# IIT-PAVIS/DiffAssemble

Hardware: AMD Instinct MI355X
Metric: denoising steps/sec (900-piece dense graph, T=100) (higher is better)
Workload: dtype bf16

## Files before the change

### diffassemble_amd/_lib.py

```python
import ctypes as C
import os

import torch

LIB_PATH = os.environ.get("DA_LIB_PATH") or os.path.join(os.path.dirname(os.path.abspath(__file__)), "lib", "libdiffassemble_hip.so")
DA_MAX_LAYERS = 8
ABI_VERSION = 19
PREC_F32, PREC_BF16 = 0, 1
VARIANT_2D, VARIANT_3D, VARIANT_DISCRETE, VARIANT_DISCRETE_ROT = 0, 1, 2, 3
ARCH_TRANSFORMER, ARCH_EXOPHORMER, ARCH_GCN = 0, 1, 2
MEAN_EPSILON, MEAN_START_X = 0, 1
ACT_NONE, ACT_GELU, ACT_LEAKY02 = 0, 1, 2
CONV_Q_PRESCALED, CONV_FOLDED_V32 = 1, 2
TRAIN_MMA_FP32, TRAIN_MMA_BF16 = 0, 1
TRAIN_BWD_ALL, TRAIN_BWD_EARLY, TRAIN_BWD_LATE = 0, 1, 2
D3PM_DRAW_SAMPLING, D3PM_DRAW_TRAINING, D3PM_DRAW_SAMPLING_ROT = 0, 1, 2
D3PM_LOSS = {"vb": 0, "cross_entropy": 1, "hybrid": 2}
DBG_COUNTERS = ("opt_gen_workgroups", "dense_fast_exits", "dual_gen_slabs", "opt_masked_gen_workgroups")
DBG_LAUNCH_COUNTERS = {"resident_launches": 4, "virtual_rows_in_launch": 5,
                       "resident_projection_launches": 6}
PROF_CLASSES = ("embed", "linear_mlp", "linear_qkvs", "attn_hidden", "attn_last", "head", "update", "conv_fused")

_fp = C.c_void_p
_FPL = _fp * DA_MAX_LAYERS


class DaWeights(C.Structure):
    _fields_ = [
        ("variant", C.c_int32), ("arch", C.c_int32), ("steps", C.c_int32), ("c_in", C.c_int32),
        ("c_out", C.c_int32), ("feat_dim", C.c_int32), ("hidden", C.c_int32), ("heads", C.c_int32),
        ("n_layers", C.c_int32), ("virt_nodes", C.c_int32),
        ("time_emb", _fp),
        ("pos_w0", _fp), ("pos_b0", _fp), ("pos_w1", _fp), ("pos_b1", _fp),
        ("mlp_w0", _fp), ("mlp_b0", _fp), ("mlp_w1", _fp), ("mlp_b1", _fp),
        ("conv_wq", _FPL), ("conv_bq", _FPL), ("conv_wk", _FPL), ("conv_bk", _FPL),
        ("conv_wv", _FPL), ("conv_bv", _FPL), ("conv_ws", _FPL), ("conv_bs", _FPL),
        ("virt_emb", _fp),
        ("head_w0", _fp), ("head_b0", _fp), ("head_w1", _fp), ("head_b1", _fp),
        ("head_r_w0", _fp), ("head_r_b0", _fp), ("head_r_w1", _fp), ("head_r_b1", _fp),
    ]


class DaGraph(C.Structure):
    _fields_ = [
        ("n_nodes", C.c_int32), ("n_real", C.c_int32), ("n_graphs", C.c_int32), ("dense", C.c_int32),
        ("n_edges", C.c_int64),
        ("row_ptr", _fp), ("col_src", _fp), ("edge_id", _fp), ("graph_ptr", _fp),
        ("max_graph_nodes", C.c_int32), ("n_pad", C.c_int32),
        ("pad_ptr", _fp), ("row_map", _fp),
        ("out_ptr", _fp), ("out_dst", _fp),
        ("hybrid", C.c_int32), ("band_degree", C.c_int32),
        ("mask", _fp), ("mask_ptr", _fp), ("irr_row_ptr", _fp), ("irr_col_src", _fp),
        ("slot_node", _fp), ("blk_class", _fp), ("blk_class_ptr", _fp), ("blk_class_stride", C.c_int32), ("reserved1", C.c_int32),
        ("rm_meta", _fp), ("agg_row_ptr", _fp), ("agg_col_src", _fp), ("agg_mult", _fp),
    ]


class DaLoopOpts(C.Structure):
    _fields_ = [("sampler", C.c_int32), ("eta", C.c_float), ("cfg", C.c_int32), ("cfg_w", C.c_float), ("noise", C.c_void_p)]


class DaD3pmOpts(C.Structure):
    _fields_ = [("cfg", C.c_int32), ("cfg_w", C.c_float), ("noise", C.c_void_p), ("seed", C.c_void_p)]


class DaD3pmRotOpts(C.Structure):
    _fields_ = [("cold", C.c_int32), ("reserved0", C.c_int32), ("x_fixed", C.c_void_p), ("noise_x", C.c_void_p), ("noise_rot", C.c_void_p),
                ("seed", C.c_void_p)]


class DaSchedule(C.Structure):
    _fields_ = [
        ("steps", C.c_int32),
        ("betas", _fp), ("alphas_cumprod", _fp), ("sqrt_recip_alphas", _fp),
        ("sqrt_recip_alphas_cumprod", _fp), ("sqrt_recipm1_alphas_cumprod", _fp),
        ("sqrt_one_minus_alphas_cumprod", _fp), ("posterior_variance", _fp),
    ]


ENCODER_CONVS, ENCODER_FEATS = 19, 1088


class DaEncoderWeights(C.Structure):
    _fields_ = [
        ("n_convs", C.c_int32), ("reserved0", C.c_int32),
        ("stem_w", _fp), ("stem_b", _fp),
        ("conv_w", _fp * ENCODER_CONVS), ("conv_b", _fp * ENCODER_CONVS),
        ("lin1_w", _fp), ("lin1_b", _fp), ("lin2_w", _fp), ("lin2_b", _fp),
    ]


PCD_STAGES, PCD_K = 3, 20


class DaPcdEncoderWeights(C.Structure):
    _fields_ = [
        ("feat_dim", C.c_int32), ("reserved0", C.c_int32),
        ("premap", _fp * PCD_STAGES), ("bn_a", _fp * PCD_STAGES), ("conv_b", _fp * PCD_STAGES),
        ("conv6", _fp), ("linear0", _fp),
    ]


LOSS3D_TRANS, LOSS3D_SHAPE_CD, LOSS3D_ROT, LOSS3D_ALL = 1, 2, 4, 7
PCD_TRAIN_LAYERS = 8


class DaPcdTrainWeights(C.Structure):
    _fields_ = [
        ("feat_dim", C.c_int32), ("reserved0", C.c_int32),
        ("premap", _fp * PCD_STAGES), ("bn_a", _fp * PCD_STAGES), ("conv_b", _fp * PCD_STAGES),
        ("conv6", _fp), ("linear0", _fp),
        ("gamma", _fp * PCD_TRAIN_LAYERS), ("beta", _fp * PCD_TRAIN_LAYERS),
        ("running_mean", _fp * PCD_TRAIN_LAYERS), ("running_var", _fp * PCD_TRAIN_LAYERS),
        ("momentum", C.c_float * PCD_TRAIN_LAYERS), ("eps", C.c_float * PCD_TRAIN_LAYERS),
        ("inv_wf", _fp * 2), ("inv_wd", _fp * 2),
    ]


class DaPcdTrainGrads(C.Structure):
    _fields_ = [
        ("wf", _fp * 6), ("wd", _fp * 6), ("gamma", _fp * 6), ("beta", _fp * 6),
        ("linear0_w", _fp), ("linear0_b", _fp), ("points", _fp),
    ]


PCD_PASSES = ("PREMAP", "EDGE_STAT_A", "EDGE_STAT_B", "EDGE_BWD1", "EDGE_BWD2", "EDGE_BWD3", "C6_STAT", "C6_BWD1", "C6_BWD2", "C6_DX",
              "BN_FIN_FWD", "BN_FIN_BWD", "REV_ADJ", "GATHER", "PREMAP_WGRAD", "HEAD_BWD", "LIN0_GRAD", "VN_LIN", "VN_STAT", "VN_APPLY")
PCD_PASS = {n: i for i, n in enumerate(PCD_PASSES)}


class DaPcdPassArgs(C.Structure):
    _fields_ = ([(n, C.c_int32) for n in ("n_parts", "n_points", "cin", "feat", "has_b", "inv", "channels", "nblk", "ld_x", "ld_g", "ld_m",
                                         "vn_cin")]
                + [("count", C.c_double), ("momentum", C.c_float), ("eps", C.c_float)]
                + [(n, _fp) for n in ("x", "w", "w2", "T", "idx", "rec_a", "rec_b", "dX_in", "partial", "Gb", "Hb", "E", "X1", "X2", "X3", "dm_in",
                                      "G6", "F", "dX1", "dX2", "dX3", "gamma", "beta", "running_mean", "running_var", "run_out", "ss",
                                      "dgamma", "dbeta", "cnt", "ptr", "cur", "rev", "dXp", "dTc", "Xc", "dWm", "dwf", "dwd", "grad_out",
                                      "dm", "vP", "vD", "vY")])


def pcd_train_pass(name, stream=None, **fields):
    a = DaPcdPassArgs()
    keys = dict(DaPcdPassArgs._fields_)
    for k, v in fields.items():
        if k not in keys:
            raise DaError(f"da_pcd_pass_args has no field {k!r}")
        setattr(a, k, v.data_ptr() if torch.is_tensor(v) else v)
    check(lib().da_pcd_train_pass(PCD_PASS[name], C.byref(a), stream if stream is not None else stream_ptr()))


class DaConfig(C.Structure):
    _fields_ = [(n, C.c_int32) for n in ("struct_bytes", "disable_mfma", "disable_dense", "disable_folds", "attn_level", "xpanel", "tail_next",
                                         "pair_split", "train_attn", "train_side_streams")]


PROTOTYPES = {
    "da_abi_version": (C.c_int, []),
    "da_last_error": (C.c_char_p, []),
    "da_config_get": (C.c_int, [C.POINTER(DaConfig)]),
    "da_config_set": (C.c_int, [C.POINTER(DaConfig)]),
    "da_build_flags": (C.c_int, []),
    "da_denoiser_create": (C.c_int, [C.POINTER(DaWeights), C.c_int, _fp, C.POINTER(_fp)]),
    "da_denoiser_destroy": (None, [_fp]),
    "da_denoiser_flags": (C.c_int, [_fp]),
    "da_gcn_dinv": (C.c_int, [C.POINTER(DaGraph), _fp, _fp]),
    "da_gcn_aggregate": (C.c_int, [C.c_int, C.POINTER(DaGraph), C.c_int, _fp, _fp, _fp, C.c_int, _fp, _fp]),
    "da_denoiser_workspace_bytes": (C.c_size_t, [_fp, C.POINTER(DaGraph)]),
    "da_denoiser_set_features": (C.c_int, [_fp, C.POINTER(DaGraph), _fp, _fp, C.c_size_t, _fp]),
    "da_denoiser_forward": (C.c_int, [_fp, C.POINTER(DaGraph), _fp, _fp, C.c_int64, _fp, _fp, C.c_int, _fp, _fp,
                                      C.c_size_t, _fp]),
    "da_ddim_step": (C.c_int, [C.POINTER(DaSchedule), C.c_int, C.c_int, C.c_int, C.c_int, _fp, _fp, _fp,
                               C.c_int64, C.c_int, C.c_int, C.c_float, _fp, _fp, _fp]),
    "da_ddpm_step": (C.c_int, [C.POINTER(DaSchedule), C.c_int, C.c_int, _fp, _fp, _fp, C.c_int64, _fp, _fp, _fp]),
# ... 158 lines not shown
```

### diffassemble_amd/csrc/da_api.hip

```cpp
#include <stdarg.h>
#include <stdlib.h>
#include <string.h>

#include <utility>
#include <vector>

#include "da_common.h"
#include "da_internal.h"
#include "da_config.h"

namespace da {

static thread_local char g_err[1024] = "";

void set_error(const char *fmt, ...) {
    va_list ap;
    va_start(ap, fmt);
    vsnprintf(g_err, sizeof(g_err), fmt, ap);
    va_end(ap);
}

struct ConvW {
    void *w = nullptr;
    float *b = nullptr;
    void *wd = nullptr;
    float *bd = nullptr;
    void *wdp = nullptr;
    void *wqs = nullptr;
    int din = 0, hc = 0, C = 0;
};

__global__ void k_scale_block(float *p, int rows, int cols, int ld, float s) {
    const size_t i = (size_t)blockIdx.x * blockDim.x + threadIdx.x;
    if (i < (size_t)rows * cols) p[(i / cols) * ld + (i % cols)] *= s;
}
static int scale_block(float *p, int rows, int cols, int ld, float s, hipStream_t st) {
    const size_t n = (size_t)rows * cols;
    if (!n) return 0;
    k_scale_block<<<(unsigned)((n + 255) / 256), 256, 0, st>>>(p, rows, cols, ld, s);
    DA_LAUNCH_CHECK();
    return 0;
}
__global__ void k_fill_bias_rows(int prec, int rows, int cols, const float *bias, void *dst) {
    const size_t i = (size_t)blockIdx.x * blockDim.x + threadIdx.x;
    if (i >= (size_t)rows * cols) return;
    const float v = bias[i % cols];
    if (prec == DA_PREC_BF16) ((bf16_t *)dst)[i] = f2bf(v); else ((float *)dst)[i] = v;
}
__global__ void k_cfg_combine(size_t n, float wgt, float *cond, const float *unc) {
    const size_t i = (size_t)blockIdx.x * blockDim.x + threadIdx.x;
    if (i < n) cond[i] = (1.0f + wgt) * cond[i] - wgt * unc[i];
}
static bool q_prescale_on() { return !(cfg().disable_folds & DA_FOLD_QSCALE); }
static float q_scale_log2(int C) { return 1.4426950408889634f / sqrtf((float)C); }

struct LoopKey {
    da_graph g;
    da_schedule s;
    int mean_type, ratio, max_iters;
    const float *x_init;
    float *traj, *x_final;
    void *ws;
    size_t ws_bytes;
    da_loop_opts opts;
    size_t traj_stride;
    size_t noise_stride;
    da_config cfg;
    const void *seed;
    const void *rot_init, *rot_traj, *rot_final, *x_fixed, *noise_rot;
    int cold;
};

}

using namespace da;

struct da_denoiser {
    int prec = 0, variant = 0, arch = 0, steps = 0, c_in = 0, c_out = 0, F = 0, D = 0, hidden = 0, heads = 0,
        n_layers = 0, V = 0, head_hidden = 0;
    float *time_emb = nullptr, *pos_w0 = nullptr, *pos_b0 = nullptr, *pos_w1 = nullptr, *pos_b1 = nullptr;
    void *mlp_w0 = nullptr, *mlp_w1 = nullptr;
    float *mlp_b0 = nullptr, *mlp_b1 = nullptr;
    ConvW conv[DA_MAX_LAYERS];
    void *virt_emb = nullptr;
    void *head_w0 = nullptr;
    float *head_b0 = nullptr;
    float *head_w1 = nullptr, *head_b1 = nullptr, *head_r_w1 = nullptr, *head_r_b1 = nullptr;
    bool fused_mlp2 = false;
    void *conv0c_w = nullptr;
    float *conv0c_b = nullptr;
    void *headc_w = nullptr;
    float *headc_b = nullptr;
    void *virt_qkvs = nullptr;
    void *conv0c_wd = nullptr, *virt_qkvs_d = nullptr;
    void *conv0c_wdp = nullptr, *convLf_wp = nullptr;
    void *conv0c_wqs = nullptr;
    bool attn_qsf = false;
    float *conv0c_bd = nullptr;
    bool q_prescaled = false;
    bool lastfold = false;
    bool dense_only = false;
    void *convLf_w = nullptr;
    float *convLf_b = nullptr;
    void *skipc_w = nullptr;
    float *skipc_b = nullptr;
    std::vector<void *> owned;
    bool prof_on = false;
    std::vector<hipEvent_t> prof_ev;
    std::vector<int> prof_cls;
    size_t prof_used = 0;
    struct LoopEntry { LoopKey a, b; hipGraphExec_t exec, exec_b; };
    std::vector<LoopEntry> loops;
    hipStream_t cap_stream = nullptr;
    hipStream_t side_stream = nullptr;
    hipEvent_t ev_fork = nullptr, ev_join = nullptr;
    hipStream_t pair_stream = nullptr;
    hipEvent_t ev_pair_fork = nullptr, ev_pair_join = nullptr;
    std::vector<LoopEntry> pair_loops;
};

namespace da {

struct Workspace {
    char *comb_in, *h, *combined, *qkvs, *xa, *xb, *z, *hh;
    char *hh_unc, *pz_unc, *head_pre_unc;
    void *pz;
    char *head_pre;
    char *feat_proj;
    char *feat_proj_unc;
    char *feat_proj4;
    size_t proj4_stride;
    float *model_out_unc;
    char *dq, *dk, *dvt, *dskip;
    size_t dense_off, dense_bytes;
    unsigned *virt_cnt;
    float *virt_part;
    float *model_out, *xbuf0, *xbuf1;
    float *gcn_dinv;
    size_t total;
};

static Workspace carve(const da_denoiser *d, const da_graph *g, void *base) {
    const size_t s = esize(d->prec);
    const size_t n = (size_t)g->n_nodes, nr = (size_t)g->n_real;
    const size_t nrp = nr + 64, np = n + 64;
    char *p = (char *)base;
    size_t off = 0;
    auto take = [&](size_t bytes) {
        char *q = p ? p + off : nullptr;
        off += align_up(bytes, 256);
        return q;
    };
    Workspace w;
    int hcmax = 0;
    for (int l = 0; l < d->n_layers; ++l) hcmax = d->conv[l].hc > hcmax ? d->conv[l].hc : hcmax;
    w.comb_in = take(nrp * d->D * s);
    w.h = take(nrp * d->hidden * s);
    w.feat_proj = take(nrp * d->hidden * s);
    w.feat_proj_unc = take(nrp * d->hidden * s);
    const bool rotv = d->variant == DA_VARIANT_DISCRETE_ROT;
    w.head_pre = take(nrp * (rotv ? 64 : 32) * s);
    w.pz = take(nrp * 32 * (size_t)d->heads * sizeof(float));
    w.combined = take(np * d->D * s);
    const bool gcn = d->arch == DA_ARCH_GCN;
    w.qkvs = take(gcn ? 0 : np * 4 * (size_t)hcmax * s);
    w.xa = take(np * 256 * s);
    w.xb = take(np * 256 * s);
    w.z = take(np * d->D * s);
    w.hh = take(nrp * d->head_hidden * s);
    const bool disc = d->variant == DA_VARIANT_DISCRETE;
    w.hh_unc = take(disc ? nrp * d->head_hidden * s : 0);
    w.pz_unc = take(disc ? nrp * 32 * (size_t)d->heads * sizeof(float) : 0);
    w.head_pre_unc = take(disc ? nrp * 32 * s : 0);
    w.dq = w.dk = w.dvt = w.dskip = nullptr;
    w.virt_cnt = nullptr; w.virt_part = nullptr;
    w.dense_off = off;
    w.dense_bytes = 0;
    if ((g->dense || g->hybrid) && g->n_pad > 0 && !gcn) {
        const size_t hb = ((size_t)g->n_pad + 64) * hcmax * s;
        w.dq = take(hb);
        w.dk = take(hb);
        w.dvt = take(hb);
        if (g->hybrid && n > nr) w.virt_cnt = (unsigned *)take((n - nr) * sizeof(unsigned));
        w.dense_bytes = off - w.dense_off;
        if (g->hybrid && n > nr) w.virt_part = (float *)take((n - nr) * (size_t)DA_VIRT_SPLIT_MAX * 64 * 6 * sizeof(float));
        w.dskip = take(np * (size_t)hcmax * s);
    }
    const int cpose = d->variant == DA_VARIANT_3D ? 7 : d->c_out;
    w.model_out = (float *)take(nr * cpose * sizeof(float));
    w.model_out_unc = (float *)take(nr * cpose * sizeof(float));
    w.xbuf0 = (float *)take(nr * 8 * sizeof(float));
    w.xbuf1 = (float *)take(nr * 8 * sizeof(float));
    w.gcn_dinv = d->arch == DA_ARCH_GCN ? (float *)take(n * sizeof(float)) : nullptr;
    w.proj4_stride = align_up(nrp * d->hidden * s, 256) / s;
    w.feat_proj4 = take(rotv ? 4 * w.proj4_stride * s : 0);
    w.total = off;
    return w;
}

static bool mfma_disabled() { return cfg().disable_mfma != 0; }

int linear(int prec, int M, int K, int Nout, const void *A, int lda, const void *W, const float *bias, int act,
           const void *res, void *out, int ldo, hipStream_t st) {
    if (!mfma_disabled()) {
        const int rc = launch_gemm_mfma(prec, M, K, Nout, A, lda, W, bias, act, res, out, ldo, nullptr, st);
        if (rc >= 0) return rc;
    }
    return launch_gemm_simple(prec == DA_PREC_F32_BF16MMA ? DA_PREC_F32 : prec, M, K, Nout, A, lda, W, bias, act, res, out, ldo, st);
}

static bool dense_disabled() { return cfg().disable_dense != 0; }

static bool step_rule_batch(const da_graph *g) { return g->max_graph_nodes >= 512 || g->n_real >= 16384; }

static bool stream_is_capturing(hipStream_t st) {
    hipStreamCaptureStatus cs = hipStreamCaptureStatusNone;
    return hipStreamIsCapturing(st, &cs) == hipSuccess && cs == hipStreamCaptureStatusActive;
}

static bool dense_ok(const da_graph *g, int heads, int C) {
    const bool hyb = g->hybrid && g->mask && g->mask_ptr && g->irr_row_ptr;
    return !dense_disabled() && (g->dense || hyb) && g->n_pad > 0 && g->graph_ptr && g->pad_ptr && g->row_map && heads == 8 &&
           (C == 32 || C == 144) && !mfma_disabled();
}

static int check_graph(const da_denoiser *d, const da_graph *g) {
    DA_REQUIRE(g && g->n_real > 0 && g->n_nodes >= g->n_real, "da_graph: bad node counts");
    const bool hyb = g->hybrid && g->mask && g->mask_ptr && g->irr_row_ptr;
    if (!((g->dense || hyb) && d->dense_only)) DA_REQUIRE(g->row_ptr && (g->col_src || g->n_edges == 0), "da_graph: CSR arrays missing");
    DA_REQUIRE(d->V == 0 || g->n_nodes == g->n_real + d->V * g->n_graphs,
               "da_graph: exophormer expects n_nodes = n_real + V*G (%d vs %d + %d*%d)", g->n_nodes, g->n_real,
               d->V, g->n_graphs);
    return 0;
}

static DeviceSchedule to_dev(const da_schedule *s) {
    DeviceSchedule r;
    r.steps = s->steps;
    r.betas = s->betas;
    r.alphas_cumprod = s->alphas_cumprod;
    r.sqrt_recip_alphas = s->sqrt_recip_alphas;
    r.sqrt_recip_alphas_cumprod = s->sqrt_recip_alphas_cumprod;
    r.sqrt_recipm1_alphas_cumprod = s->sqrt_recipm1_alphas_cumprod;
    r.sqrt_one_minus_alphas_cumprod = s->sqrt_one_minus_alphas_cumprod;
    r.posterior_variance = s->posterior_variance;
    return r;
}

template <typename F>
static int timed(da_denoiser *d, int cls, hipStream_t st, F &&launch) {
    if (!d->prof_on) return launch();
    if (d->prof_used + 2 > d->prof_ev.size()) {
        for (int k = 0; k < 2; ++k) {
            hipEvent_t e;
            DA_CHECK_HIP(hipEventCreate(&e));
            d->prof_ev.push_back(e);
        }
    }
    hipEvent_t a = d->prof_ev[d->prof_used], b = d->prof_ev[d->prof_used + 1];
    DA_CHECK_HIP(hipEventRecord(a, st));
    int rc = launch();
    DA_CHECK_HIP(hipEventRecord(b, st));
    d->prof_used += 2;
    d->prof_cls.push_back(cls);
    return rc;
}

struct DiscreteIn {
    const int32_t *idx;
    char *hh;
    char *pz, *pre;
    int folded;
    int rot = 0;
    const int32_t *rot_acc = nullptr;
    D3pmRows rows() const { D3pmRows r; if (folded) { r.pz = pz; r.pre = pre; } else r.hh = hh; return r; }
};

static int forward_impl(da_denoiser *d, const da_graph *g, const float *x, const int64_t *t, int64_t t_scalar,
                        float *out, float *alpha, int alpha_all, float *pre_head, const Workspace &w,
                        hipStream_t st, DdimFuse *ddim = nullptr, bool uncond = false, bool h_ready = false,
                        DiscreteIn *disc = nullptr) {
    const int prec = d->prec, nr = g->n_real, n = g->n_nodes, D = d->D;
    int rc;
    VirtScatter vsc;
    bool virt_scattered = false;
    if (!h_ready && d->fused_mlp2 && n > nr && !alpha && w.dq && d->virt_qkvs_d && dense_ok(g, d->heads, d->conv[0].C) && DA_XENV("DA_VIRT_SCATTER_IN_EMBED", 1)) {
        vsc.rows = n - nr; vsc.V = d->V; vsc.H = d->heads; vsc.C = d->conv[0].C; vsc.n_real = nr; vsc.n_pad = g->n_pad;
        vsc.src = d->virt_qkvs_d; vsc.row_map = g->row_map; vsc.Q = w.dq; vsc.K = w.dk; vsc.Vt = w.dvt; vsc.S = w.dskip;
        virt_scattered = true;
    }
    if (disc) {
        disc->folded = 0;
        if ((rc = timed(d, DA_PROF_EMBED, st, [&] {
                 if (disc->rot)
                     return launch_embed_idx_time_rot(prec, nr, d->c_out, d->F, D, d->hidden, disc->idx, disc->rot_acc, t, t_scalar, d->steps, d->time_emb,
                                                      d->pos_w1, w.comb_in, w.feat_proj4, w.proj4_stride, w.feat_proj, st);
                 return launch_embed_idx_time(prec, nr, d->c_out, d->F, D, disc->idx, t, t_scalar, d->steps, d->time_emb, d->pos_w1, w.comb_in, st); }))) return rc;
    } else
    if (!h_ready && (rc = timed(d, DA_PROF_EMBED, st, [&] {
             return launch_embed_pos_time(prec, nr, d->c_in, d->F, D, x, t, t_scalar, d->steps, d->time_emb,
                                          d->pos_w0, d->pos_b0, d->pos_w1, d->pos_b1, w.comb_in, st, virt_scattered ? &vsc : nullptr); }))) return rc;
    const int act1 = d->variant == DA_VARIANT_3D ? DA_ACT_LEAKY02 : DA_ACT_GELU;
    const int act2 = d->variant == DA_VARIANT_3D ? DA_ACT_LEAKY02 : DA_ACT_NONE;
    if (!h_ready && (rc = timed(d, DA_PROF_LINEAR_MLP, st, [&] {
             const size_t es_ = esize(prec);
             int r2 = mfma_disabled() ? -1
                                      : launch_gemm_mfma(prec, nr, D - d->F, d->hidden, w.comb_in + (size_t)d->F * es_, D,
                                                         (const char *)d->mlp_w0 + (size_t)d->F * es_, nullptr, act1, nullptr,
                                                         w.h, d->hidden, nullptr, st, D, uncond ? w.feat_proj_unc : w.feat_proj);
             if (r2 >= 0) return r2;
             if (uncond) { set_error("unconditional pass: the hoisted mlp.0 path is not available for this shape"); return 1; }
             if (disc && disc->rot) { set_error("discrete rot: the hoisted mlp.0 path is not available for this shape"); return 1; }
             return linear(prec, nr, D, d->hidden, w.comb_in, D, d->mlp_w0, d->mlp_b0, act1, nullptr, w.h, d->hidden, st); }))) return rc;
    const bool fused = d->fused_mlp2;
    if (!fused && (rc = timed(d, DA_PROF_LINEAR_MLP, st, [&] {
             return linear(prec, nr, d->hidden, D, w.h, d->hidden, d->mlp_w1, d->mlp_b1, act2, nullptr, w.combined, D, st); }))) return rc;
    const void *xin = fused ? w.h : w.combined;
    int ldx = fused ? d->hidden : D;
    if (d->arch == DA_ARCH_GCN) {
        const ConvW &c0 = d->conv[0], &c1 = d->conv[1];
        const int hid = c0.hc;
        if ((rc = timed(d, DA_PROF_LINEAR_QKVS, st, [&] {
                 return linear(prec, nr, D, hid, w.combined, D, c0.w, nullptr, DA_ACT_NONE, nullptr, w.xa, hid, st); }))) return rc;
        if ((rc = timed(d, DA_PROF_ATTN_HIDDEN, st, [&] {
                 return launch_gcn_aggregate(prec, g, hid, w.gcn_dinv, w.xa, c0.b, DA_ACT_GELU, w.xb, st); }))) return rc;
        if ((rc = timed(d, DA_PROF_ATTN_LAST, st, [&] {
                 return launch_gcn_aggregate(prec, g, hid, w.gcn_dinv, w.xb, nullptr, DA_ACT_NONE, w.xa, st); }))) return rc;
        if ((rc = timed(d, DA_PROF_LINEAR_QKVS, st, [&] {
                 return linear(prec, nr, hid, D, w.xa, hid, c1.w, c1.b, DA_ACT_GELU, w.combined, w.z, D, st); }))) return rc;
    } else
    for (int l = 0; l < d->n_layers; ++l) {
        ConvW c = d->conv[l];
        if (fused && l == 0) { c.w = d->conv0c_w; c.b = d->conv0c_b; c.din = d->hidden; }
        const int nproj = (fused && l == 0) ? nr : n;
        const bool virt0 = fused && l == 0 && n > nr;
        const bool last = l == d->n_layers - 1;
        void *dst = last ? (void *)w.z : (void *)((l & 1) ? w.xb : w.xa);
        const int act = (!last && d->arch == DA_ARCH_TRANSFORMER) ? DA_ACT_GELU : DA_ACT_NONE;
        float *al = !alpha ? nullptr
                           : (alpha_all ? alpha + (size_t)l * g->n_edges * d->heads : (last ? alpha : nullptr));
        const void *resid = (last && !fused) ? w.combined : nullptr;
        if (last && fused && d->lastfold && !al && w.dq && (g->hybrid || d->V == 0) && dense_ok(g, d->heads, c.C)) {
            QkvScatter qs;
            qs.HC = c.hc; qs.C = c.C; qs.Cv = 32; qs.n_pad = g->n_pad; qs.row_map = g->row_map;
            qs.Q = w.dq; qs.K = w.dk; qs.Vt = w.dvt; qs.S = nullptr;
            rc = timed(d, DA_PROF_LINEAR_QKVS, st, [&] {
                return launch_gemm_mfma(prec, n, c.din, 2 * c.hc + d->heads * 32, xin, ldx, d->convLf_w, d->convLf_b, DA_ACT_NONE,
                                        nullptr, nullptr, 0, &qs, st, 0, nullptr, d->convLf_wp); });
            if (rc > 0) return rc;
            if (rc == 0) {
                DenseLayout L;
                L.Q = w.dq; L.K = w.dk; L.Vt = w.dvt; L.S = nullptr; L.n_pad = g->n_pad; L.q_prescaled = d->q_prescaled;
                DenseFold fo;
                fo.cv = 32; fo.out = disc ? (void *)disc->pz : w.pz; fo.n_rows = nr;
                const DenseMask mk = dense_mask_of(g);
                rc = timed(d, DA_PROF_ATTN_LAST, st, [&] {
                    return launch_attn_dense(prec, L, d->heads, c.C, g->n_graphs, g->max_graph_nodes, g->graph_ptr,
                                             g->pad_ptr, g->dense == 2, nullptr, DA_ACT_NONE, nullptr, st,
                                             g->hybrid ? &mk : nullptr, &fo); });
                if (rc > 0) return rc;
                if (rc == 0 && disc) {
                    if ((rc = timed(d, DA_PROF_HEAD, st, [&] {
                             return linear(prec, nr, d->hidden, 32, w.h, d->hidden, d->headc_w, d->headc_b, DA_ACT_NONE, nullptr, disc->pre, 32, st); }))) return rc;
                    if ((rc = timed(d, DA_PROF_HEAD, st, [&] {
                             return linear(prec, nr, c.din, 32, xin, ldx, d->skipc_w, d->skipc_b, DA_ACT_NONE, disc->pre, disc->pre, 32, st); }))) return rc;
                    disc->folded = 1;
                    return 0;
                }
                if (rc == 0) {
                    {
                        const bool fuse_ddim = ddim && d->c_out == d->c_in;
                        int rt = -1;
                        if ((rc = timed(d, DA_PROF_HEAD, st, [&] {
                                 rt = launch_tail_fused(prec, nr, d->heads, d->c_out, d->hidden, c.din, w.h, xin, ldx, d->headc_w, d->headc_b,
                                                        d->skipc_w, d->skipc_b, w.pz, d->head_w1, d->head_b1, out, st, fuse_ddim ? ddim : nullptr);
                                 return rt > 0 ? rt : 0; }))) return rc;
                        if (rt == 0) { if (fuse_ddim) ddim->done = 1; return 0; }
                    }
                    if ((rc = timed(d, DA_PROF_HEAD, st, [&] {
                             return linear(prec, nr, d->hidden, 32, w.h, d->hidden, d->headc_w, d->headc_b, DA_ACT_NONE, nullptr, w.head_pre, 32, st); }))) return rc;
                    if ((rc = timed(d, DA_PROF_HEAD, st, [&] {
                             return linear(prec, nr, c.din, 32, xin, ldx, d->skipc_w, d->skipc_b, DA_ACT_NONE, w.head_pre, w.head_pre, 32, st); }))) return rc;
                    if (ddim && d->c_out == d->c_in) ddim->done = 1;
                    return timed(d, DA_PROF_HEAD, st, [&] {
                        return launch_head_fold(prec, nr, d->heads, d->c_out, w.pz, w.head_pre, d->head_w1, d->head_b1, out, st,
                                                (ddim && ddim->done) ? ddim : nullptr); });
                }
            }
        }
#ifdef DA_EXPERIMENTS
        if (!al && !last && g->dense && !g->hybrid && n == nr && !resid && dense_ok(g, d->heads, c.C) &&
            conv_fused_applicable(prec, d->heads, c.C, c.din, g->max_graph_nodes, c.hc)) {
            rc = timed(d, DA_PROF_CONV_FUSED, st, [&] {
                return launch_conv_fused(prec, d->heads, c.C, c.din, g->n_graphs, g->max_graph_nodes, g->graph_ptr,
                                         g->dense == 2, xin, ldx, c.w, c.b, act, dst, c.hc, st); });
            if (rc) return rc < 0 ? 1 : rc;
            xin = dst; ldx = c.hc;
            continue;
        }
#endif
        if (!al && w.dq && dense_ok(g, d->heads, c.C)) {
            QkvScatter qs;
            qs.HC = c.hc; qs.C = c.C; qs.n_pad = g->n_pad; qs.row_map = g->row_map;
            qs.Q = w.dq; qs.K = w.dk; qs.Vt = w.dvt; qs.S = w.dskip;
            const void *wdense = (fused && l == 0) ? d->conv0c_wd : c.wd;
            const float *bdense = (fused && l == 0) ? d->conv0c_bd : c.bd;
            const int xpm = xpanel_mode();
            const void *wpanel = (xpm == 1 || (xpm == 2 && step_rule_batch(g))) ? ((fused && l == 0) ? d->conv0c_wdp : c.wdp) : nullptr;
            const void *wqs = (fused && l == 0) ? d->conv0c_wqs : c.wqs;
            const bool qsf = !last && !g->hybrid && !resid && !virt0 && n == nr && wqs && ldx == c.din &&
                             attn_qsf_applicable(prec, d->heads, c.C, c.din, g->n_graphs, g->max_graph_nodes, g->n_pad, d->q_prescaled);
            if (qsf) rc = 0; else
            rc = timed(d, DA_PROF_LINEAR_QKVS, st, [&] {
                return launch_gemm_mfma(prec, nproj, c.din, 4 * c.hc, xin, ldx, wdense, bdense, DA_ACT_NONE, nullptr, nullptr, 0, &qs, st, 0,
                                        nullptr, wpanel); });
            if (rc > 0) return rc;
            if (rc == 0 && virt0 && !virt_scattered &&
                (rc = launch_scatter_virtual(prec, n - nr, d->V, d->heads, c.C, d->virt_qkvs_d, nr, g->row_map, g->n_pad, w.dq, w.dk,
                                             w.dvt, w.dskip, nullptr, st))) return rc;
            if (rc == 0) {
                DenseLayout L;
                L.Q = w.dq; L.K = w.dk; L.Vt = w.dvt; L.S = w.dskip; L.n_pad = g->n_pad; L.q_prescaled = d->q_prescaled;
                if (qsf) { L.x = xin; L.ldx = ldx; L.kin = c.din; L.wqs = wqs; L.bias = bdense; }
                if (g->hybrid) {
                    DenseMask mk = dense_mask_of(g);
                    int virt_taken = 0;
                    [[maybe_unused]] const int vil = DA_XENV("DA_VIRT_IN_LAUNCH", 1);
                    if (n > nr && !resid && w.virt_cnt && w.virt_part && !(cfg().disable_folds & DA_FOLD_HYBRID_OVERLAP) && vil && (g->n_real < 8192 || vil == 2)) {
                        mk.v_rows = n - nr; mk.v_n_real = nr;
                        mk.v_row_ptr = g->agg_row_ptr ? g->agg_row_ptr : g->irr_row_ptr; mk.v_col_src = g->agg_row_ptr ? g->agg_col_src : g->irr_col_src;
                        mk.v_mult = g->agg_row_ptr ? g->agg_mult : nullptr;
                        mk.v_part = w.virt_part; mk.v_cnt = w.virt_cnt; mk.v_taken = &virt_taken;
                        rc = timed(d, last ? DA_PROF_ATTN_LAST : DA_PROF_ATTN_HIDDEN, st, [&] {
                            return launch_attn_dense(prec, L, d->heads, c.C, g->n_graphs, g->max_graph_nodes, g->graph_ptr, g->pad_ptr, 0, resid, act, dst, st, &mk); });
                        if (rc) return rc < 0 ? 1 : rc;
                        if (!virt_taken) {
                            rc = timed(d, last ? DA_PROF_ATTN_LAST : DA_PROF_ATTN_HIDDEN, st, [&] {
                                return launch_attn_csr_cont(prec, n, nr, mk.v_row_ptr, mk.v_col_src, g->row_map, d->heads, c.C, g->n_pad, L, resid, act, dst, st, mk.v_mult); });
                            if (rc) return rc < 0 ? 1 : rc;
                        }
                        xin = dst; ldx = c.hc;
                        continue;
                    }
                    if (d->side_stream && !d->prof_on && n > nr && g->n_real >= 8192) {
                        StreamJoin side_guard;
                        DA_CHECK_HIP(hipEventRecord(d->ev_fork, st));
                        DA_CHECK_HIP(hipStreamWaitEvent(d->side_stream, d->ev_fork, 0));
                        side_guard.arm(d->side_stream, st, d->ev_join);
                        rc = launch_attn_csr_cont(prec, n, nr, g->agg_row_ptr ? g->agg_row_ptr : g->irr_row_ptr, g->agg_row_ptr ? g->agg_col_src : g->irr_col_src,
                                                  g->row_map, d->heads, c.C, g->n_pad, L, resid, act, dst, d->side_stream, g->agg_row_ptr ? g->agg_mult : nullptr);
                        if (rc) return rc < 0 ? 1 : rc;
                        DA_CHECK_HIP(hipEventRecord(d->ev_join, d->side_stream));
                        rc = launch_attn_dense(prec, L, d->heads, c.C, g->n_graphs, g->max_graph_nodes, g->graph_ptr,
                                               g->pad_ptr, 0, resid, act, dst, st, &mk);
                        if (rc) return rc < 0 ? 1 : rc;
                        DA_CHECK_HIP(hipStreamWaitEvent(st, d->ev_join, 0));
                        side_guard.armed = false;
                        xin = dst; ldx = c.hc;
                        continue;
                    }
                    rc = timed(d, last ? DA_PROF_ATTN_LAST : DA_PROF_ATTN_HIDDEN, st, [&] {
                        int r2 = launch_attn_dense(prec, L, d->heads, c.C, g->n_graphs, g->max_graph_nodes, g->graph_ptr,
                                                   g->pad_ptr, 0, resid, act, dst, st, &mk);
                        if (r2) return r2;
                        return launch_attn_csr_cont(prec, n, nr, g->agg_row_ptr ? g->agg_row_ptr : g->irr_row_ptr, g->agg_row_ptr ? g->agg_col_src : g->irr_col_src,
                                                    g->row_map, d->heads, c.C, g->n_pad, L, resid, act, dst, st, g->agg_row_ptr ? g->agg_mult : nullptr); });
                    if (rc) return rc < 0 ? 1 : rc;
                    xin = dst; ldx = c.hc;
                    continue;
                }
                rc = timed(d, qsf ? DA_PROF_CONV_FUSED : (last ? DA_PROF_ATTN_LAST : DA_PROF_ATTN_HIDDEN), st, [&] {
                    return launch_attn_dense(prec, L, d->heads, c.C, g->n_graphs, g->max_graph_nodes, g->graph_ptr,
                                             g->pad_ptr, g->dense == 2, resid, act, dst, st); });
                if (rc > 0) return rc;
                if (rc == 0) { xin = dst; ldx = c.hc; continue; }
            }
        }
        if ((rc = timed(d, DA_PROF_LINEAR_QKVS, st, [&] {
                 return linear(prec, nproj, c.din, 4 * c.hc, xin, ldx, c.w, c.b, DA_ACT_NONE, nullptr, w.qkvs, 4 * c.hc, st); }))) return rc;
        if (virt0 && (rc = launch_scatter_virtual(prec, n - nr, d->V, d->heads, c.C, d->virt_qkvs, nr, nullptr, 0, nullptr, nullptr,
                                                  nullptr, nullptr, w.qkvs, st))) return rc;
        DA_REQUIRE(g->row_ptr && (g->col_src || g->n_edges == 0), "da_graph: this call walks the edge list (alpha requested or no "
                   "MFMA attention for this layer) but the CSR arrays are missing");
        int tiny = -1;
        if (!al && g->dense && n == nr && g->graph_ptr && !dense_disabled()) {
            if ((rc = timed(d, last ? DA_PROF_ATTN_LAST : DA_PROF_ATTN_HIDDEN, st, [&] {
                     tiny = launch_attn_tiny(prec, g->n_graphs, g->max_graph_nodes, g->graph_ptr, g->dense == 2, d->heads, c.C, w.qkvs, resid, act, dst, st);
                     return tiny > 0 ? tiny : 0; }))) return rc;
        }
        if (tiny != 0 && (rc = timed(d, last ? DA_PROF_ATTN_LAST : DA_PROF_ATTN_HIDDEN, st, [&] {
                 return launch_attn_csr(prec, n, g->row_ptr, g->col_src, g->edge_id, d->heads, c.C, w.qkvs,
                                        resid, act, dst, al, nullptr, st); }))) return rc;
        xin = dst;
        ldx = c.hc;
    }
    char *const hh = disc ? disc->hh : w.hh;
    if (fused) {
        const int hw = d->variant == DA_VARIANT_DISCRETE_ROT ? 64 : 32;
        if ((rc = timed(d, DA_PROF_HEAD, st, [&] {
                 return linear(prec, nr, d->hidden, hw, w.h, d->hidden, d->headc_w, d->headc_b, DA_ACT_NONE, nullptr, w.head_pre, hw, st); }))) return rc;
        rc = timed(d, DA_PROF_HEAD, st, [&] {
            return launch_gemm_mfma(prec, nr, D, d->head_hidden, w.z, D, d->head_w0, d->head_b0, DA_ACT_GELU, nullptr, hh,
                                    d->head_hidden, nullptr, st, D, w.head_pre); });
        if (rc > 0) return rc;
        DA_REQUIRE(rc == 0, "fused head GEMM: shape not supported");
    } else if ((rc = timed(d, DA_PROF_HEAD, st, [&] {
             return linear(prec, nr, D, d->head_hidden, w.z, D, d->head_w0, d->head_b0, DA_ACT_GELU, nullptr, hh,
                           d->head_hidden, st); }))) return rc;
    if (disc) return 0;
    return timed(d, DA_PROF_HEAD, st, [&] {
        if (d->variant == DA_VARIANT_3D)
            return launch_head3d(prec, nr, hh, d->head_w1, d->head_b1, d->head_r_w1, d->head_r_b1, out, pre_head, st);
        return launch_head2d(prec, nr, d->c_out, hh, d->head_w1, d->head_b1, out, st);
    });
}

}

__global__ void k_pair_delay(unsigned long long ticks) {
    const unsigned long long t0 = wall_clock64();
    while (wall_clock64() - t0 < ticks) __builtin_amdgcn_s_sleep(32);
}


static int loop_iters(const da_schedule *s, int ratio, int max_iters) {
    const int total = (s->steps + ratio - 1) / ratio;
    return (max_iters > 0 && max_iters < total) ? max_iters : total;
}

static int loop_opts(const char *who, const da_denoiser *d, const da_loop_opts *opts, da_loop_opts *o) {
    memset(o, 0, sizeof(*o));
    if (opts) { o->sampler = opts->sampler; o->eta = opts->eta; o->cfg = opts->cfg; o->cfg_w = opts->cfg_w; o->noise = opts->noise; }
    DA_REQUIRE(o->sampler == 0 || o->sampler == 1, "%s: sampler must be 0 (DDIM) or 1 (DDPM)", who);
    DA_REQUIRE(!(o->sampler == 1 || o->eta > 0.f) || o->noise, "%s: eta > 0 / DDPM need the noise buffer", who);
    DA_REQUIRE(d->variant == DA_VARIANT_2D || (!o->cfg && o->sampler == 0 && o->eta == 0.f), "%s: the 3D loop has no guidance / stochastic variant", who);
    return 0;
}

static LoopKey loop_key(const da_graph *g, const da_schedule *s, int mean_type, int ratio, int n_iters, const void *x_init, void *traj,
                        void *x_final, void *ws, size_t ws_bytes, const da_loop_opts &o, size_t traj_stride = 0, size_t noise_stride = 0,
                        const void *seed = nullptr) {
    LoopKey k;
    memset(&k, 0, sizeof(k));
    k.g = *g; k.s = *s; k.mean_type = mean_type; k.ratio = ratio; k.max_iters = n_iters;
    k.x_init = (const float *)x_init; k.traj = (float *)traj; k.x_final = (float *)x_final; k.ws = ws; k.ws_bytes = ws_bytes;
    k.opts = o; k.traj_stride = traj ? traj_stride : 0; k.noise_stride = o.noise ? noise_stride : 0;
    k.cfg = cfg(); k.seed = seed;
    return k;
}
static const LoopKey no_key = {};

static const da_denoiser::LoopEntry *cache_find(const std::vector<da_denoiser::LoopEntry> &c, const LoopKey &a, const LoopKey &b, bool two_graphs) {
    const da_denoiser::LoopEntry *hit = nullptr;
    for (const auto &e : c)
        if (memcmp(&a, &e.a, sizeof(a)) == 0 && memcmp(&b, &e.b, sizeof(b)) == 0 && (e.exec_b != nullptr) == two_graphs) hit = &e;
    return hit;
}
static void cache_insert(std::vector<da_denoiser::LoopEntry> &c, size_t capacity, const da_denoiser::LoopEntry &e) {
    if (c.size() >= capacity) {
        (void)hipGraphExecDestroy(c.front().exec);
        if (c.front().exec_b) (void)hipGraphExecDestroy(c.front().exec_b);
        c.erase(c.begin());
    }
    c.push_back(e);
}

template <typename F>
static int record_graph(da_denoiser *d, const char *what, F &&enqueue, hipGraphExec_t *out) {
    *out = nullptr;
    if (!d->cap_stream) DA_CHECK_HIP(hipStreamCreateWithFlags(&d->cap_stream, hipStreamNonBlocking));
    hipStream_t cs = d->cap_stream;
    hipGraph_t graph = nullptr;
    DA_CHECK_HIP(hipStreamBeginCapture(cs, hipStreamCaptureModeRelaxed));
    const int rc = enqueue(cs);
    const hipError_t e_end = hipStreamEndCapture(cs, &graph);
    const bool captured = e_end == hipSuccess && graph;
    hipError_t e_inst = hipSuccess;
    if (!rc && captured) e_inst = hipGraphInstantiate(out, graph, nullptr, nullptr, 0);
    if (graph) (void)hipGraphDestroy(graph);
    if (rc) return rc;
    if (!captured) { set_error("%s: hipStreamEndCapture failed: %s", what, hipGetErrorString(e_end)); return 2; }
    if (e_inst != hipSuccess || !*out) { *out = nullptr; set_error("%s: hipGraphInstantiate failed: %s", what, hipGetErrorString(e_inst)); return 2; }
    return 0;
}

template <typename F>
static int launch_loop_graph(da_denoiser *d, const char *what, const LoopKey &key, F &&enqueue, hipStream_t st) {
    const da_denoiser::LoopEntry *hit = cache_find(d->loops, key, no_key, false);
    hipGraphExec_t exec = hit ? hit->exec : nullptr;
    if (!exec) {
        const int rc = record_graph(d, what, enqueue, &exec);
        if (rc) return rc;
        cache_insert(d->loops, 8, {key, no_key, exec, nullptr});
    }
    DA_CHECK_HIP(hipGraphLaunch(exec, st));
    return 0;
}

static int ensure_pair_stream(da_denoiser *d) {
    if (d->pair_stream) return 0;
    const int prio = DA_XENV("DA_PAIR_PRIO", 0);
    if (prio) {
        int lo = 0, hi = 0;
        DA_CHECK_HIP(hipDeviceGetStreamPriorityRange(&lo, &hi));
        DA_CHECK_HIP(hipStreamCreateWithPriority(&d->pair_stream, hipStreamNonBlocking, prio > 0 ? hi : lo));
    } else
        DA_CHECK_HIP(hipStreamCreateWithFlags(&d->pair_stream, hipStreamNonBlocking));
    DA_CHECK_HIP(hipEventCreateWithFlags(&d->ev_pair_fork, hipEventDisableTiming));
    DA_CHECK_HIP(hipEventCreateWithFlags(&d->ev_pair_join, hipEventDisableTiming));
    return 0;
}
static int fork_pair_stream(da_denoiser *d, hipStream_t us, StreamJoin &join) {
    DA_CHECK_HIP(hipEventRecord(d->ev_pair_fork, us));
    DA_CHECK_HIP(hipStreamWaitEvent(d->pair_stream, d->ev_pair_fork, 0));
    join.arm(d->pair_stream, us, d->ev_pair_join);
    return 0;
}

extern "C" {

int da_abi_version(void) { return DA_ABI_VERSION; }
const char *da_last_error(void) { return da::g_err; }

int da_denoiser_create(const da_weights *w, int precision, void *stream, da_denoiser **out) {
    DA_REQUIRE(w && out, "da_denoiser_create: null argument");
    DA_REQUIRE(precision == DA_PREC_F32 || precision == DA_PREC_BF16, "bad precision %d", precision);
    DA_REQUIRE(w->n_layers >= 2 && w->n_layers <= DA_MAX_LAYERS, "n_layers out of range");
    DA_REQUIRE(w->arch == DA_ARCH_TRANSFORMER || w->arch == DA_ARCH_EXOPHORMER || w->arch == DA_ARCH_GCN, "bad arch %d", w->arch);
    DA_REQUIRE(w->arch != DA_ARCH_GCN || w->n_layers == 2, "gcn arch: n_layers must be 2 (backbones/gcn.py:9-14)");
    DA_REQUIRE(w->heads == 8, "heads must be 8");
    DA_REQUIRE(w->c_in >= 1 && w->c_in <= 8, "da_denoiser_create: c_in = %d outside [1, 8]", w->c_in);
    DA_REQUIRE(w->variant == DA_VARIANT_2D || w->variant == DA_VARIANT_3D || w->variant == DA_VARIANT_DISCRETE || w->variant == DA_VARIANT_DISCRETE_ROT,
               "bad variant %d", w->variant);
    const bool rotv = w->variant == DA_VARIANT_DISCRETE_ROT;
    const bool discrete = w->variant == DA_VARIANT_DISCRETE || rotv;
    if (discrete) {
        DA_REQUIRE(w->c_in == 1, "da_denoiser_create(discrete): c_in must be 1 (one position index per piece), got %d", w->c_in);
        DA_REQUIRE(w->c_out >= 2 && w->c_out <= 1024, "da_denoiser_create(discrete): K = c_out = %d outside [2, 1024]", w->c_out);
        DA_REQUIRE(w->arch == DA_ARCH_TRANSFORMER, "da_denoiser_create(discrete): arch must be DA_ARCH_TRANSFORMER");
        DA_REQUIRE(w->pos_w1 && w->head_w1 && w->head_b1, "da_denoiser_create(discrete): pos_w1 (pos_mlp.weight [K, 32]) / head_w1 / head_b1 missing");
        DA_REQUIRE(!rotv || (w->head_w0 && w->head_b0 && w->head_r_w0 && w->head_r_b0 && w->head_r_w1 && w->head_r_b1),
                   "da_denoiser_create(discrete rot): head_w0 / head_b0 or head_r_w0 / head_r_b0 / head_r_w1 / head_r_b1 (final_mlp_rot) missing");
    }
    hipStream_t st = (hipStream_t)stream;
    da_denoiser *d = new da_denoiser();
    d->prec = precision; d->variant = w->variant; d->arch = w->arch; d->steps = w->steps; d->c_in = w->c_in;
    d->c_out = w->c_out; d->F = w->feat_dim; d->D = w->feat_dim + 64; d->hidden = w->hidden; d->heads = w->heads;
    d->n_layers = w->n_layers; d->V = w->arch == DA_ARCH_EXOPHORMER ? w->virt_nodes : 0;
    d->head_hidden = w->variant == DA_VARIANT_3D ? 512 : (rotv ? 64 : 32);
    const int D = d->D, H = d->heads;
    const size_t s = esize(precision);
    int rc = 0;
    auto fail = [&](int code) { da_denoiser_destroy(d); return code; };
    auto alloc = [&](size_t bytes) -> void * {
        void *p = nullptr;
        if (hipMalloc(&p, bytes < 256 ? 256 : bytes) != hipSuccess) { set_error("hipMalloc(%zu) failed", bytes); return nullptr; }
        d->owned.push_back(p);
        return p;
    };
    auto copy_f32 = [&](const float *src, size_t n) -> float * {
        float *p = (float *)alloc(n * 4);
        if (!p || hipMemcpyAsync(p, src, n * 4, hipMemcpyDeviceToDevice, st) != hipSuccess) { rc = 2; return nullptr; }
        return p;
    };
    auto pack = [&](const float *src, size_t n) -> void * {
        void *p = alloc(n * s + 4096);
        if (!p || launch_convert(precision, n, src, p, st)) { rc = 2; return nullptr; }
        return p;
    };
    d->attn_qsf = attn_qsf_enabled();
    auto pack_qs = [&](const void *wsrc, int K, int hc, int C) -> void * {
        if (!d->attn_qsf) return nullptr;
        if (precision != DA_PREC_BF16 || C != 32 || H != 8 || (K != 128 && K != 256) || !wsrc || mfma_disabled()) return nullptr;
        void *p = alloc(w_qs_bytes(H, K));
        if (!p || pack_w_qs(H, K, hc, wsrc, p, st)) { rc = 2; return nullptr; }
        return p;
    };
    auto pack_panel = [&](const void *wsrc, int K, int Nout) -> void * {
        const size_t nb = xpanel_in_model() ? da_linear_packed_bytes(precision, K, Nout) : 0;
        if (!nb || !wsrc) return nullptr;
        void *p = alloc(nb);
        if (!p || pack_w_xpanel(K, Nout, wsrc, K, p, st)) { rc = 2; return nullptr; }
        return p;
    };
    d->time_emb = copy_f32(w->time_emb, (size_t)w->steps * 32);
    if (discrete) {
        d->pos_w1 = copy_f32(w->pos_w1, (size_t)w->c_out * 32);
    } else {
        d->pos_w0 = copy_f32(w->pos_w0, 16 * (size_t)w->c_in); d->pos_b0 = copy_f32(w->pos_b0, 16);
        d->pos_w1 = copy_f32(w->pos_w1, 32 * 16); d->pos_b1 = copy_f32(w->pos_b1, 32);
    }
    d->mlp_w0 = pack(w->mlp_w0, (size_t)d->hidden * D); d->mlp_b0 = copy_f32(w->mlp_b0, d->hidden);
    d->mlp_w1 = pack(w->mlp_w1, (size_t)D * d->hidden); d->mlp_b1 = copy_f32(w->mlp_b1, D);
    if (rc) return fail(rc);
    if (d->arch == DA_ARCH_GCN) {
        for (int l = 0; l < 2; ++l) {
            ConvW &c = d->conv[l];
            c.din = l == 0 ? D : 256;
            c.hc = l == 0 ? 256 : D;
            if (!w->conv_wq[l] || !w->conv_bq[l]) { set_error("gcn conv %d: missing weight pointer", l); return fail(1); }
            c.w = pack(w->conv_wq[l], (size_t)c.hc * c.din);
            c.b = copy_f32(w->conv_bq[l], c.hc);
            c.wd = c.w; c.bd = c.b;
            if (rc) return fail(rc);
        }
    }
    for (int l = 0; l < (d->arch == DA_ARCH_GCN ? 0 : d->n_layers); ++l) {
        ConvW &c = d->conv[l];
        c.din = l == 0 ? D : 32 * H;
        c.C = l == d->n_layers - 1 ? D / H : 32;
        c.hc = c.C * H;
        const size_t blk = (size_t)c.hc * c.din;
        char *wp = (char *)alloc(4 * blk * s + 4096);
        c.b = (float *)alloc(4 * (size_t)c.hc * 4);
        if (!wp || !c.b) return fail(2);
        c.w = wp;
        const float *ws[4] = {w->conv_wq[l], w->conv_wk[l], w->conv_wv[l], w->conv_ws[l]};
        const float *bs[4] = {w->conv_bq[l], w->conv_bk[l], w->conv_bv[l], w->conv_bs[l]};
        for (int k = 0; k < 4; ++k) {
            if (!ws[k] || !bs[k]) { set_error("conv %d: missing weight pointer", l); return fail(1); }
            if (launch_convert(precision, blk, ws[k], wp + k * blk * s, st)) return fail(2);
            if (hipMemcpyAsync(c.b + (size_t)k * c.hc, bs[k], (size_t)c.hc * 4, hipMemcpyDeviceToDevice, st) != hipSuccess) return fail(2);
        }
        c.wd = c.w; c.bd = c.b;
        if (q_prescale_on()) {
            char *wd = (char *)alloc(4 * blk * s + 4096);
            float *tq = (float *)alloc(blk * 4);
            c.bd = (float *)alloc(4 * (size_t)c.hc * 4);
            if (!wd || !tq || !c.bd) return fail(2);
            c.wd = wd;
            if (hipMemcpyAsync(tq, ws[0], blk * 4, hipMemcpyDeviceToDevice, st) != hipSuccess) return fail(2);
            if (scale_block(tq, c.hc, c.din, c.din, q_scale_log2(c.C), st)) return fail(2);
            if (launch_convert(precision, blk, tq, wd, st)) return fail(2);
            if (hipMemcpyAsync(wd + blk * s, wp + blk * s, 3 * blk * s, hipMemcpyDeviceToDevice, st) != hipSuccess) return fail(2);
            if (hipMemcpyAsync(c.bd, c.b, 4 * (size_t)c.hc * 4, hipMemcpyDeviceToDevice, st) != hipSuccess) return fail(2);
            if (scale_block(c.bd, 1, c.hc, c.hc, q_scale_log2(c.C), st)) return fail(2);
        }
        c.wdp = pack_panel(c.wd, c.din, 4 * c.hc);
        if (l < d->n_layers - 1) c.wqs = pack_qs(c.wd, c.din, c.hc, c.C);
        if (rc) return fail(rc);
    }
    d->q_prescaled = q_prescale_on();
    if (d->V > 0) {
        if (!w->virt_emb) { set_error("exophormer: virt_emb missing"); return fail(1); }
        d->virt_emb = pack(w->virt_emb, (size_t)d->V * D);
    }
    float *hw0 = nullptr;
    if (d->variant == DA_VARIANT_3D) {
        char *hp = (char *)alloc(512 * (size_t)D * s + 4096);
        d->head_b0 = (float *)alloc(512 * 4);
        if (!hp || !d->head_b0) return fail(2);
        d->head_w0 = hp;
        if (launch_convert(precision, 256 * (size_t)D, w->head_w0, hp, st)) return fail(2);
        if (launch_convert(precision, 256 * (size_t)D, w->head_r_w0, hp + 256 * (size_t)D * s, st)) return fail(2);
        if (hipMemcpyAsync(d->head_b0, w->head_b0, 256 * 4, hipMemcpyDeviceToDevice, st) != hipSuccess) return fail(2);
        if (hipMemcpyAsync(d->head_b0 + 256, w->head_r_b0, 256 * 4, hipMemcpyDeviceToDevice, st) != hipSuccess) return fail(2);
        d->head_w1 = copy_f32(w->head_w1, 3 * 256); d->head_b1 = copy_f32(w->head_b1, 3);
        d->head_r_w1 = copy_f32(w->head_r_w1, 3 * 256); d->head_r_b1 = copy_f32(w->head_r_b1, 3);
    } else if (rotv) {
        hw0 = (float *)alloc(64 * (size_t)D * 4);
        d->head_b0 = (float *)alloc(64 * 4);
        if (!hw0 || !d->head_b0) return fail(2);
        if (hipMemcpyAsync(hw0, w->head_w0, 32 * (size_t)D * 4, hipMemcpyDeviceToDevice, st) != hipSuccess) return fail(2);
        if (hipMemcpyAsync(hw0 + 32 * (size_t)D, w->head_r_w0, 32 * (size_t)D * 4, hipMemcpyDeviceToDevice, st) != hipSuccess) return fail(2);
        if (hipMemcpyAsync(d->head_b0, w->head_b0, 32 * 4, hipMemcpyDeviceToDevice, st) != hipSuccess) return fail(2);
        if (hipMemcpyAsync(d->head_b0 + 32, w->head_r_b0, 32 * 4, hipMemcpyDeviceToDevice, st) != hipSuccess) return fail(2);
        d->head_w0 = pack(hw0, 64 * (size_t)D);
        d->head_w1 = copy_f32(w->head_w1, (size_t)w->c_out * 32); d->head_b1 = copy_f32(w->head_b1, w->c_out);
        d->head_r_w1 = copy_f32(w->head_r_w1, 4 * 32); d->head_r_b1 = copy_f32(w->head_r_b1, 4);
    } else {
        d->head_w0 = pack(w->head_w0, 32 * (size_t)D); d->head_b0 = copy_f32(w->head_b0, 32);
        d->head_w1 = copy_f32(w->head_w1, (size_t)w->c_out * 32); d->head_b1 = copy_f32(w->head_b1, w->c_out);
    }
    if (rc) return fail(rc);
    {
        const bool off = (cfg().disable_folds & DA_FOLD_MLP2) != 0;
        if (!off && !mfma_disabled() && (d->variant == DA_VARIANT_2D || discrete) && d->hidden % 32 == 0 && d->arch != DA_ARCH_GCN) {
            const int hid = d->hidden, hc0 = d->conv[0].hc;
            float *w2t = (float *)alloc((size_t)hid * D * 4);
            float *cw = (float *)alloc((size_t)4 * hc0 * hid * 4);
            const int hwn = rotv ? 64 : 32;
            const float *hsrc = rotv ? hw0 : w->head_w0;
            float *hw = (float *)alloc((size_t)hwn * hid * 4);
            d->conv0c_b = (float *)alloc((size_t)4 * hc0 * 4);
            d->headc_b = (float *)alloc(hwn * 4);
            if (!w2t || !cw || !hw || !d->conv0c_b || !d->headc_b) return fail(2);
            if (launch_transpose_f32(D, hid, w->mlp_w1, w2t, st)) return fail(2);
            const float *ws[4] = {w->conv_wq[0], w->conv_wk[0], w->conv_wv[0], w->conv_ws[0]};
            const float *bs[4] = {w->conv_bq[0], w->conv_bk[0], w->conv_bv[0], w->conv_bs[0]};
            for (int k = 0; k < 4; ++k) {
                if (launch_gemm_simple(DA_PREC_F32, hc0, D, hid, ws[k], D, w2t, nullptr, DA_ACT_NONE, nullptr,
                                       cw + (size_t)k * hc0 * hid, hid, st)) return fail(2);
                if (launch_gemm_simple(DA_PREC_F32, 1, D, hc0, w->mlp_b1, D, ws[k], bs[k], DA_ACT_NONE, nullptr,
                                       d->conv0c_b + (size_t)k * hc0, hc0, st)) return fail(2);
            }
            if (launch_gemm_simple(DA_PREC_F32, hwn, D, hid, hsrc, D, w2t, nullptr, DA_ACT_NONE, nullptr, hw, hid, st)) return fail(2);
            if (launch_gemm_simple(DA_PREC_F32, 1, D, hwn, w->mlp_b1, D, hsrc, nullptr, DA_ACT_NONE, nullptr, d->headc_b, hwn, st)) return fail(2);
            d->conv0c_w = pack(cw, (size_t)4 * hc0 * hid);
            d->headc_w = pack(hw, (size_t)hwn * hid);
            d->conv0c_wd = d->conv0c_w; d->conv0c_bd = d->conv0c_b;
            if (d->q_prescaled) {
                d->conv0c_bd = (float *)alloc((size_t)4 * hc0 * 4);
                if (!d->conv0c_bd) return fail(2);
                if (hipMemcpyAsync(d->conv0c_bd, d->conv0c_b, (size_t)4 * hc0 * 4, hipMemcpyDeviceToDevice, st) != hipSuccess) return fail(2);
                if (scale_block(d->conv0c_bd, 1, hc0, hc0, q_scale_log2(d->conv[0].C), st)) return fail(2);
                if (scale_block(cw, hc0, hid, hid, q_scale_log2(d->conv[0].C), st)) return fail(2);
                d->conv0c_wd = pack(cw, (size_t)4 * hc0 * hid);
            }
            d->conv0c_wdp = pack_panel(d->conv0c_wd, hid, 4 * hc0);
            if (d->n_layers > 1) d->conv0c_wqs = pack_qs(d->conv0c_wd, hid, hc0, d->conv[0].C);
            if (d->V > 0) {
                float *vq = (float *)alloc((size_t)d->V * 4 * hc0 * 4);
                if (!vq) return fail(2);
                for (int k = 0; k < 4; ++k)
                    if (launch_gemm_simple(DA_PREC_F32, d->V, D, hc0, w->virt_emb, D, ws[k], bs[k], DA_ACT_NONE, nullptr,
                                           vq + (size_t)k * hc0, 4 * hc0, st)) return fail(2);
                d->virt_qkvs = pack(vq, (size_t)d->V * 4 * hc0);
                d->virt_qkvs_d = d->virt_qkvs;
                if (d->q_prescaled) {
                    if (scale_block(vq, d->V, hc0, 4 * hc0, q_scale_log2(d->conv[0].C), st)) return fail(2);
                    d->virt_qkvs_d = pack(vq, (size_t)d->V * 4 * hc0);
                }
            }
// ... 402 lines not shown
}

int da_denoiser_set_features_rot(da_denoiser *d, const da_graph *g, const float *feats4, void *workspace, size_t workspace_bytes,
                                 void *stream) {
    DA_REQUIRE(d && g && feats4 && workspace, "da_denoiser_set_features_rot: null argument");
    int rc = require_rot("da_denoiser_set_features_rot", d);
    if (rc || (rc = check_graph(d, g))) return rc;
    Workspace w = carve(d, g, workspace);
    DA_REQUIRE(workspace_bytes >= w.total, "workspace too small: %zu < %zu", workspace_bytes, w.total);
    hipStream_t st = (hipStream_t)stream;
    for (int r = 3; r >= 0; --r) {
        if ((rc = launch_set_feats(d->prec, g->n_real, d->F, d->D, feats4 + (size_t)r * g->n_real * d->F, w.comb_in, st))) return rc;
        rc = launch_gemm_mfma(d->prec, g->n_real, d->F, d->hidden, w.comb_in, d->D, d->mlp_w0, d->mlp_b0, DA_ACT_NONE, nullptr,
                              w.feat_proj4 + (size_t)r * w.proj4_stride * esize(d->prec), d->hidden, nullptr, st, d->D, nullptr);
        if (rc > 0) return rc;
        DA_REQUIRE(rc == 0, "da_denoiser_set_features_rot: feature projection shape not supported (F=%d)", d->F);
    }
    if (w.dense_bytes)
        DA_CHECK_HIP(hipMemsetAsync((char *)workspace + w.dense_off, 0, w.dense_bytes, st));
    return 0;
}

int da_denoiser_forward_rot(da_denoiser *d, const da_graph *g, const int32_t *idx, const int32_t *rot_acc, const int64_t *t,
                            int64_t t_scalar, float *logits, float *rot_logits, float *alpha, int alpha_all_layers, void *workspace,
                            size_t workspace_bytes, void *stream) {
    DA_REQUIRE(d && g && idx && logits && rot_logits && workspace, "da_denoiser_forward_rot: null argument");
    int rc = require_rot("da_denoiser_forward_rot", d);
    if (rc || (rc = check_graph(d, g))) return rc;
    DA_REQUIRE(!alpha || g->edge_id, "alpha requested but graph has no edge_id");
    Workspace w = carve(d, g, workspace);
    DA_REQUIRE(workspace_bytes >= w.total, "workspace too small: %zu < %zu", workspace_bytes, w.total);
    hipStream_t st = (hipStream_t)stream;
    DiscreteIn di{idx, w.hh, (char *)w.pz, w.head_pre, 0, 1, rot_acc};
    if ((rc = forward_impl(d, g, nullptr, t, t_scalar, nullptr, alpha, alpha_all_layers, nullptr, w, st, nullptr, false, false, &di))) return rc;
    return timed(d, DA_PROF_HEAD, st, [&] {
        return launch_d3pm_rot_tail(d->prec, g->n_real, d->c_out, w.hh, d->head_w1, d->head_b1, d->head_r_w1, d->head_r_b1, nullptr, nullptr,
                                    logits, rot_logits, nullptr, st); });
}

static int enqueue_loop_rot(da_denoiser *d, const da_graph *g, const da_schedule *s, int ratio, int n_iters, const int32_t *idx_init,
                            const int32_t *rot_init, int32_t *traj_idx, int32_t *traj_acc, int32_t *idx_final, int32_t *acc_final,
                            const Workspace &w, hipStream_t st, const da_d3pm_rot_opts &o) {
    const int nr = g->n_real, K = d->c_out;
    const int first = ((s->steps - 1) / ratio) * ratio;
    int32_t *const st_idx = (int32_t *)w.xbuf0, *const st_acc = st_idx + nr, *const st_rot = (int32_t *)w.xbuf1;
    const int32_t *cur = idx_init, *rot = rot_init, *acc = nullptr;
    int it = 0, rc;
    for (int i = first; i >= 0 && it < n_iters; i -= ratio, ++it) {
        int32_t *nxt = traj_idx ? traj_idx + (size_t)it * nr : st_idx;
        int32_t *nacc = traj_acc ? traj_acc + (size_t)it * nr : st_acc;
        const int32_t *in = o.x_fixed ? o.x_fixed : cur;
        DiscreteIn di{in, w.hh, (char *)w.pz, w.head_pre, 0, 1, acc};
        if ((rc = forward_impl(d, g, nullptr, nullptr, i, nullptr, nullptr, 0, nullptr, w, st, nullptr, false, false, &di))) return rc;
        D3pmRotStep sp;
        sp.s = to_dev(s); sp.x_t = in; sp.rot_t = rot; sp.t_scalar = i; sp.ratio = ratio; sp.iteration = it; sp.seed = o.seed;
        sp.noise_x = o.noise_x ? o.noise_x + (size_t)it * nr * K : nullptr;
        sp.noise_rot = o.noise_rot ? o.noise_rot + (size_t)it * nr * 4 : nullptr;
        sp.x_prev = nxt; sp.cold = o.cold; sp.need_prev = o.cold;
        sp.rot_acc_in = acc; sp.rot_next = st_rot; sp.rot_acc_out = nacc;
        if ((rc = timed(d, DA_PROF_UPDATE, st, [&] {
                 return launch_d3pm_rot_tail(d->prec, nr, K, w.hh, d->head_w1, d->head_b1, d->head_r_w1, d->head_r_b1, nullptr, nullptr, nullptr,
                                             nullptr, &sp, st); }))) return rc;
        cur = nxt; acc = nacc; rot = st_rot;
    }
    if (idx_final && cur != idx_final) DA_CHECK_HIP(hipMemcpyAsync(idx_final, cur, (size_t)nr * sizeof(int32_t), hipMemcpyDeviceToDevice, st));
    if (acc_final && acc && acc != acc_final) DA_CHECK_HIP(hipMemcpyAsync(acc_final, acc, (size_t)nr * sizeof(int32_t), hipMemcpyDeviceToDevice, st));
    return 0;
}

int da_sample_loop_rot(da_denoiser *d, const da_graph *g, const da_schedule *s, int inference_ratio, int max_iters, const int32_t *idx_init,
                       const int32_t *rot_init, int32_t *traj_idx, int32_t *traj_rot_acc, int32_t *idx_final, int32_t *rot_acc_final,
                       void *workspace, size_t workspace_bytes, int use_graph, const da_d3pm_rot_opts *opts, void *stream) {
    DA_REQUIRE(d && g && s && idx_init && rot_init && workspace && opts, "da_sample_loop_rot: null argument");
    int rc = require_rot("da_sample_loop_rot", d);
    if (rc) return rc;
    DA_REQUIRE(inference_ratio >= 1 && s->steps >= 1 && s->alphas_cumprod, "da_sample_loop_rot: bad ratio / schedule");
    da_d3pm_rot_opts o;
    memset(&o, 0, sizeof(o));
    o.cold = opts->cold ? 1 : 0; o.x_fixed = opts->x_fixed; o.noise_x = opts->noise_x; o.noise_rot = o.cold ? opts->noise_rot : nullptr;
    o.seed = opts->seed;
    DA_REQUIRE((o.noise_x && (o.noise_rot || !o.cold)) || o.seed, "da_sample_loop_rot: needs the uniforms (opts->noise_x, opts->noise_rot) or a seed (opts->seed)");
    if ((rc = check_graph(d, g))) return rc;
    Workspace w = carve(d, g, workspace);
    DA_REQUIRE(workspace_bytes >= w.total, "workspace too small: %zu < %zu", workspace_bytes, w.total);
    hipStream_t st = (hipStream_t)stream;
    const int n_iters = loop_iters(s, inference_ratio, max_iters);
    auto enqueue = [&](hipStream_t on) {
        return enqueue_loop_rot(d, g, s, inference_ratio, n_iters, idx_init, rot_init, traj_idx, traj_rot_acc, idx_final, rot_acc_final, w, on, o); };
    if (d->prof_on || stream_is_capturing(st)) use_graph = 0;
    if (!use_graph) return enqueue(st);
    da_loop_opts ko;
    memset(&ko, 0, sizeof(ko));
    ko.noise = o.noise_x;
    LoopKey key = loop_key(g, s, -2, inference_ratio, n_iters, idx_init, traj_idx, idx_final, workspace, workspace_bytes, ko, 0, 0, o.seed);
    key.rot_init = rot_init; key.rot_traj = traj_rot_acc; key.rot_final = rot_acc_final; key.x_fixed = o.x_fixed; key.noise_rot = o.noise_rot;
    key.cold = o.cold;
    return launch_loop_graph(d, "da_sample_loop_rot", key, enqueue, st);
}

size_t da_attn_dense_scratch_bytes(int prec, const da_graph *g, int heads, int C) {
    if (!g) return 0;
    const size_t s = esize(prec), hc = (size_t)heads * C;
    return 3 * align_up(((size_t)g->n_pad + 64) * hc * s, 256) + align_up(((size_t)g->n_nodes + 64) * hc * s, 256);
}

int da_conv_dense(int prec, const da_graph *g, int heads, int C, int Din, const void *x, const void *w,
                  const float *b, const void *residual, int act, void *out, void *scratch, void *stream) {
    DA_REQUIRE(g && x && w && out && scratch, "da_conv_dense: null argument");
    DA_REQUIRE(dense_ok(g, heads, C), "da_conv_dense: graph is not dense or head width %d unsupported", C);
    hipStream_t st = (hipStream_t)stream;
    const size_t s = esize(prec), hc = (size_t)heads * C;
#ifdef DA_EXPERIMENTS
    if (!residual && !g->hybrid && conv_fused_applicable(prec, heads, C, Din, g->max_graph_nodes, (int)hc)) {
        int rf = launch_conv_fused(prec, heads, C, Din, g->n_graphs, g->max_graph_nodes, g->graph_ptr, g->dense == 2, x, Din, w,
                                   b, act, out, (int)hc, st);
        DA_REQUIRE(rf == 0, "da_conv_dense: fused conv launch failed (%d)", rf);
        return 0;
    }
#endif
    const size_t hb = align_up(((size_t)g->n_pad + 64) * hc * s, 256);
    char *base = (char *)scratch;
    QkvScatter qs;
    qs.HC = (int)hc; qs.C = C; qs.n_pad = g->n_pad; qs.row_map = g->row_map;
    qs.Q = base; qs.K = base + hb; qs.Vt = base + 2 * hb; qs.S = base + 3 * hb;
    int rc = launch_gemm_mfma(prec, g->n_nodes, Din, 4 * (int)hc, x, Din, w, b, DA_ACT_NONE, nullptr, nullptr, 0, &qs, st);
    DA_REQUIRE(rc <= 0, "da_conv_dense: projection launch failed");
    DA_REQUIRE(rc == 0, "da_conv_dense: projection shape (Din=%d, HC=%d) not supported by the MFMA kernel", Din, (int)hc);
    DenseLayout L;
    L.Q = qs.Q; L.K = qs.K; L.Vt = qs.Vt; L.S = qs.S; L.n_pad = g->n_pad;
    rc = launch_attn_dense(prec, L, heads, C, g->n_graphs, g->max_graph_nodes, g->graph_ptr, g->pad_ptr,
                           g->dense == 2, residual, act, out, st);
    DA_REQUIRE(rc == 0, "da_conv_dense: attention launch failed (%d)", rc);
    return 0;
}

int da_conv_dense_ex(int prec, const da_graph *g, int heads, int C, int Din, const void *x, const void *w, const float *b,
                     const void *residual, int act, void *out, void *scratch, int flags, void *stream) {
    DA_REQUIRE(g && x && w && out && scratch, "da_conv_dense_ex: null argument");
    DA_REQUIRE(dense_ok(g, heads, C), "da_conv_dense_ex: graph is not dense or head width %d unsupported", C);
    const bool folded = (flags & DA_CONV_FOLDED_V32) != 0;
    DA_REQUIRE(!folded || (C == 144 && !residual && act == DA_ACT_NONE), "da_conv_dense_ex: folded value heads need C = 144, no residual, no activation");
    hipStream_t st = (hipStream_t)stream;
    const size_t s = esize(prec), hc = (size_t)heads * C;
    const size_t hb = align_up(((size_t)g->n_pad + 64) * hc * s, 256);
    char *base = (char *)scratch;
    QkvScatter qs;
    qs.HC = (int)hc; qs.C = C; qs.n_pad = g->n_pad; qs.row_map = g->row_map;
    qs.Q = base; qs.K = base + hb; qs.Vt = base + 2 * hb; qs.S = folded ? nullptr : base + 3 * hb;
    qs.Cv = folded ? 32 : 0;
    const int nout = folded ? 2 * (int)hc + heads * 32 : 4 * (int)hc;
    const bool qsf = attn_qsf_enabled() && !folded && !residual && !g->hybrid && g->n_nodes == g->n_real && b && w_qs_bytes(heads, Din) <= 2 * hb &&
                     attn_qsf_applicable(prec, heads, C, Din, g->n_graphs, g->max_graph_nodes, g->n_pad, (flags & DA_CONV_Q_PRESCALED) ? 1 : 0);
    void *wq_img = base + hb;
    int rc = 0;
    if (qsf) {
        if ((rc = pack_w_qs(heads, Din, (int)hc, w, wq_img, st))) return rc;
    } else
    rc = launch_gemm_mfma(prec, g->n_nodes, Din, nout, x, Din, w, b, DA_ACT_NONE, nullptr, nullptr, 0, &qs, st);
    DA_REQUIRE(rc == 0, "da_conv_dense_ex: projection shape (Din=%d, Nout=%d) not supported by the MFMA kernels", Din, nout);
    DenseLayout L;
    L.Q = qs.Q; L.K = qs.K; L.Vt = qs.Vt; L.S = qs.S; L.n_pad = g->n_pad; L.q_prescaled = (flags & DA_CONV_Q_PRESCALED) ? 1 : 0;
    if (qsf) { L.x = x; L.ldx = Din; L.kin = Din; L.wqs = wq_img; L.bias = b; }
    DenseFold fo;
    fo.cv = 32; fo.out = out; fo.n_rows = g->n_real;
    const DenseMask mk = dense_mask_of(g);
    rc = launch_attn_dense(prec, L, heads, C, g->n_graphs, g->max_graph_nodes, g->graph_ptr, g->pad_ptr, g->dense == 2, residual, act,
                           folded ? nullptr : out, st, g->hybrid ? &mk : nullptr, folded ? &fo : nullptr);
    DA_REQUIRE(rc == 0, "da_conv_dense_ex: attention launch failed (%d)", rc);
    return 0;
}

int da_debug_counters(int64_t *out, int n, int reset) {
    DA_REQUIRE(out && n >= DA_DBG_NCOUNTERS, "da_debug_counters: need room for %d counters", DA_DBG_NCOUNTERS);
    unsigned long long a[4] = {0, 0, 0, 0}, b2[2] = {0, 0};
    int rc;
    if ((rc = da::attn_dense_counters(a, reset))) return rc;
#ifdef DA_EXPERIMENTS
    if ((rc = da::attn_dual_counters(b2, reset))) return rc;
#endif
    for (int k = 0; k < n; ++k) out[k] = 0;
    out[DA_DBG_OPT_GEN_WORKGROUPS] = (int64_t)a[0];
    out[DA_DBG_DENSE_FAST_EXITS] = (int64_t)a[1];
    out[DA_DBG_DUAL_GEN_SLABS] = (int64_t)b2[0];
    out[DA_DBG_OPT_MASKED_GEN_WORKGROUPS] = (int64_t)a[2];
    out[DA_DBG_RES_LAUNCHES] = (int64_t)da::attn_res_launches(reset);
    out[DA_DBG_RES_PROJ_LAUNCHES] = (int64_t)da::attn_res_qsf_launches(reset);
    out[DA_DBG_VIRT_IN_LAUNCH] = (int64_t)da::attn_virt_launches(reset);
    return 0;
}

int da_profile_enable(da_denoiser *d, int on) {
    DA_REQUIRE(d, "da_profile_enable: null denoiser");
    d->prof_on = on != 0;
    d->prof_used = 0;
    d->prof_cls.clear();
    return 0;
}

int da_profile_read(da_denoiser *d, float *ms, int32_t *counts) {
    DA_REQUIRE(d && ms && counts, "da_profile_read: null argument");
    for (int k = 0; k < DA_PROF_NCLASS; ++k) { ms[k] = 0.f; counts[k] = 0; }
    for (size_t k = 0; k < d->prof_cls.size(); ++k) {
        DA_CHECK_HIP(hipEventSynchronize(d->prof_ev[2 * k + 1]));
        float t = 0.f;
        DA_CHECK_HIP(hipEventElapsedTime(&t, d->prof_ev[2 * k], d->prof_ev[2 * k + 1]));
        ms[d->prof_cls[k]] += t;
        counts[d->prof_cls[k]] += 1;
    }
    d->prof_used = 0;
    d->prof_cls.clear();
    return 0;
}

int da_linear(int prec, int M, int K, int Nout, const void *A, int lda, const void *W, const float *bias, int act,
              const void *residual, void *out, int ldo, void *stream) {
    DA_REQUIRE(A && W && out, "da_linear: null argument");
    return da::linear(prec, M, K, Nout, A, lda, W, bias, act, residual, out, ldo, (hipStream_t)stream);
}

size_t da_linear_packed_bytes(int prec, int K, int Nout) {
    if (prec != DA_PREC_BF16 || (K != 128 && K != 256) || Nout < 512 || Nout > 4096 || (Nout & 31)) return 0;
    return da::xpanel_packed_bytes(K, Nout);
}

int da_linear_pack(int prec, int K, int Nout, const void *W, int ldw, void *packed, void *stream) {
    DA_REQUIRE(W && packed, "da_linear_pack: null argument");
    DA_REQUIRE(da_linear_packed_bytes(prec, K, Nout) > 0, "da_linear_pack: no packed form for prec %d, K %d, Nout %d", prec, K, Nout);
    DA_REQUIRE((((size_t)W) & 15) == 0 && (((size_t)packed) & 15) == 0 && ((ldw <= 0 ? K : ldw) & 7) == 0, "da_linear_pack: W / packed must be 16-byte aligned");
    return da::pack_w_xpanel(K, Nout, W, ldw, packed, (hipStream_t)stream);
}

int da_linear_packed(int prec, int M, int K, int Nout, const void *A, int lda, const void *W, const void *packed,
                     const float *bias, int act, const void *residual, void *out, int ldo, void *stream) {
    DA_REQUIRE(A && W && out, "da_linear_packed: null argument");
    if (!da::mfma_disabled()) {
        const int rc = da::launch_gemm_mfma(prec, M, K, Nout, A, lda, W, bias, act, residual, out, ldo, nullptr, (hipStream_t)stream, 0, nullptr,
                                            packed);
        if (rc >= 0) return rc;
    }
    return da::linear(prec, M, K, Nout, A, lda, W, bias, act, residual, out, ldo, (hipStream_t)stream);
}

int da_attn_csr(int prec, const da_graph *g, int heads, int C, const void *qkvs, const void *residual, int act,
                void *out, float *alpha, void *stream) {
    DA_REQUIRE(g && qkvs && out, "da_attn_csr: null argument");
    if (!alpha && g->dense && g->n_nodes == g->n_real && g->graph_ptr && !dense_disabled()) {
        const int rt = launch_attn_tiny(prec, g->n_graphs, g->max_graph_nodes, g->graph_ptr, g->dense == 2, heads, C, qkvs, residual, act, out, (hipStream_t)stream);
        if (rt >= 0) return rt;
    }
    return launch_attn_csr(prec, g->n_nodes, g->row_ptr, g->col_src, g->edge_id, heads, C, qkvs, residual, act, out,
                           alpha, nullptr, (hipStream_t)stream);
}

}
```

### diffassemble_amd/csrc/da_attn_common.h

```cpp
#pragma once
#include "da_common.h"
#include "da_internal.h"

namespace da {

typedef __attribute__((ext_vector_type(8))) __bf16 bf16x8;
typedef __attribute__((ext_vector_type(4))) __bf16 bf16x4;
typedef __attribute__((ext_vector_type(4))) float f32x4;
typedef __attribute__((ext_vector_type(4))) unsigned int u32x4;
typedef __attribute__((ext_vector_type(2))) unsigned int u32x2;
typedef __attribute__((ext_vector_type(16))) float f32x16;

struct AttnDenseParams {
    const void *Q, *K, *Vt, *S;
    const void *res;
    void *out;
    const int32_t *graph_ptr, *pad_ptr;
    int n_pad, H, n_graphs, nqt, act, nodiag;
    int max_nodes;
    float sc;
    unsigned long long *prof;
    int fast;
    int debug;
    int force_gen;
    const unsigned char *mask;
    const long long *mask_ptr;
    const int32_t *irr_row_ptr;
    const int32_t *irr_col_src;
    const int32_t *row_map;
    const int32_t *slot_node;
    const unsigned char *blk_class;
    const long long *blk_class_ptr;
    int blk_class_stride;
    const int32_t *rm_meta;
    void *fold_out;
    int n_rows;
    int v_rows, v_split, v_n_real;
    const int32_t *v_row_ptr, *v_col_src;
    const float *v_mult;
    float *v_part;
    unsigned *v_cnt;
    const void *x;
    int ldx, kin;
    const void *wqs;
    const float *bias_q, *bias_k, *bias_v, *bias_s;
};

template <typename T, int C, int CV = C, int BK = 0> struct Cfg {
    static constexpr int ES = (int)sizeof(T);
    static constexpr int ROWB = C * ES;
    static constexpr int ROWBV = CV * ES;
    static constexpr int NCH = ROWB / 32;
    static constexpr int RS = ROWB + (((ROWB / 16) & 1) ? 0 : 16);
    static constexpr int KSPR = RS / 16;
    static constexpr int KVALID = ROWB / 16;
    static constexpr int BKEYS = BK ? BK : (ES == 2 ? 64 : 32);
    static constexpr int KB = BKEYS / 32;
    static constexpr int RSV = ES == 2 ? ((ROWBV - 64 + 255) / 256 * 256 + 64) : ((ROWBV - 32 + 63) / 64 * 64 + 32);
    static constexpr int KVALIDV = ROWBV / 16;
    static constexpr int VSPR = RSV / 16;
    static constexpr int NCB = (CV + 31) / 32;
    static constexpr int NIK = (BKEYS * KSPR + 63) / 64;
    static constexpr int NIV = (BKEYS * VSPR + 63) / 64;
    static constexpr int NI = NIK + NIV;
    static constexpr int MAXI = (NI + 3) / 4;
    static constexpr int KBYTES = NIK * 1024, VBYTES = NIV * 1024, STAGE = KBYTES + VBYTES;
    static_assert(ROWB % 32 == 0, "head width must be a multiple of 32 bytes");
};

__device__ __forceinline__ f32x16 mma_chunk(bf16_t, const u32x4 &a, const u32x4 &b, f32x16 c) {
    return __builtin_amdgcn_mfma_f32_32x32x16_bf16(__builtin_bit_cast(bf16x8, a), __builtin_bit_cast(bf16x8, b), c, 0, 0, 0);
}
__device__ __forceinline__ f32x16 mma_chunk(float, const u32x4 &a, const u32x4 &b, f32x16 c) {
    const f32x4 x = __builtin_bit_cast(f32x4, a), y = __builtin_bit_cast(f32x4, b);
    c = __builtin_amdgcn_mfma_f32_32x32x2f32(x[0], y[0], c, 0, 0, 0);
    c = __builtin_amdgcn_mfma_f32_32x32x2f32(x[1], y[1], c, 0, 0, 0);
    c = __builtin_amdgcn_mfma_f32_32x32x2f32(x[2], y[2], c, 0, 0, 0);
    c = __builtin_amdgcn_mfma_f32_32x32x2f32(x[3], y[3], c, 0, 0, 0);
    return c;
}

__device__ __forceinline__ u32x2 tr_read(unsigned lds_byte_addr, int imm) {
    u32x2 r;
    asm volatile("ds_read_b64_tr_b16 %0, %1 offset:%2" : "=v"(r) : "v"(lds_byte_addr), "n"(imm));
    return r;
}
template <int RSV>
__device__ __forceinline__ f32x16 mma_pv_f32(const unsigned char *vcol, int half, const float (&p)[16], f32x16 o) {
#pragma unroll
    for (int e = 0; e < 16; ++e) {
        const float v = *(const float *)(vcol + (16 * half + e) * RSV);
        o = __builtin_amdgcn_mfma_f32_32x32x2f32(v, p[e], o, 0, 0, 0);
    }
    return o;
}

__device__ __forceinline__ void ld4(const float *s, float v[4]) { const f32x4 f = *(const f32x4 *)s; v[0] = f[0]; v[1] = f[1]; v[2] = f[2]; v[3] = f[3]; }
__device__ __forceinline__ void ld4(const bf16_t *s, float v[4]) {
    const u32x2 u = *(const u32x2 *)s;
    v[0] = bf2f((bf16_t)(u[0] & 0xffff)); v[1] = bf2f((bf16_t)(u[0] >> 16));
    v[2] = bf2f((bf16_t)(u[1] & 0xffff)); v[3] = bf2f((bf16_t)(u[1] >> 16));
}
__device__ __forceinline__ void st4(float *d, const float v[4]) { *(f32x4 *)d = (f32x4){v[0], v[1], v[2], v[3]}; }
__device__ __forceinline__ void st4(bf16_t *d, const float v[4]) {
    const bf16x4 b = {(__bf16)v[0], (__bf16)v[1], (__bf16)v[2], (__bf16)v[3]};
    *(u32x2 *)d = __builtin_bit_cast(u32x2, b);
}

__device__ __forceinline__ void unpack_chunk(float, const u32x4 &u, float (&v)[4]) {
    const f32x4 f = __builtin_bit_cast(f32x4, u);
    v[0] = f[0]; v[1] = f[1]; v[2] = f[2]; v[3] = f[3];
}
__device__ __forceinline__ void unpack_chunk(bf16_t, const u32x4 &u, float (&v)[8]) {
#pragma unroll
    for (int k = 0; k < 4; ++k) { v[2 * k] = bf2f((bf16_t)(u[k] & 0xffff)); v[2 * k + 1] = bf2f((bf16_t)(u[k] >> 16)); }
}
__device__ __forceinline__ void ldc(const float *s, float (&v)[4]) { const f32x4 f = *(const f32x4 *)s; v[0] = f[0]; v[1] = f[1]; v[2] = f[2]; v[3] = f[3]; }
__device__ __forceinline__ void ldc(const bf16_t *s, float (&v)[8]) {
    const u32x4 u = *(const u32x4 *)s;
#pragma unroll
    for (int k = 0; k < 4; ++k) { v[2 * k] = bf2f((bf16_t)(u[k] & 0xffff)); v[2 * k + 1] = bf2f((bf16_t)(u[k] >> 16)); }
}
__device__ __forceinline__ void stc(float *d, const float (&v)[4]) { *(f32x4 *)d = (f32x4){v[0], v[1], v[2], v[3]}; }
__device__ __forceinline__ void stc(bf16_t *d, const float (&v)[8]) {
    bf16x8 b;
#pragma unroll
    for (int k = 0; k < 8; ++k) b[k] = (__bf16)v[k];
    *(u32x4 *)d = __builtin_bit_cast(u32x4, b);
}

__device__ __forceinline__ void wait_vmcnt(int n) {
    switch (n) {
#define DA_VMCNT_CASE(k) case k: asm volatile("s_waitcnt vmcnt(" #k ")" ::: "memory"); break;
        DA_VMCNT_CASE(1) DA_VMCNT_CASE(2) DA_VMCNT_CASE(3) DA_VMCNT_CASE(4) DA_VMCNT_CASE(5) DA_VMCNT_CASE(6) DA_VMCNT_CASE(7) DA_VMCNT_CASE(8)
        DA_VMCNT_CASE(9) DA_VMCNT_CASE(10) DA_VMCNT_CASE(11) DA_VMCNT_CASE(12) DA_VMCNT_CASE(13) DA_VMCNT_CASE(14) DA_VMCNT_CASE(15) DA_VMCNT_CASE(16)
        DA_VMCNT_CASE(17) DA_VMCNT_CASE(18) DA_VMCNT_CASE(19) DA_VMCNT_CASE(20) DA_VMCNT_CASE(21) DA_VMCNT_CASE(22) DA_VMCNT_CASE(23) DA_VMCNT_CASE(24)
#undef DA_VMCNT_CASE
        default: asm volatile("s_waitcnt vmcnt(0)" ::: "memory"); break;
    }
}

__device__ __forceinline__ float pow2_floor_exp(float lq) { return (float)((int)((__builtin_bit_cast(unsigned, lq) >> 23) & 0xffu) - 127); }

template <typename T, typename CFG, int CO, int RSOF>
__device__ __forceinline__ void remainder_edges(const AttnDenseParams &p, float *so, int h, size_t np, int pad0, int n_g, int qtile0,
                                                int wid, int lane, bool wave_on, const int (&rm_beg)[4], const int (&rm_end)[4],
                                                const int (&rm_slot)[4]) {
    constexpr int NCK = CFG::ROWB / 16, MAXT = (NCK + 7) / 8, EPK = 16 / CFG::ES;
    constexpr int NCKV = CFG::ROWBV / 16, MAXTV = (NCKV + 7) / 8;
    const int sub = lane & 7;
    const float scale = p.sc * 0.6931471805599453f;
    auto load_row = [&](const void *base, size_t row, u32x4 (&dst)[MAXT]) {
#pragma unroll
        for (int t = 0; t < MAXT; ++t) {
            const int ck = sub + 8 * t;
            dst[t] = ck < NCK ? *(const u32x4 *)((const unsigned char *)base + row * CFG::ROWB + ck * 16) : (u32x4){0u, 0u, 0u, 0u};
        }
    };
    auto load_vrow = [&](size_t row, u32x4 (&dst)[MAXTV]) {
#pragma unroll
        for (int t = 0; t < MAXTV; ++t) {
            const int ck = sub + 8 * t;
            dst[t] = ck < NCKV ? *(const u32x4 *)((const unsigned char *)p.Vt + row * CFG::ROWBV + ck * 16) : (u32x4){0u, 0u, 0u, 0u};
        }
    };
    constexpr int RG = MAXT >= 3 ? 2 : 4;
    if (wave_on) {
#pragma unroll
      for (int r0 = 0; r0 < 4; r0 += RG) {
        u32x4 qr[4][MAXT], kr[4][MAXT], vr[4][MAXTV];
#pragma unroll
        for (int r = r0; r < r0 + RG; ++r) {
            const int qg = min(qtile0 + wid * 32 + (lane >> 3) + 8 * r, n_g - 1);
            load_row(p.Q, (size_t)h * np + pad0 + qg, qr[r]);
            load_row(p.K, (size_t)h * np + rm_slot[r], kr[r]);
            load_vrow((size_t)h * np + rm_slot[r], vr[r]);
        }
#pragma unroll
        for (int r = r0; r < r0 + RG; ++r) {
            if (rm_end[r] <= rm_beg[r]) continue;
            const int ql = wid * 32 + (lane >> 3) + 8 * r;
            float *orow = so + ql * RSOF;
            float mm = orow[CO], ll = orow[CO + 1];
            if (!(ll > 0.f)) { mm = -INFINITY; ll = 0.f; }
            float qv[MAXT][EPK], acc[MAXTV][EPK];
#pragma unroll
            for (int t = 0; t < MAXT; ++t) {
                unpack_chunk(T(), qr[r][t], qv[t]);
#pragma unroll
                for (int x = 0; x < EPK; ++x) qv[t][x] *= scale;
            }
#pragma unroll
            for (int t = 0; t < MAXTV; ++t)
#pragma unroll
                for (int x = 0; x < EPK; ++x) acc[t][x] = (sub + 8 * t < NCKV) ? orow[(sub + 8 * t) * EPK + x] : 0.f;
            for (int e = rm_beg[r]; e < rm_end[r]; ++e) {
                u32x4 k2[MAXT], v2[MAXTV];
                if (e > rm_beg[r]) {
// ... 60 lines not shown
```

### diffassemble_amd/csrc/da_attn_dense.hip

```cpp
#include <stdlib.h>

#include "da_attn_common.h"

namespace da {

#ifdef DA_ATTN_PROBE
#define DA_ATTN_DBG(...) __VA_ARGS__
#define DA_TICK(var) const unsigned long long var = __builtin_readcyclecounter()
#else
#define DA_ATTN_DBG(...)
#define DA_TICK(var)
#endif

__device__ unsigned long long g_attn_fallbacks[4];

template <typename T, int C, bool MASKED, int CV, int NST, int NW>
__global__ __launch_bounds__(64 * NW, (sizeof(T) == 4 && C == 144 && CV == 144) ? 1 : 2) void k_attn_dense(AttnDenseParams p) {
    using CF = Cfg<T, C, CV>;
    constexpr int QT = 32 * NW, NT = 64 * NW, MAXI = (CF::NI + NW - 1) / NW;
    extern __shared__ __attribute__((aligned(16))) unsigned char smem[];

    float *mlut = (float *)(smem + NST * CF::STAGE);
    if (MASKED && threadIdx.x < 64) {
        const int e = threadIdx.x >> 2, b = threadIdx.x & 3;
// ... 543 lines not shown
                        const float corr = __builtin_amdgcn_exp2f((m[sl] - mnew) * p.sc);
                        m[sl] = mnew;
                        l[sl] *= corr;
#pragma unroll
                        for (int r = 0; r < 16; ++r) O[sl][r] *= corr;
                        bsum = exp_block(m[sl] * p.sc);
                    }
                    l[sl] += bsum;
                    bf16x8 pf0, pf1;
#pragma unroll
                    for (int e = 0; e < 4; ++e) {
                        pf0[2 * e] = (__bf16)e2[e][0]; pf0[2 * e + 1] = (__bf16)e2[e][1];
                        pf1[2 * e] = (__bf16)e2[4 + e][0]; pf1[2 * e + 1] = (__bf16)e2[4 + e][1];
                    }
                    if (sl == 0) asm volatile("s_waitcnt lgkmcnt(0)" : "+v"(vlo[0]), "+v"(vhi[0]), "+v"(vlo[1]), "+v"(vhi[1]));
                    const u32x4 v0 = {vlo[0][0], vlo[0][1], vhi[0][0], vhi[0][1]};
                    const u32x4 v1 = {vlo[1][0], vlo[1][1], vhi[1][0], vhi[1][1]};
                    O[sl] = __builtin_amdgcn_mfma_f32_32x32x16_bf16(__builtin_bit_cast(bf16x8, v0), pf0, O[sl], 0, 0, 0);
                    O[sl] = __builtin_amdgcn_mfma_f32_32x32x16_bf16(__builtin_bit_cast(bf16x8, v1), pf1, O[sl], 0, 0, 0);
                    if (sl + 1 < NS) __builtin_amdgcn_sched_barrier(0);
                }
            }
        }
        dma_barrier();
        if (wave_on) {
#pragma unroll
            for (int sl = 0; sl < NS; ++sl) {
                const float lt = l[sl] + __shfl_xor(l[sl], 32);
                const float inv = lt > 0.f ? 1.0f / (lt + 1e-16f) : 0.f;
                float *orow = so + ((wid + 4 * sl) * 32 + i) * RSOF;
#pragma unroll
                for (int jj = 0; jj < 4; ++jj) {
                    const int c0 = 8 * jj + 4 * half;
                    *(f32x4 *)(orow + c0) = (f32x4){O[sl][4 * jj] * inv, O[sl][4 * jj + 1] * inv, O[sl][4 * jj + 2] * inv, O[sl][4 * jj + 3] * inv};
                }
            }
        }
    };
    if (two) run(SlabTag<2>());
    else run(SlabTag<1>());
    dma_barrier();

    constexpr int EPC = 8, CPR = C / EPC;
    const int nq = min(QT, n_g - qt * QT);
    constexpr int NB = 3;
    for (int it0 = tid; it0 < nq * CPR; it0 += 256 * NB) {
        u32x4 skv[NB], rsv[NB];
#pragma unroll
        for (int k = 0; k < NB; ++k) {
            const int it = it0 + 256 * k;
            if (it < nq * CPR) {
                const int q = it / CPR, ch = it - q * CPR;
                const size_t off = ((size_t)node0 + qt * QT + q) * HC + (size_t)h * C + ch * EPC;
                skv[k] = *(const u32x4 *)((const T *)p.S + off);
                if (p.res) rsv[k] = *(const u32x4 *)((const T *)p.res + off);
            }
        }
#pragma unroll
        for (int k = 0; k < NB; ++k) {
            const int it = it0 + 256 * k;
            if (it < nq * CPR) {
                const int q = it / CPR, ch = it - q * CPR;
                const size_t off = ((size_t)node0 + qt * QT + q) * HC + (size_t)h * C + ch * EPC;
                const float *src = so + q * RSOF + ch * EPC;
                float v[EPC], sk[EPC];
                const f32x4 a = *(const f32x4 *)src, b2 = *(const f32x4 *)(src + 4);
                v[0] = a[0]; v[1] = a[1]; v[2] = a[2]; v[3] = a[3]; v[4] = b2[0]; v[5] = b2[1]; v[6] = b2[2]; v[7] = b2[3];
                unpack_chunk(T(), skv[k], sk);
#pragma unroll
                for (int e = 0; e < EPC; ++e) v[e] += sk[e];
                if (p.res) {
                    unpack_chunk(T(), rsv[k], sk);
#pragma unroll
                    for (int e = 0; e < EPC; ++e) v[e] += sk[e];
                }
#pragma unroll
                for (int e = 0; e < EPC; ++e) v[e] = apply_act(v[e], p.act);
                stc((T *)p.out + off, v);
            }
        }
    }
}

#endif

static int attn_opt_last_env() { return DA_XENV("DA_ATTN_OPT_LAST", 1); }
static int attn_opt_masked_env() { return DA_XENV("DA_ATTN_OPT_MASKED", 1); }
static int attn_opt_env() { return cfg().attn_level >= 1; }
#ifdef DA_EXPERIMENTS
static int attn2_env() { return DA_XENV("DA_ATTN2", 0); }
static int launch_attn_dense2(AttnDenseParams p, int heads, int n_graphs, int max_graph_nodes, hipStream_t st) {
    using CF = Cfg<bf16_t, 32, 32>;
    p.nqt = (max_graph_nodes + 255) / 256;
    const int nblocks = p.nqt * heads * n_graphs;
    k_attn_dense2<<<nblocks, 256, 4 * CF::STAGE, st>>>(p);
    DA_LAUNCH_CHECK();
    return 0;
}
#endif

template <typename T, int C, bool MASKED, int CV, int NST, int NW>
static int launch_tcmn(AttnDenseParams p, hipStream_t st) {
    using CF = Cfg<T, C, CV>;
    int lds = NST * CF::STAGE + (MASKED ? 256 : 0);
    DA_ATTN_DBG({ lds += DA_XENV("DA_ATTN_LDS_PAD", 0); })
    static bool attr_done = false;
    if (!attr_done && lds > 48 * 1024) {
        DA_CHECK_HIP(hipFuncSetAttribute((const void *)k_attn_dense<T, C, MASKED, CV, NST, NW>, hipFuncAttributeMaxDynamicSharedMemorySize, lds));
        attr_done = true;
    }
    p.nqt = (p.max_nodes + 32 * NW - 1) / (32 * NW);
    k_attn_dense<T, C, MASKED, CV, NST, NW><<<p.nqt * p.H * p.n_graphs, 64 * NW, lds, st>>>(p);
    DA_LAUNCH_CHECK();
    return 0;
}
[[maybe_unused]] static int attn_nw(int) {
    const int env = DA_XENV("DA_ATTN_NW", 0);
    return (env == 5 || env == 8) ? env : 4;
}
[[maybe_unused]] static int attn_stages_env() { return DA_XENV("DA_ATTN_STAGES", 0); }
template <typename T, int C, bool MASKED, int CV>
static int launch_tcm(const AttnDenseParams &p, hipStream_t st) {
    if constexpr (C == 32) {
#ifdef DA_EXPERIMENTS
        if (attn_nw(p.max_nodes) == 5) return launch_tcmn<T, C, MASKED, CV, 4, 5>(p, st);
        if (attn_nw(p.max_nodes) == 8) return launch_tcmn<T, C, MASKED, CV, 4, 8>(p, st);
#endif
        return launch_tcmn<T, C, MASKED, CV, 4, 4>(p, st);
    } else if constexpr (sizeof(T) == 2 && CV == 32 && !MASKED) {
#ifdef DA_EXPERIMENTS
        if (attn_stages_env() == 3) return launch_tcmn<T, C, MASKED, CV, 3, 4>(p, st);
#endif
        return launch_tcmn<T, C, MASKED, CV, 2, 4>(p, st);
    } else {
        return launch_tcmn<T, C, MASKED, CV, 2, 4>(p, st);
    }
}
template <typename T, int C>
static int launch_tc(const AttnDenseParams &p, hipStream_t st) {
    return p.mask ? launch_tcm<T, C, true, C>(p, st) : launch_tcm<T, C, false, C>(p, st);
}

[[maybe_unused]] static int attn_dual_env() { return DA_XENV("DA_ATTN_DUAL", 0); }
int launch_attn_dense(int prec, const DenseLayout &L, int heads, int C, int n_graphs, int max_graph_nodes,
                      const int32_t *graph_ptr, const int32_t *pad_ptr, int nodiag, const void *res, int act,
                      void *out, hipStream_t st, const DenseMask *mk, const DenseFold *fold) {
    if (heads != 8 || (C != 32 && C != 144)) return -1;
    if ((size_t)C * (size_t)L.n_pad * esize(prec) >= ((size_t)1 << 31)) return -1;
    AttnDenseParams p;
    p.Q = L.Q; p.K = L.K; p.Vt = L.Vt; p.S = L.S; p.res = res; p.out = out;
    p.graph_ptr = graph_ptr; p.pad_ptr = pad_ptr; p.n_pad = L.n_pad; p.H = heads; p.n_graphs = n_graphs;
    p.nqt = 0; p.max_nodes = max_graph_nodes; p.act = act; p.nodiag = nodiag;
    p.x = L.x; p.ldx = L.ldx; p.kin = L.kin; p.wqs = L.wqs;
    p.bias_q = L.bias; p.bias_k = L.bias ? L.bias + heads * C : nullptr; p.bias_v = L.bias ? L.bias + 2 * heads * C : nullptr; p.bias_s = L.bias ? L.bias + 3 * heads * C : nullptr;
    p.fast = L.q_prescaled ? 1 : 0;
    if (DA_XENV("DA_ATTN_NO_FAST", 0)) p.fast = 0;
    p.sc = L.q_prescaled ? 1.0f : 1.4426950408889634f / sqrtf((float)C);
    p.mask = mk ? mk->mask : nullptr; p.mask_ptr = mk ? (const long long *)mk->mask_ptr : nullptr;
    p.irr_row_ptr = mk ? mk->irr_row_ptr : nullptr; p.irr_col_src = mk ? mk->irr_col_src : nullptr;
    p.row_map = mk ? mk->row_map : nullptr;
    p.slot_node = mk ? mk->slot_node : nullptr;
    p.blk_class = mk ? mk->blk_class : nullptr; p.blk_class_ptr = mk ? (const long long *)mk->blk_class_ptr : nullptr;
    p.blk_class_stride = mk ? mk->blk_class_stride : 0;
    p.rm_meta = mk ? mk->rm_meta : nullptr;
    const bool virt = mk && mk->v_rows > 0 && mk->v_row_ptr && mk->v_col_src && mk->v_part && mk->v_cnt && mk->v_taken && !fold && !res;
    p.v_rows = virt ? mk->v_rows : 0; p.v_split = 0; p.v_n_real = virt ? mk->v_n_real : 0;
    p.v_row_ptr = virt ? mk->v_row_ptr : nullptr; p.v_col_src = virt ? mk->v_col_src : nullptr; p.v_mult = virt ? mk->v_mult : nullptr;
    p.v_part = virt ? mk->v_part : nullptr; p.v_cnt = virt ? mk->v_cnt : nullptr;
    if (mk && mk->v_taken) *mk->v_taken = 0;
    { const char *e = DA_XENV_LIVE("DA_ATTN_DEBUG"); p.debug = e ? atoi(e) : 0; }
    if (p.x && DA_XENV("DA_QSF_FAKE_FM", 0)) p.debug = 77;
    { const int fg = DA_XENV("DA_ATTN_FORCE_GEN", 0) ? 1 : 0; p.force_gen = fg; if (fg) p.fast = p.fast ? 2 : 0; }
    { const char *e = DA_XENV_LIVE("DA_ATTN_PROF_PTR"); p.prof = e ? (unsigned long long *)strtoull(e, nullptr, 0) : nullptr; }
    if (n_graphs <= 0 || max_graph_nodes <= 0) return 0;
    p.fold_out = nullptr; p.n_rows = 0;
    if (fold) {
        if (C != 144 || fold->cv != 32) return -1;
        if (!DA_XENV("DA_ATTN_LAST_FAST", 1)) p.fast = 0;
        p.fold_out = fold->out; p.n_rows = fold->n_rows;
#ifdef DA_EXPERIMENTS
        if (!mk && prec == DA_PREC_BF16 && L.q_prescaled && attn_dual_env() DA_ATTN_DBG(&& !p.debug && !p.prof)) {
            const int r2 = launch_attn_dual(L, heads, C, n_graphs, max_graph_nodes, graph_ptr, pad_ptr, nodiag, act, out, fold, st);
            if (r2 >= 0) return r2;
        }
#endif
        if (prec == DA_PREC_BF16 && L.q_prescaled && p.fast && attn_opt_env() && attn_opt_last_env() && (!p.mask || attn_opt_masked_env())
            DA_ATTN_DBG(&& !p.debug && !p.prof)) {
            const int ro = launch_attn_opt(p, C, st);
            if (ro >= 0) return ro;
        }
        if (mk) return prec == DA_PREC_BF16 ? launch_tcm<bf16_t, 144, true, 32>(p, st) : launch_tcm<float, 144, true, 32>(p, st);
        return prec == DA_PREC_BF16 ? launch_tcm<bf16_t, 144, false, 32>(p, st) : launch_tcm<float, 144, false, 32>(p, st);
    }
    if (prec == DA_PREC_BF16 && C == 32 && L.q_prescaled && p.fast && attn_opt_env() && (!p.mask || attn_opt_masked_env()) DA_ATTN_DBG(&& !p.debug && !p.prof)) {
        const int ro = launch_attn_opt(p, C, st);
        if (ro == 0 && p.v_rows > 0 && attn_opt_took_virtual_rows()) *mk->v_taken = 1;
        if (ro >= 0) return ro;
    }
    p.v_rows = 0;
    DA_REQUIRE(!p.x, "launch_attn_dense: projection in the prologue requested for a layer the resident kernel does not take");
#ifdef DA_EXPERIMENTS
    if (prec == DA_PREC_BF16 && C == 32 && !p.mask && attn2_env() DA_ATTN_DBG(&& !p.debug && !p.prof))
        return launch_attn_dense2(p, heads, n_graphs, max_graph_nodes, st);
#endif
    if (prec == DA_PREC_BF16) return C == 32 ? launch_tc<bf16_t, 32>(p, st) : launch_tc<bf16_t, 144>(p, st);
    return C == 32 ? launch_tc<float, 32>(p, st) : launch_tc<float, 144>(p, st);
}

bool attn_res_qsf_shape_ok(int max_nodes, int n_pad, int n_graphs, int kin);
bool attn_qsf_applicable(int prec, int heads, int C, int kin, int n_graphs, int max_graph_nodes, int n_pad, int q_prescaled) {
    if (prec != DA_PREC_BF16 || heads != 8 || C != 32 || !q_prescaled || !attn_opt_env()) return false;
    if (DA_XENV("DA_ATTN_NO_FAST", 0) DA_ATTN_DBG(|| DA_XENV_LIVE("DA_ATTN_DEBUG") || DA_XENV_LIVE("DA_ATTN_PROF_PTR"))) return false;
    if ((size_t)C * (size_t)n_pad * 2 >= ((size_t)1 << 31)) return false;
    return attn_res_qsf_shape_ok(max_graph_nodes, n_pad, n_graphs, kin);
}
bool attn_qsf_enabled() {
    const int x = DA_XENV("DA_ATTN_RES_QSF", -1);
    return x < 0 ? !(cfg().disable_folds & DA_FOLD_ATTN_PROJ) : x != 0;
}

int attn_dense_counters(unsigned long long *out4, int reset) {
    DA_CHECK_HIP(hipMemcpyFromSymbol(out4, HIP_SYMBOL(g_attn_fallbacks), 4 * sizeof(unsigned long long)));
    if (reset) { const unsigned long long z[4] = {0, 0, 0, 0}; DA_CHECK_HIP(hipMemcpyToSymbol(HIP_SYMBOL(g_attn_fallbacks), z, sizeof(z))); }
    unsigned long long o2[2] = {0, 0};
    const int rc = attn_opt_counters(o2, reset);
    if (rc) return rc;
    out4[0] = o2[0];
    out4[2] = o2[1];
    return 0;
}

}
```

### diffassemble_amd/csrc/da_attn_opt.hip

```cpp
#include <stdlib.h>

#include <type_traits>

#include "da_attn_common.h"
#include "da_attn_res_asm.inc"

namespace da {

#ifdef DA_OPT_PROBE
#define DA_OPB(...) __VA_ARGS__
#else
#define DA_OPB(...)
#endif

__device__ unsigned long long g_opt_fallbacks[2];

__device__ __forceinline__ void virt_rows_block(const AttnDenseParams &p, int vb, unsigned char *smem) {
    constexpr int EPL = 4, U = 4, C = 32;
    const int row = vb / p.v_split, part = vb - row * p.v_split;
    const int i = p.v_n_real + row;
    const int beg = p.v_row_ptr[i], end = p.v_row_ptr[i + 1];
    const int lane = threadIdx.x & 63, wv = threadIdx.x >> 6;
    const int head = lane >> 3, sub = (lane & 7) * EPL;
    const size_t hb = (size_t)head * (size_t)p.n_pad;
// ... 706 lines not shown
}
static thread_local bool t_virt_taken = false;
bool attn_opt_took_virtual_rows() { return t_virt_taken; }

template <int C, bool FOLD, bool MASKED, int NST, int MINB, int BK = 64, int VAR = 0, int NWV = 4>
static int launch_optt(AttnDenseParams p, hipStream_t st) {
    const int lds = NST * (OptK<C, BK>::STAGE + (MASKED ? 1024 : 0)) + 64 + (MASKED ? 256 + 512 : 0);
    static bool attr_done[16] = {};
    int dev = 0;
    DA_CHECK_HIP(hipGetDevice(&dev));
    if (lds > 48 * 1024 && !attr_done[dev & 15]) {
        DA_CHECK_HIP(hipFuncSetAttribute((const void *)k_attn_optt<C, FOLD, MASKED, NST, MINB, BK, VAR, NWV>, hipFuncAttributeMaxDynamicSharedMemorySize, lds));
        attr_done[dev & 15] = true;
    }
    p.nqt = (p.max_nodes + 32 * NWV - 1) / (32 * NWV);
    DA_OPB({ const char *e = DA_XENV_LIVE("DA_OPT_PROF_PTR"); p.prof = e ? (unsigned long long *)strtoull(e, nullptr, 0) : nullptr; })
    int grid = p.nqt * p.H * p.n_graphs;
    t_virt_taken = false;
    if constexpr (C == 32 && !FOLD && MASKED && NWV == 4) {
        if (p.v_rows > 0) {
            p.v_split = p.v_n_real >= 8192 ? DA_VIRT_SPLIT_MAX : 4;
            grid += (p.v_rows * p.v_split + 7) & ~7;
            t_virt_taken = true;
            __atomic_fetch_add(&g_virt_launches, 1ll, __ATOMIC_RELAXED);
        }
    } else {
        p.v_rows = 0;
    }
    k_attn_optt<C, FOLD, MASKED, NST, MINB, BK, VAR, NWV><<<grid, 64 * NWV, lds, st>>>(p);
    DA_LAUNCH_CHECK();
    return 0;
}

template <int KS>
__host__ __device__ static inline int res_qsf_qs_off(int max_nodes) {
    const int img = ((max_nodes + 63) >> 6) * OptK<32, 64>::STAGE;
    return img >= 8 * OptK<32, 64>::STAGE + 2 * KS * 1024 ? img - 2 * KS * 1024 : img + 512 + 2 * KS * 1024 + 512;
}

template <int NWV, bool QUEUE, bool KPF, int XV = 0>
__global__ __launch_bounds__(64 * NWV, NWV >= 16 ? 1 : ((NWV > 5 || (XV & 8)) ? 4 : 5)) void k_attn_res(AttnDenseParams p) {
    constexpr bool O2 = (XV & 1) != 0, PROG = (XV & 16) != 0, MSK = (XV & 32) != 0, QSF = (XV & 64) != 0, PIPE2 = (XV & 256) != 0;
    static_assert(!PIPE2 || (NWV == 16 && KPF && !PROG && !MSK && !O2), "pipelined key loop: the sixteen-wave instances on complete graphs");
    static_assert(!QSF || (NWV == 16 && KPF && QUEUE && !PROG && !MSK && !O2), "projection in the prologue: the sixteen-wave default instance");
    static_assert(!MSK || (NWV == 16 && KPF && !PROG && !O2), "masked resident instance: sixteen waves, K fragments one block ahead");
    static_assert(!PROG || (NWV == 16 && KPF), "progressive landing: the sixteen-wave instance (two waves per piece index), K fragments one block ahead");
    using T = bf16_t;
    constexpr int C = 32, CV = 32;
    using CF = Cfg<T, C, CV, 64>;
    using KG = OptK<C, 64>;
    static_assert(KG::NI == 8, "eight 1 KB pieces per 64-key stage");
    static_assert(CF::ROWB == 64 && CF::ROWBV == 64 && KG::RS == 64 && CF::RSV == 64 && KG::KBYTES == 4096, "one tile stride for K and V; 2 KB per 32-key block");
    constexpr int TPW = NWV >= 8 ? NWV / 8 : 1;
    constexpr int STAGE = KG::STAGE;
    extern __shared__ __attribute__((aligned(16))) unsigned char smem[];
    DA_OPB(unsigned long long pb_[8] = {__builtin_readcyclecounter(), 0, 0, 0, 0, 0, 0, 0};)
    const int bid = (XV & 64) ? (int)(blockIdx.x & 7) * (int)(gridDim.x >> 3) + (int)(blockIdx.x >> 3) : (int)blockIdx.x;
    const int h = bid & 7, g = bid >> 3;
    const int npg = (p.max_nodes + 63) & ~63;
    const bool upad = (long long)p.n_pad == (long long)p.n_graphs * npg;
    const int pad0 = upad ? g * npg : p.pad_ptr[g];
    const int tid = threadIdx.x, lane = tid & 63, i = lane & 31, half = lane >> 5;
    const int wid = __builtin_amdgcn_readfirstlane(tid >> 6);
    const int HC = p.H * C;
    const size_t np = (size_t)p.n_pad;
    const unsigned char *Qg = (const unsigned char *)p.Q + ((size_t)h * np + pad0) * CF::ROWB;
    const unsigned char *Kg = (const unsigned char *)p.K + ((size_t)h * np + pad0) * CF::ROWB;
    const unsigned char *Vg = (const unsigned char *)p.Vt + ((size_t)h * np + pad0) * CF::ROWBV;
    const unsigned lds0 = (unsigned)(size_t)(__attribute__((address_space(3))) unsigned char *)smem;
    unsigned *qctr = (unsigned *)(smem + ((p.max_nodes + 63) >> 6) * STAGE);
    volatile unsigned *land = qctr + 4;
    float *mlut = (float *)(qctr + 36);
    if (MSK && tid < 64) mlut[tid] = (((tid >> 2) >> (tid & 3)) & 1) ? 0.f : -INFINITY;
    constexpr int KS = QSF ? ((XV & 128) ? 8 : 16) : 1;
    [[maybe_unused]] unsigned char *wimg = (unsigned char *)qctr + 512;
    [[maybe_unused]] float *biasl = (float *)(wimg + 2 * KS * 1024);
    if constexpr (QSF) {
        const unsigned char *wsrc = (const unsigned char *)p.wqs + (size_t)h * 4 * KS * 1024;
        const unsigned wl = lds0 + (unsigned)(wimg - smem);
        const int qs_off = res_qsf_qs_off<KS>(p.max_nodes);
        for (int j = wid; j < 4 * KS; j += NWV) {
            const int blk = j / KS, s_ = j - blk * KS;
            const unsigned dst = (blk == 1 || blk == 2) ? wl + (unsigned)(((blk - 1) * KS + s_) * 1024) : lds0 + (unsigned)(qs_off + ((blk ? 1 : 0) * KS + s_) * 1024);
            asm volatile("s_mov_b32 m0, %0\n\ts_nop 0\n\tglobal_load_lds_dwordx4 %1, %2" ::"s"(dst), "v"((unsigned)lane * 16u), "s"(wsrc + (size_t)j * 1024) : "memory");
        }
        if (tid < 128) biasl[tid] = (tid < 32 ? p.bias_q : (tid < 64 ? p.bias_k : (tid < 96 ? p.bias_v : p.bias_s)))[32 * h + (tid & 31)];
    }
    if (QUEUE && tid == 0) { *qctr = 0u; asm volatile("s_waitcnt lgkmcnt(0)" ::: "memory"); }
    if (PROG && tid < 32) { land[tid] = 0u; asm volatile("s_waitcnt lgkmcnt(0)" ::: "memory"); }
    int node0 = 0, n_g = 0;
    if (!upad) { node0 = p.graph_ptr[g]; n_g = p.graph_ptr[g + 1] - node0; }
    const int nkt = upad ? (npg >> 6) : ((n_g + 63) >> 6);
    u32x4 qf0[2] = {};
    if constexpr (PROG) {
        const unsigned char *qrow = Qg + (size_t)(wid * 32 + i) * CF::ROWB + half * 16;
        asm volatile("global_load_dwordx4 %0, %2, off\n\tglobal_load_dwordx4 %1, %2, off offset:32" : "=&v"(qf0[0]), "=&v"(qf0[1]) : "v"(qrow) : "memory");
    }

    if constexpr (QSF) {
    } else if constexpr (NWV % 8 != 0) {
        for (int idx = wid; idx < nkt * 8; idx += NWV) {
            const int kt = idx >> 3, pq = idx & 7;
            unsigned so_;
            if (pq < KG::NIK) {
                const int s = pq * 64 + lane, row = s / KG::KSPR, col = s - row * KG::KSPR;
                so_ = (unsigned)(row * CF::ROWB + (col ^ KG::f(row)) * 16);
            } else {
                const int s = (pq - KG::NIK) * 64 + lane, row = s / CF::VSPR, col = s - row * CF::VSPR;
                so_ = (unsigned)(row * CF::ROWBV + col * 16);
            }
            const unsigned long long sa = (unsigned long long)(size_t)((pq < KG::NIK ? Kg : Vg) + (size_t)kt * 64 * CF::ROWB);
            const unsigned long long su = (unsigned long long)(unsigned)__builtin_amdgcn_readfirstlane((int)(unsigned)sa) |
                                          ((unsigned long long)(unsigned)__builtin_amdgcn_readfirstlane((int)(unsigned)(sa >> 32)) << 32);
            const unsigned ml = (unsigned)__builtin_amdgcn_readfirstlane((int)(lds0 + (unsigned)(kt * STAGE + pq * 1024)));
            asm volatile("s_mov_b32 m0, %0\n\ts_nop 0\n\tglobal_load_lds_dwordx4 %1, %2" ::"s"(ml), "v"(so_), "s"((const unsigned char *)(size_t)su) : "memory");
        }
    } else {
        const int pq = wid & 7, t0 = wid >> 3;
        unsigned so_;
        if (pq < KG::NIK) {
            const int s = pq * 64 + lane, row = s / KG::KSPR, col = s - row * KG::KSPR;
            so_ = (unsigned)(row * CF::ROWB + (col ^ KG::f(row)) * 16);
        } else {
            const int s = (pq - KG::NIK) * 64 + lane, row = s / CF::VSPR, col = s - row * CF::VSPR;
            so_ = (unsigned)(row * CF::ROWBV + col * 16);
        }
        const unsigned char *src0 = pq < KG::NIK ? Kg : Vg;
        for (int kt = t0; kt < nkt; kt += TPW) {
            const unsigned char *src = src0 + (size_t)kt * 64 * CF::ROWB;
            asm volatile("s_mov_b32 m0, %0\n\ts_nop 0\n\tglobal_load_lds_dwordx4 %1, %2" ::"s"(lds0 + (unsigned)(kt * STAGE + pq * 1024)), "v"(so_), "s"(src)
                         : "memory");
        }
    }
    DA_OPB(pb_[1] = __builtin_readcyclecounter();)
    if (upad) {
        if constexpr (PROG) {
            typedef __attribute__((ext_vector_type(2))) int i32x2_;
            i32x2_ gp2;
            const int32_t *gpp = p.graph_ptr + g;
            asm volatile("s_load_dwordx2 %0, %1, 0x0\n\ts_waitcnt lgkmcnt(0)" : "=s"(gp2) : "s"(gpp) : "memory");
            node0 = gp2[0]; n_g = gp2[1] - gp2[0];
        } else { node0 = p.graph_ptr[g]; n_g = p.graph_ptr[g + 1] - node0; }
    }
    const int nslab = (n_g + 31) >> 5;
    int slab = wid;
    u32x4 qf[CF::NCH];
    auto load_q = [&](int sl, u32x4(&dst)[CF::NCH]) {
        const unsigned char *qrow = Qg + (size_t)(max(min(sl, nslab - 1), 0) * 32 + i) * CF::ROWB;
#pragma unroll
        for (int ch = 0; ch < CF::NCH; ++ch) dst[ch] = *(const u32x4 *)(qrow + ch * 32 + half * 16);
    };
    static_assert(!PROG || CF::NCH == 2, "progressive landing: two Q fragments per lane");
    [[maybe_unused]] u32x4 xq[KS];
    [[maybe_unused]] const int xstep = p.debug == 77 ? 1024 : 32;
    [[maybe_unused]] auto x_row = [&](int sl) {
        const int nd = max(min(sl * 32 + i, n_g - 1), 0);
        const unsigned char *row = (const unsigned char *)p.x + ((size_t)(node0 + nd) * (size_t)p.ldx + 8 * half) * 2;
        if (p.debug == 77) row = (const unsigned char *)p.x + ((size_t)(node0 + max(min(sl * 32, n_g - 32), 0)) * (size_t)p.ldx) * 2 + lane * 16;
        return row;
    };
    [[maybe_unused]] auto x_issue = [&](int sl) {
        const unsigned char *row = x_row(sl);
#pragma unroll
        for (int s_ = 0; s_ < KS; ++s_) xq[s_] = *(const u32x4 *)(row + s_ * xstep);
    };
    struct Reload { enum { value = 1 }; };
    struct NoReload { enum { value = 0 }; };
    typedef const __attribute__((address_space(1))) u32x4 *xptr_t;
    [[maybe_unused]] auto chain1 = [&](auto rl, const unsigned char *wb, f32x16 &a, const unsigned char *nxt = nullptr) {
        unsigned lo = (unsigned)lane * 16u;
        asm volatile("" : "+v"(lo));
#pragma unroll
        for (int r = 0; r < 16; ++r) a[r] = 0.f;
        u32x4 wa = *(const u32x4 *)(wb + lo);
#pragma unroll
        for (int s_ = 0; s_ < KS; ++s_) {
            u32x4 wn = wa;
            if (s_ + 1 < KS) wn = *(const u32x4 *)(wb + (size_t)(s_ + 1) * 1024 + lo);
            __builtin_amdgcn_sched_barrier(0);
            a = __builtin_amdgcn_mfma_f32_32x32x16_bf16(__builtin_bit_cast(bf16x8, wa), __builtin_bit_cast(bf16x8, xq[s_]), a, 0, 0, 0);
            __builtin_amdgcn_sched_barrier(0);
            if constexpr (decltype(rl)::value) {
                asm volatile("" : "+v"(nxt));
                xq[s_] = *(xptr_t)(size_t)nxt;
                nxt += xstep;
            }
            wa = wn;
        }
    };
    [[maybe_unused]] auto chunk_of = [&](const f32x16 &a, int blk, int t) {
        const f32x4 b0 = *(const f32x4 *)(biasl + 32 * blk + 16 * t + 8 * half), b1 = *(const f32x4 *)(biasl + 32 * blk + 16 * t + 8 * half + 4);
        bf16x8 q8;
#pragma unroll
        for (int e = 0; e < 4; ++e) { q8[e] = (__bf16)(a[8 * t + e] + b0[e]); q8[4 + e] = (__bf16)(a[8 * t + 4 + e] + b1[e]); }
        return __builtin_bit_cast(u32x4, q8);
    };
    [[maybe_unused]] auto project_qs = [&](int sl, bool keep) {
        const unsigned char *wq_ = smem + (size_t)res_qsf_qs_off<KS>(p.max_nodes);
        const int row = sl * 32 + i;
        f32x16 a;
        chain1(NoReload(), wq_, a);
#pragma unroll
        for (int t = 0; t < 2; ++t) {
            const u32x4 qc = chunk_of(a, 0, t);
            if (keep) qf[t] = qc;
            if (row < n_g) *(u32x4 *)(const_cast<unsigned char *>(Qg) + (size_t)row * CF::ROWB + (2 * t + half) * 16) = qc;
        }
        chain1(NoReload(), wq_ + (size_t)KS * 1024, a);
#pragma unroll
        for (int t = 0; t < 2; ++t) {
            const u32x4 sc_ = chunk_of(a, 3, t);
            if (row < n_g) *(u32x4 *)((unsigned char *)p.S + ((size_t)(node0 + row) * HC + (size_t)h * C) * 2 + (2 * t + half) * 16) = sc_;
        }
    };
    [[maybe_unused]] auto project_kv = [&](auto rl, int sl, const unsigned char *nxt = nullptr) {
        const int rt = (sl & 1) * 32 + i;
        unsigned char *st_ = smem + (size_t)(sl >> 1) * STAGE + (size_t)rt * 64;
        f32x16 a;
        chain1(NoReload(), wimg, a);
#pragma unroll
        for (int t = 0; t < 2; ++t) *(u32x4 *)(st_ + (((2 * t + half) ^ KG::f(rt)) << 4)) = chunk_of(a, 1, t);
        chain1(rl, wimg + (size_t)KS * 1024, a, nxt);
#pragma unroll
        for (int t = 0; t < 2; ++t) *(u32x4 *)(st_ + KG::KBYTES + ((2 * t + half) << 4)) = chunk_of(a, 2, t);
    };
    if constexpr (QSF) { if (slab < nslab) x_issue(slab); }
    else if constexpr (!PROG) load_q(slab, qf);
    [[maybe_unused]] const int t0p = wid >> 3, nmine = nkt > t0p ? (nkt - t0p + 1) >> 1 : 0;
    [[maybe_unused]] int posted = 0;
    [[maybe_unused]] auto wait_le = [&](int n) {
        switch (n) {
            case 0: asm volatile("s_waitcnt vmcnt(0)" ::: "memory"); break;
            case 1: asm volatile("s_waitcnt vmcnt(1)" ::: "memory"); break;
            case 2: asm volatile("s_waitcnt vmcnt(2)" ::: "memory"); break;
            case 3: asm volatile("s_waitcnt vmcnt(3)" ::: "memory"); break;
            case 4: asm volatile("s_waitcnt vmcnt(4)" ::: "memory"); break;
            case 5: asm volatile("s_waitcnt vmcnt(5)" ::: "memory"); break;
            case 6: asm volatile("s_waitcnt vmcnt(6)" ::: "memory"); break;
            case 7: asm volatile("s_waitcnt vmcnt(7)" ::: "memory"); break;
            case 8: asm volatile("s_waitcnt vmcnt(8)" ::: "memory"); break;
            default: asm volatile("s_waitcnt vmcnt(9)" ::: "memory"); break;
        }
    };
    [[maybe_unused]] auto post_upto = [&](int tmax) {
        while (posted < nmine && t0p + 2 * posted <= tmax) {
            wait_le(nmine - 1 - posted);
            if (lane == 0) __hip_atomic_fetch_add((unsigned *)land + t0p + 2 * posted, 1u, __ATOMIC_RELAXED, __HIP_MEMORY_SCOPE_WORKGROUP);
            ++posted;
        }
    };
    [[maybe_unused]] auto await_tile = [&](int t) {
        const unsigned a_ = (unsigned)(size_t)(__attribute__((address_space(3))) unsigned *)(land + t);
        unsigned v_;
        do {
            asm volatile("ds_read_b32 %0, %1\n\ts_waitcnt lgkmcnt(0)" : "=v"(v_) : "v"(a_) : "memory");
            if (__builtin_amdgcn_readfirstlane((int)v_) >= 8) break;
            __builtin_amdgcn_s_sleep(1);
        } while (true);
    };
    if constexpr (PROG) {
        __builtin_amdgcn_s_barrier();
        post_upto(slab < nslab ? 1 : (1 << 30));
        if (nmine == 0) asm volatile("s_waitcnt vmcnt(0)" ::: "memory");
        qf[0] = qf0[0]; qf[1] = qf0[1];
        asm volatile("" : "+v"(qf[0]), "+v"(qf[1]));
        if (slab < nslab) await_tile(0);
    } else {
    if constexpr (QSF) {
        const int slabB = slab + NWV;
        const bool hasA = slab < nslab, hasB = slabB < nslab;
        asm volatile("s_waitcnt vmcnt(0) lgkmcnt(0)" ::: "memory");
        __builtin_amdgcn_s_barrier();
        if (hasA) {
            project_qs(slab, true);
            if (hasB) { project_kv(Reload(), slab, x_row(slabB)); project_qs(slabB, false); }
            else project_kv(NoReload(), slab);
        }
        __builtin_amdgcn_s_barrier();
        if (hasB) project_kv(NoReload(), slabB);
        asm volatile("s_waitcnt vmcnt(0) lgkmcnt(0)" ::: "memory");
        __builtin_amdgcn_s_barrier();
    } else {
    asm volatile("s_waitcnt vmcnt(0)" : "+v"(qf[0]), "+v"(qf[CF::NCH - 1]));
    __builtin_amdgcn_s_barrier();
    }
    }
    DA_OPB(pb_[6] = __builtin_readcyclecounter();)

    const int pi_i = (i & 3) + 4 * ((i >> 3) & 3) + 16 * ((i >> 2) & 1);
    int kfo[CF::NCH];
#pragma unroll
    for (int ch = 0; ch < CF::NCH; ++ch) kfo[ch] = pi_i * KG::RS + (((2 * ch + half) ^ KG::f(pi_i)) * 16);
    const int li = lane & 15;
    const unsigned vbase = lds0 + (unsigned)(KG::KBYTES + (16 * half + (li >> 2)) * CF::RSV + (16 * ((lane >> 4) & 1) + 4 * (li & 3)) * 2);

    typedef __attribute__((ext_vector_type(2))) __bf16 bf16x2;
    const bf16x2 one2 = {(__bf16)1.0f, (__bf16)1.0f};
    f32x16 O, Ob;
    float ls, m;
    if (XV & 2) { if (wid >= NWV / 2) __builtin_amdgcn_s_setprio(1); }
    auto boff = [&](int b) { return (b >> 1) * STAGE + (b & 1) * 2048; };

    for (int round = 0; slab < nslab; ++round) {
        const int q0 = slab * 32, qidx = q0 + i;
        bool gen = p.force_gen != 0;
        auto pass = [&](const bool first) {
#pragma unroll
            for (int r = 0; r < 16; ++r) { O[r] = 0.f; if (O2) Ob[r] = 0.f; }
            ls = 0.f;
            m = -1e30f;
            u32x4 kf[CF::NCH];
#pragma unroll
            for (int ch = 0; ch < CF::NCH; ++ch) kf[ch] = *(const u32x4 *)(smem + kfo[ch]);
            int b_first = 0;
            [[maybe_unused]] f32x16 sA;
            if constexpr (PIPE2) {
                static_assert(!PIPE2 || CF::NCH == 2, "two K fragments per block");
                const int nfull = n_g >> 5;
                if (!gen && !p.nodiag && nfull >= 3) {
#pragma unroll
                    for (int r = 0; r < 16; ++r) sA[r] = 0.f;
#pragma unroll
                    for (int ch = 0; ch < CF::NCH; ++ch) sA = mma_chunk(T(), kf[ch], qf[ch], sA);
                    u32x4 kfA0 = *(const u32x4 *)(smem + boff(1) + kfo[0]), kfA1 = *(const u32x4 *)(smem + boff(1) + kfo[1]);
                    const unsigned ones = 0x3f803f80u;
                    asm volatile("s_nop 7\n\ts_nop 7" : "+v"(sA), "+v"(kfA0), "+v"(kfA1));
                    int b = 0;
                    for (; b + 1 < nfull && b + 3 < nslab; b += 2) {
                        const unsigned kad0 = lds0 + (unsigned)(boff(b + 2) + kfo[0]), kad1 = lds0 + (unsigned)(boff(b + 2) + kfo[1]);
                        const unsigned vad = vbase + (unsigned)boff(b);
                        constexpr int ABL = (XV >> 9) & 7;
                        if constexpr (ABL == 1) DA_RES_PAIR_NOWAIT();
                        else if constexpr (ABL == 2) DA_RES_PAIR_NOVALU();
                        else if constexpr (ABL == 3) DA_RES_PAIR_NOMFMA();
                        else if constexpr (ABL == 4) DA_RES_PAIR_NOREAD();
                        else if constexpr (ABL == 5) DA_RES_PAIR_HALFEXP();
                        else DA_RES_PAIR();
                    }
                    asm volatile("s_waitcnt lgkmcnt(0)\n\ts_nop 7\n\ts_nop 7" : "+v"(sA), "+v"(kfA0), "+v"(kfA1), "+v"(O), "+v"(ls));
                    kf[0] = kfA0; kf[1] = kfA1;
                    b_first = b;
                }
            }
            for (int b = b_first; b < nslab; ++b) {
                const int key0 = b * 32;
                const int bo = boff(b);
                const bool given = PIPE2 && b_first > 0 && b == b_first;
                if (PROG && first && !(b & 1)) post_upto(3 * (b >> 1) + 1);
                if (!KPF && b > 0) {
#pragma unroll
                    for (int ch = 0; ch < CF::NCH; ++ch) kf[ch] = *(const u32x4 *)(smem + bo + kfo[ch]);
                }
                __builtin_amdgcn_sched_barrier(0);
                f32x16 s;
                if (given) {
                    if constexpr (PIPE2) s = sA;
                } else {
#pragma unroll
                for (int r = 0; r < 16; ++r) s[r] = 0.f;
#pragma unroll
                for (int ch = 0; ch < CF::NCH; ++ch) s = mma_chunk(T(), kf[ch], qf[ch], s);
                }
                asm volatile("" : "+v"(s));
                u32x2 vlo[2], vhi[2];
                const unsigned vb = vbase + (unsigned)bo;
#pragma unroll
                for (int mm = 0; mm < 2; ++mm) {
                    vlo[mm] = tr_read(vb, (8 * mm) * CF::RSV);
                    vhi[mm] = tr_read(vb, (8 * mm + 4) * CF::RSV);
                }
                if (KPF && b + 1 < nslab && !given) {
                    if (PROG && first && (b & 1)) await_tile((b + 1) >> 1);
                    const int bn = boff(b + 1);
#pragma unroll
                    for (int ch = 0; ch < CF::NCH; ++ch) kf[ch] = *(const u32x4 *)(smem + bn + kfo[ch]);
                }
                {
// ... 86 lines not shown
                    const unsigned mw = mw_n;
                    anym |= mw;
                    __builtin_amdgcn_sched_barrier(0);
                    f32x16 s;
                    if (full) {
#pragma unroll
                        for (int r = 0; r < 16; ++r) s[r] = 0.f;
                    } else {
#pragma unroll
                        for (int j = 0; j < 4; ++j) {
                            const f32x4 b4 = *(const f32x4 *)((const unsigned char *)mlut + (((mw >> (4 * j)) & 15u) << 4));
                            s[4 * j] = b4[0]; s[4 * j + 1] = b4[1]; s[4 * j + 2] = b4[2]; s[4 * j + 3] = b4[3];
                        }
                    }
#pragma unroll
                    for (int ch = 0; ch < CF::NCH; ++ch) s = mma_chunk(T(), kf[ch], qf[ch], s);
                    asm volatile("" : "+v"(s));
                    u32x2 vlo[2], vhi[2];
                    const unsigned vb = vbase + (unsigned)bo;
#pragma unroll
                    for (int mm = 0; mm < 2; ++mm) {
                        vlo[mm] = tr_read(vb, (8 * mm) * CF::RSV);
                        vhi[mm] = tr_read(vb, (8 * mm + 4) * CF::RSV);
                    }
                    const bool last = rem == 0ull;
                    int bn = b;
                    if (!last) {
                        bn = __builtin_ctzll(rem);
                        rem &= rem - 1ull;
                        const int bon = boff(bn);
#pragma unroll
                        for (int ch = 0; ch < CF::NCH; ++ch) kf[ch] = *(const u32x4 *)(smem + bon + kfo[ch]);
                        mw_n = ((fullm >> bn) & 1ull) ? 0xffffu : *(const unsigned short *)(mrow2 + 4 * bn);
                    }
                    if (gen) {
                        const float a0 = fmaxf(fmaxf(s[0], s[1]), s[2]), a1 = fmaxf(fmaxf(s[3], s[4]), s[5]);
                        const float a2 = fmaxf(fmaxf(s[6], s[7]), s[8]), a3 = fmaxf(fmaxf(s[9], s[10]), s[11]);
                        const float a4 = fmaxf(fmaxf(s[12], s[13]), s[14]);
                        const float mloc = fmaxf(fmaxf(fmaxf(a0, a1), a2), fmaxf(fmaxf(a3, a4), s[15]));
                        const float mnew = fmaxf(m, fmaxf(mloc, __shfl_xor(mloc, 32)));
                        if (__any(mnew > m)) {
                            const float corr = __builtin_amdgcn_exp2f(m - mnew);
#pragma unroll
                            for (int r = 0; r < 16; ++r) O[r] *= corr;
                            ls *= corr;
                            m = mnew;
                        }
#pragma unroll
                        for (int r = 0; r < 16; ++r) s[r] -= m;
                    }
                    bf16x8 pf0, pf1;
#pragma unroll
                    for (int e = 0; e < 4; ++e) {
                        const float x0 = __builtin_amdgcn_exp2f(s[2 * e]), x1 = __builtin_amdgcn_exp2f(s[2 * e + 1]);
                        const float y0 = __builtin_amdgcn_exp2f(s[8 + 2 * e]), y1 = __builtin_amdgcn_exp2f(s[8 + 2 * e + 1]);
                        pf0[2 * e] = (__bf16)x0; pf0[2 * e + 1] = (__bf16)x1;
                        pf1[2 * e] = (__bf16)y0; pf1[2 * e + 1] = (__bf16)y1;
                        __builtin_amdgcn_sched_barrier(0);
                    }
                    asm volatile("s_waitcnt lgkmcnt(0)" : "+v"(vlo[0]), "+v"(vhi[0]), "+v"(vlo[1]), "+v"(vhi[1]));
                    const u32x4 v0 = {vlo[0][0], vlo[0][1], vhi[0][0], vhi[0][1]};
                    const u32x4 v1 = {vlo[1][0], vlo[1][1], vhi[1][0], vhi[1][1]};
                    O = __builtin_amdgcn_mfma_f32_32x32x16_bf16(__builtin_bit_cast(bf16x8, v0), pf0, O, 0, 0, 0);
                    O = __builtin_amdgcn_mfma_f32_32x32x16_bf16(__builtin_bit_cast(bf16x8, v1), pf1, O, 0, 0, 0);
#pragma unroll
                    for (int e = 0; e < 4; ++e) {
                        const bf16x2 pa = {pf0[2 * e], pf0[2 * e + 1]}, pb = {pf1[2 * e], pf1[2 * e + 1]};
                        ls = __builtin_amdgcn_fdot2_f32_bf16(pa, one2, ls, false);
                        ls = __builtin_amdgcn_fdot2_f32_bf16(pb, one2, ls, false);
                    }
                    if (last) break;
                    b = bn;
                }
            }
            int nrem = rend - rbeg;
#pragma unroll
            for (int o_ = 32; o_ > 0; o_ >>= 1) nrem = max(nrem, __shfl_xor(nrem, o_));
            nrem = __builtin_amdgcn_readfirstlane(nrem);
            for (int k = 0; k < nrem; ++k) {
                const bool on = rbeg + k < rend;
                size_t sj = (size_t)h * np + (size_t)(k == 0 ? rslot : p.row_map[p.irr_col_src[on ? rbeg + k : max(rbeg, 0)]]);
                const unsigned char *kr = (const unsigned char *)p.K + sj * CF::ROWB, *vr = (const unsigned char *)p.Vt + sj * CF::ROWBV;
                float sc_ = 0.f;
#pragma unroll
                for (int ch = 0; ch < CF::NCH; ++ch) {
                    const u32x4 kk = *(const u32x4 *)(kr + ch * 32 + half * 16);
#pragma unroll
                    for (int w_ = 0; w_ < 4; ++w_) {
                        sc_ = fmaf(bf2f((bf16_t)(qf[ch][w_] & 0xffff)), bf2f((bf16_t)(kk[w_] & 0xffff)), sc_);
                        sc_ = fmaf(bf2f((bf16_t)(qf[ch][w_] >> 16)), bf2f((bf16_t)(kk[w_] >> 16)), sc_);
                    }
                }
                sc_ += __shfl_xor(sc_, 32);
                u32x2 vv[4];
#pragma unroll
                for (int jj = 0; jj < 4; ++jj) vv[jj] = *(const u32x2 *)(vr + (8 * jj + 4 * half) * 2);
                if (gen) {
                    const float mnew = on ? fmaxf(m, sc_) : m;
                    if (mnew > m) {
                        const float corr = __builtin_amdgcn_exp2f(m - mnew);
#pragma unroll
                        for (int r = 0; r < 16; ++r) O[r] *= corr;
                        ls *= corr;
                        m = mnew;
                    }
                    sc_ -= m;
                }
                const float pe = on ? __builtin_amdgcn_exp2f(sc_) : 0.f;
                anym |= on ? 1u : 0u;
                if (half == 0) ls += pe;
#pragma unroll
                for (int jj = 0; jj < 4; ++jj) {
                    O[4 * jj] = fmaf(pe, bf2f((bf16_t)(vv[jj][0] & 0xffff)), O[4 * jj]);
                    O[4 * jj + 1] = fmaf(pe, bf2f((bf16_t)(vv[jj][0] >> 16)), O[4 * jj + 1]);
                    O[4 * jj + 2] = fmaf(pe, bf2f((bf16_t)(vv[jj][1] & 0xffff)), O[4 * jj + 2]);
                    O[4 * jj + 3] = fmaf(pe, bf2f((bf16_t)(vv[jj][1] >> 16)), O[4 * jj + 3]);
                }
            }
        };
        if constexpr (MSK) pass_masked(); else
        pass(PROG && round == 0);
        if (PROG && round == 0) post_upto(1 << 30);
        if (O2) {
#pragma unroll
            for (int r = 0; r < 16; ++r) O[r] += Ob[r];
        }
        DA_OPB({ asm volatile("" : "+v"(O), "+v"(ls)); if (round < 2) pb_[2 + 2 * round] = __builtin_readcyclecounter(); })
        if (!gen) {
            const float lt0 = ls + __shfl_xor(ls, 32);
            bool ok = lt0 > 8.673617379884035e-19f && lt0 < 1.2676506002282294e30f;
            if (MSK) ok = ok || (lt0 == 0.f && (anym | (unsigned)__shfl_xor((int)anym, 32)) == 0u);
            if (__any(!ok && qidx < n_g)) {
                gen = true;
                if (lane == 0) atomicAdd(&g_opt_fallbacks[MSK ? 1 : 0], 1ull);
                if constexpr (MSK) pass_masked(); else
                pass(false);
                if (O2) {
#pragma unroll
                    for (int r = 0; r < 16; ++r) O[r] += Ob[r];
                }
            }
        }
        int nxt = slab + NWV;
        if (QUEUE) {
            unsigned t_ = 0;
            if (lane == 0) t_ = __hip_atomic_fetch_add(qctr, 1u, __ATOMIC_RELAXED, __HIP_MEMORY_SCOPE_WORKGROUP);
            nxt = NWV + __builtin_amdgcn_readfirstlane((int)t_);
        }
        [[maybe_unused]] u32x4 qn[CF::NCH];
        const bool more = nxt < nslab;
        if (more) load_q(nxt, qn);
        const float lt = ls + __shfl_xor(ls, 32);
        const float inv = lt > 0.f ? 1.0f / (lt + (gen ? 1e-16f : 0.f)) : 0.f;
        if (qidx < n_g) {
            const size_t roff = (size_t)(MSK ? my_node : node0 + qidx) * HC + (size_t)h * C + 4 * half;
            u32x2 sk[4], rs[4];
#pragma unroll
            for (int jj = 0; jj < 4; ++jj) {
                sk[jj] = *(const u32x2 *)((const T *)p.S + roff + 8 * jj);
                rs[jj] = p.res ? *(const u32x2 *)((const T *)p.res + roff + 8 * jj) : (u32x2){0u, 0u};
            }
#pragma unroll
            for (int jj = 0; jj < 4; ++jj) {
                float v4[4] = {__fmul_rn(O[4 * jj], inv), __fmul_rn(O[4 * jj + 1], inv), __fmul_rn(O[4 * jj + 2], inv), __fmul_rn(O[4 * jj + 3], inv)};
                v4[0] += bf2f((bf16_t)(sk[jj][0] & 0xffff)); v4[1] += bf2f((bf16_t)(sk[jj][0] >> 16));
                v4[2] += bf2f((bf16_t)(sk[jj][1] & 0xffff)); v4[3] += bf2f((bf16_t)(sk[jj][1] >> 16));
                if (p.res) {
                    v4[0] += bf2f((bf16_t)(rs[jj][0] & 0xffff)); v4[1] += bf2f((bf16_t)(rs[jj][0] >> 16));
                    v4[2] += bf2f((bf16_t)(rs[jj][1] & 0xffff)); v4[3] += bf2f((bf16_t)(rs[jj][1] >> 16));
                }
#pragma unroll
                for (int e = 0; e < 4; ++e) v4[e] = apply_act(v4[e], p.act);
                st4((T *)p.out + roff + 8 * jj, v4);
            }
        }
        if (more) {
#pragma unroll
            for (int ch = 0; ch < CF::NCH; ++ch) qf[ch] = qn[ch];
            asm volatile("" : "+v"(qf[0]), "+v"(qf[CF::NCH - 1]));
        }
        slab = nxt;
        DA_OPB({ if (round < 2) pb_[3 + 2 * round] = __builtin_readcyclecounter(); })
    }
    DA_OPB({ if (p.prof && lane == 0) { pb_[7] = __builtin_readcyclecounter(); unsigned long long *o_ = p.prof + ((size_t)blockIdx.x * NWV + wid) * 8;
             for (int k = 0; k < 8; ++k) o_[k] = pb_[k]; } })
}

static long long g_res_launches = 0;
long long attn_res_launches(int reset) {
    return reset ? __atomic_exchange_n(&g_res_launches, 0ll, __ATOMIC_RELAXED) : __atomic_load_n(&g_res_launches, __ATOMIC_RELAXED);
}
static long long g_res_qsf_launches = 0;
long long attn_res_qsf_launches(int reset) {
    return reset ? __atomic_exchange_n(&g_res_qsf_launches, 0ll, __ATOMIC_RELAXED) : __atomic_load_n(&g_res_qsf_launches, __ATOMIC_RELAXED);
}

static size_t attn_res_qsf_lds(int max_nodes, int kin) {
    const size_t img = (size_t)((max_nodes + 63) >> 6) * OptK<32, 64>::STAGE, wb = (size_t)2 * (kin >> 4) * 1024, base = img + 512 + wb + 512;
    const size_t qs = (size_t)(kin == 128 ? res_qsf_qs_off<8>(max_nodes) : res_qsf_qs_off<16>(max_nodes));
    return qs >= img ? qs + wb : base;
}
static bool attn_res_takes(int max_nodes, int n_pad, int n_graphs) {
    return cfg().attn_level >= 2 && DA_XENV("DA_OPT_HID", 0) == 0 && max_nodes >= DA_XENV("DA_ATTN_RES_MIN", 512) && max_nodes <= 19 * 64 &&
           (long long)n_pad * 2 >= (long long)n_graphs * max_nodes;
}
bool attn_res_qsf_shape_ok(int max_nodes, int n_pad, int n_graphs, int kin) {
    if (kin != 128 && kin != 256) return false;
    if (DA_XENV("DA_ATTN_RES_PH", 1) != 1 || DA_XENV("DA_ATTN_RES_PIPE", 0) != 0) return false;
    return attn_res_takes(max_nodes, n_pad, n_graphs) && attn_res_qsf_lds(max_nodes, kin) <= (size_t)160 * 1024;
}

__global__ void k_pack_w_qs(int heads, int kin, int hc, const bf16_t *__restrict__ W, u32x4 *__restrict__ out) {
    const int KS = kin >> 4;
    const size_t idx = (size_t)blockIdx.x * blockDim.x + threadIdx.x, total = (size_t)heads * 4 * KS * 64;
    if (idx >= total) return;
    const int lane = (int)(idx & 63), s = (int)((idx >> 6) % KS), hm = (int)((idx >> 6) / KS), m = hm & 3, h = hm >> 2;
    const int a = lane & 31, row = (a & 0x13) | (((a >> 2) & 1) << 3) | (((a >> 3) & 1) << 2);
    out[idx] = *(const u32x4 *)(W + ((size_t)m * hc + 32 * h + row) * kin + 16 * s + 8 * (lane >> 5));
}
size_t w_qs_bytes(int heads, int kin) { return (size_t)heads * 4 * kin * 64; }
int pack_w_qs(int heads, int kin, int hc, const void *wd, void *packed, hipStream_t st) {
    const size_t total = w_qs_bytes(heads, kin) / 16;
    k_pack_w_qs<<<(unsigned)((total + 255) / 256), 256, 0, st>>>(heads, kin, hc, (const bf16_t *)wd, (u32x4 *)packed);
    DA_LAUNCH_CHECK();
    return 0;
}

template <int NWV, bool QUEUE, bool KPF, int XV = 0>
static int launch_res(const AttnDenseParams &p, hipStream_t st) {
    int lds = ((p.max_nodes + 63) >> 6) * OptK<32, 64>::STAGE + 16 + 128 + 256;
    if (XV & 64) lds = (int)attn_res_qsf_lds(p.max_nodes, (XV & 128) ? 128 : 256);
    static bool attr_done[16] = {};
    int dev = 0;
    DA_CHECK_HIP(hipGetDevice(&dev));
    if (!attr_done[dev & 15]) {
        DA_CHECK_HIP(hipFuncSetAttribute((const void *)k_attn_res<NWV, QUEUE, KPF, XV>, hipFuncAttributeMaxDynamicSharedMemorySize, 160 * 1024));
        attr_done[dev & 15] = true;
    }
    AttnDenseParams q = p;
    DA_OPB({ const char *e = DA_XENV_LIVE("DA_OPT_PROF_PTR"); q.prof = e ? (unsigned long long *)strtoull(e, nullptr, 0) : nullptr; })
    k_attn_res<NWV, QUEUE, KPF, XV><<<p.H * p.n_graphs, 64 * NWV, lds, st>>>(q);
    DA_LAUNCH_CHECK();
    __atomic_fetch_add(&g_res_launches, 1ll, __ATOMIC_RELAXED);
    return 0;
}

int launch_attn_opt(const AttnDenseParams &p, int C, hipStream_t st) {
    const bool fold = p.fold_out != nullptr, masked = p.mask != nullptr;
    t_virt_taken = false;
    if (masked && p.max_nodes > 4096) return -1;
    if (masked && p.blk_class && p.blk_class_stride > 128) return -1;
    if (C == 32 && !fold) {
        if (masked) {
#ifdef DA_EXPERIMENTS
            if (DA_XENV("DA_OPT_MASKED_VAR", 0) == 30) return launch_optt<32, false, true, 4, 4, 64, 256>(p, st);
#endif
#ifdef DA_EXPERIMENTS
            if (cfg().attn_level >= 2 && DA_XENV("DA_ATTN_RES_MASKED", 0) && p.max_nodes >= 512 && p.max_nodes <= 19 * 64 - 64 &&
                (long long)p.n_pad * 2 >= (long long)p.n_graphs * p.max_nodes)
                return launch_res<16, true, true, 32>(p, st);
#endif
            return launch_optt<32, false, true, 4, 4>(p, st);
        }
        [[maybe_unused]] const int v = DA_XENV("DA_OPT_HID", 0);
        {
            const int res = cfg().attn_level >= 2, res_min = DA_XENV("DA_ATTN_RES_MIN", 512);
#ifdef DA_EXPERIMENTS
            const int res_small = DA_XENV("DA_ATTN_RES_SMALL", 0);
            if (res && res_small && v == 0 && p.max_nodes > 128 && p.max_nodes <= 160 && (long long)p.n_pad * 2 >= (long long)p.n_graphs * p.max_nodes)
                return res_small == 2 ? launch_res<5, false, true, 8>(p, st)
                                      : launch_res<5, false, true>(p, st);
#endif
            if (res && v == 0 && p.max_nodes >= res_min && p.max_nodes <= 19 * 64  && (long long)p.n_pad * 2 >= (long long)p.n_graphs * p.max_nodes) {
                if (p.x) {
                    DA_REQUIRE(attn_res_qsf_shape_ok(p.max_nodes, p.n_pad, p.n_graphs, p.kin) && p.wqs && p.bias_q && p.bias_k && p.bias_v && p.bias_s,
                               "k_attn_res: projection in the prologue requested for a shape it does not take");
                    __atomic_fetch_add(&g_res_qsf_launches, 1ll, __ATOMIC_RELAXED);
                    return p.kin == 256 ? launch_res<16, true, true, 64>(p, st) : launch_res<16, true, true, 64 + 128>(p, st);
                }
#ifdef DA_EXPERIMENTS
                switch (DA_XENV("DA_ATTN_RES_PH", 1)) {
                    case 3: return launch_res<16, false, true>(p, st);
                    case 4: return launch_res<16, true, false>(p, st);
                    case 5: return launch_res<16, true, true, 1>(p, st);
                    case 6: return launch_res<16, true, true, 2>(p, st);
                    case 7: return launch_res<16, true, true, 3>(p, st);
                    case 8: return launch_res<16, true, true, 16>(p, st);
                    default: break;
                }
#endif
#ifdef DA_EXPERIMENTS
                switch (DA_XENV("DA_ATTN_RES_PIPE", 0)) {
                    case 1: return launch_res<16, true, true, 256>(p, st);
                    case 2: return launch_res<16, true, true, 256 + 512 * 1>(p, st);
                    case 3: return launch_res<16, true, true, 256 + 512 * 2>(p, st);
                    case 4: return launch_res<16, true, true, 256 + 512 * 3>(p, st);
                    case 5: return launch_res<16, true, true, 256 + 512 * 4>(p, st);
                    case 6: return launch_res<16, true, true, 256 + 512 * 5>(p, st);
                    default: break;
                }
#endif
                return launch_res<16, true, true>(p, st);
            }
        }
#ifdef DA_EXPERIMENTS
        switch (v) {
            case 1: return launch_optt<32, false, false, 4, 4, 64, 1>(p, st);
            case 2: return launch_optt<32, false, false, 4, 4, 64, 2>(p, st);
            case 3: return launch_optt<32, false, false, 6, 4, 32, 0>(p, st);
            case 10: return launch_optt<32, false, false, 4, 4, 64, 64>(p, st);
            case 11: return launch_optt<32, false, false, 5, 4, 64, 64>(p, st);
            case 12: return launch_optt<32, false, false, 6, 4, 32, 64>(p, st);
            case 20: return launch_optt<32, false, false, 4, 4, 64, 128>(p, st);
            case 30: return launch_optt<32, false, false, 4, 4, 64, 256>(p, st);
            case 40: return launch_optt<32, false, false, 3, 5, 64, 0>(p, st);
            case 50: return launch_optt<32, false, false, 4, 4, 64, 512>(p, st);
            case 60: return launch_optt<32, false, false, 4, 4, 64, 1024>(p, st);
            case 70: return launch_optt<32, false, false, 4, 4, 64, 0, 5>(p, st);
#ifdef DA_ATTN_ABLATE
            case 201: return launch_optt<32, false, false, 4, 4, 64, 2048>(p, st);
            case 202: return launch_optt<32, false, false, 4, 4, 64, 4096>(p, st);
            case 104: return launch_optt<32, false, false, 4, 4, 64, 4>(p, st);
            case 108: return launch_optt<32, false, false, 4, 4, 64, 8>(p, st);
            case 116: return launch_optt<32, false, false, 4, 4, 64, 16>(p, st);
            case 132: return launch_optt<32, false, false, 4, 4, 64, 32>(p, st);
            case 160: return launch_optt<32, false, false, 4, 4, 64, 60>(p, st);
#endif
            default: break;
        }
#endif
        return launch_optt<32, false, false, 4, 4>(p, st);
    }
    if (C == 144 && fold) {
        if (masked) {
#ifdef DA_EXPERIMENTS
            if (DA_XENV("DA_OPT_MASKED_VAR", 0) == 30) return launch_optt<144, true, true, 2, 3, 64, 256>(p, st);
#endif
            return launch_optt<144, true, true, 2, 3>(p, st);
        }
#ifdef DA_EXPERIMENTS
        switch (DA_XENV("DA_OPT_LAST", 0)) {
            case 1: return launch_optt<144, true, false, 4, 3, 32, 0>(p, st);
            case 2: return launch_optt<144, true, false, 3, 3, 32, 0>(p, st);
            case 3: return launch_optt<144, true, false, 3, 4, 32, 0>(p, st);
            case 4: return launch_optt<144, true, false, 2, 3, 64, 1>(p, st);
            case 5: return launch_optt<144, true, false, 4, 3, 32, 1>(p, st);
            case 6: return launch_optt<144, true, false, 2, 3, 64, 2>(p, st);
            case 7: return launch_optt<144, true, false, 4, 3, 32, 2>(p, st);
            case 10: return launch_optt<144, true, false, 4, 3, 32, 64>(p, st);
            case 11: return launch_optt<144, true, false, 3, 2, 64, 64>(p, st);
            case 12: return launch_optt<144, true, false, 3, 3, 32, 64>(p, st);
            case 30: return launch_optt<144, true, false, 2, 3, 64, 256>(p, st);
            case 60: return launch_optt<144, true, false, 2, 3, 64, 1024>(p, st);
            case 70: return launch_optt<144, true, false, 2, 3, 64, 0, 5>(p, st);
#ifdef DA_ATTN_ABLATE
            case 201: return launch_optt<144, true, false, 2, 3, 64, 2048>(p, st);
            case 202: return launch_optt<144, true, false, 2, 3, 64, 4096>(p, st);
            case 104: return launch_optt<144, true, false, 2, 3, 64, 4>(p, st);
            case 108: return launch_optt<144, true, false, 2, 3, 64, 8>(p, st);
            case 116: return launch_optt<144, true, false, 2, 3, 64, 16>(p, st);
            case 132: return launch_optt<144, true, false, 2, 3, 64, 32>(p, st);
            case 124: return launch_optt<144, true, false, 2, 3, 64, 24>(p, st);
            case 128: return launch_optt<144, true, false, 2, 3, 64, 28>(p, st);
            case 160: return launch_optt<144, true, false, 2, 3, 64, 60>(p, st);
#endif
            default: break;
        }
#endif
        return launch_optt<144, true, false, 2, 3>(p, st);
    }
    return -1;
}

int attn_opt_counters(unsigned long long *out2, int reset) {
    DA_CHECK_HIP(hipMemcpyFromSymbol(out2, HIP_SYMBOL(g_opt_fallbacks), 2 * sizeof(unsigned long long)));
    if (reset) { const unsigned long long z[2] = {0, 0}; DA_CHECK_HIP(hipMemcpyToSymbol(HIP_SYMBOL(g_opt_fallbacks), z, sizeof(z))); }
    return 0;
}

}
```

### diffassemble_amd/csrc/da_config.h

```cpp
#pragma once
#include <stdlib.h>

#include "../../include/diffassemble_hip.h"

namespace da {

da_config &cfg();

enum { DA_FOLD_MLP2 = 1, DA_FOLD_LAST = 2, DA_FOLD_QSCALE = 4, DA_FOLD_DDIM = 8, DA_FOLD_TAIL = 16, DA_FOLD_HYBRID_OVERLAP = 32, DA_FOLD_ATTN_PROJ = 64 };

#ifdef DA_EXPERIMENTS
inline int xenv_read(const char *name, int dflt) { const char *e = getenv(name); return e ? atoi(e) : dflt; }
#define DA_XENV(name, dflt) ([]() -> int { static const int v_ = da::xenv_read(name, dflt); return v_; }())
#define DA_XENV_LIVE(name) getenv(name)
#define DA_XENV_SET(name) (getenv(name) != nullptr)
#else
#define DA_XENV(name, dflt) (dflt)
#define DA_XENV_LIVE(name) ((const char *)nullptr)
#define DA_XENV_SET(name) (false)
#endif

}
```

### diffassemble_amd/csrc/da_internal.h

```cpp
#pragma once
#include "da_common.h"
#include "da_config.h"

namespace da {

struct DeviceSchedule {
    int steps;
    const float *betas, *alphas_cumprod, *sqrt_recip_alphas, *sqrt_recip_alphas_cumprod,
        *sqrt_recipm1_alphas_cumprod, *sqrt_one_minus_alphas_cumprod, *posterior_variance;
};

__device__ __forceinline__ float ddim2d_value(const DeviceSchedule &s, int mean_type, long long ti, int ratio,
                                              int prev_all_nonneg, float eta, float xv, float m, float noise) {
    ti = ti < 0 ? 0 : (ti >= s.steps ? s.steps - 1 : ti);
    const long long tp = ti - ratio;
    const float ap = s.alphas_cumprod[ti];
    const float ap_prev = (prev_all_nonneg && tp >= 0) ? s.alphas_cumprod[tp] : 1.0f;
    const float beta = 1.0f - ap;
    const float x0 = mean_type == DA_MEAN_START_X ? m : (xv - sqrtf(beta) * m) / sqrtf(ap);
    const float eps = (s.sqrt_recip_alphas_cumprod[ti] * xv - x0) / s.sqrt_recipm1_alphas_cumprod[ti];
    const float var = ((1.0f - ap_prev) / (1.0f - ap)) * (1.0f - ap / ap_prev);
    const float std_eta = eta * sqrtf(var);
    float prev = sqrtf(ap_prev) * x0 + sqrtf(1.0f - ap_prev - std_eta * std_eta) * eps;
    if (eta > 0.f) prev += std_eta * noise;
    return prev;
}

struct DdimFuse {
    DeviceSchedule s;
    int mean_type, ratio, prev_all_nonneg;
    long long t;
    const float *x;
    float *x_prev;
    int done;
    int nx_on, nx_done, nx_steps, nx_cin, nx_ldw;
    long long nx_t;
    const float *nx_time_emb, *nx_w0, *nx_b0, *nx_w1, *nx_b1;
    const void *nx_wp;
    const void *nx_feat_proj;
    void *nx_h;
};

int launch_set_feats(int prec, int n, int F, int D, const float *feats, void *comb_in, hipStream_t st);
int launch_set_virtual_rows(int prec, int rows, int V, int D, const void *emb, void *dst, hipStream_t st);
struct VirtScatter {
    int rows = 0, V = 0, H = 0, C = 0, n_real = 0, n_pad = 0;
    const void *src = nullptr;
    const int32_t *row_map = nullptr;
    void *Q = nullptr, *K = nullptr, *Vt = nullptr, *S = nullptr;
};
int launch_embed_pos_time(int prec, int n, int c_in, int F, int D, const float *x, const int64_t *t, int64_t t_scalar,
                          int steps, const float *time_emb, const float *w0, const float *b0, const float *w1,
                          const float *b1, void *comb_in, hipStream_t st, const VirtScatter *vs = nullptr);
int launch_gemm_simple(int prec, int M, int K, int Nout, const void *A, int lda, const void *W, const float *bias,
                       int act, const void *res, void *out, int ldo, hipStream_t st);
int launch_head2d(int prec, int n, int c_out, const void *hh, const float *w2, const float *b2, float *out, hipStream_t st);
int launch_ddim2d(const DeviceSchedule &s, int mean_type, int n, int c, const float *x, const float *mo,
                  const int64_t *t, int64_t t_scalar, int ratio, int prev_all_nonneg, float eta, const float *noise,
                  float *x_prev, hipStream_t st);
int launch_ddpm2d(const DeviceSchedule &s, int n, int c, const float *x, const float *mo, const int64_t *t,
                  int64_t t_scalar, const float *noise, float *x_prev, hipStream_t st);
int launch_convert(int prec, size_t n, const float *src, void *dst, hipStream_t st);
int launch_transpose_f32(int rows, int cols, const float *src, float *dst, hipStream_t st);
int launch_gemm_tn(int M, int N, int K, const float *A, int lda, const float *B, int ldb, float *C, int ldc, float *partial,
                   hipStream_t st, bool bfc = false);
int launch_gemm_tn_bf16(int M, int N, int K, const bf16_t *A, int lda, const bf16_t *B, int ldb, float *C, int ldc, float *partial,
                        hipStream_t st);
int launch_gemm_mfma_splitk(int M, int K, int Nout, const void *A, int lda, const void *W, const float *bias, const void *res,
                            void *out, int ldo, float *partial, size_t partial_floats, hipStream_t st, bool in16 = false,
                            const float *gelu_pre = nullptr, float *act_out = nullptr);
int launch_gemm_mfma_mixed(bool in16, bool out16, int M, int K, int Nout, const void *A, int lda, const void *W, const float *bias,
                           const void *res, void *out, int ldo, hipStream_t st);
int launch_gemm_tn_db(int M, int N, int K, const void *A, int lda, const void *B, int ldb, float *C, int ldc, float *partial,
                      float *db, float *bscratch, hipStream_t st, bool a16 = false, bool b16 = false);
int colsum_add(int M, int N, const float *A, int lda, float *out, float *scratch, hipStream_t st);
int launch_conv(int prec, int B, const void *X, int Cin, int Hi, const void *W, const float *bias, const void *res, void *Y,
                int Cout, int ksize, int stride, int relu, hipStream_t st);
int launch_enc_stem(int prec, int B, const float *patches, const float *w, const float *bias, void *Y, int relu, hipStream_t st);
int launch_mm_nn_f32(int M, int N, int K, const float *A, int lda, const float *B, int ldb, const float *bias, float *C,
                     int ldc, hipStream_t st);
int launch_scatter_virtual(int prec, int rows, int V, int H, int C, const void *src, int n_real, const int32_t *row_map,
                           int n_pad, void *Q, void *K, void *Vt, void *S, void *qkvs, hipStream_t st);
int launch_tail_fused(int prec, int n, int H, int c_out, int hidden, int din, const void *h, const void *xin, int ldx, const void *wh,
                      const float *bh, const void *wsk, const float *bsk, const void *pz, const float *w2, const float *b2, float *out,
                      hipStream_t st, DdimFuse *dfp);
int launch_head_fold(int prec, int n, int H, int c_out, const void *pz, const void *pre, const float *w2, const float *b2,
                     float *out, hipStream_t st, const DdimFuse *df = nullptr);

int launch_attn_tiny(int prec, int n_graphs, int max_graph_nodes, const int32_t *graph_ptr, int nodiag, int heads, int C, const void *qkvs,
                     const void *residual, int act, void *out, hipStream_t st);
int launch_attn_csr(int prec, int n_nodes, const int32_t *row_ptr, const int32_t *col_src, const int32_t *edge_id,
                    int heads, int C, const void *qkvs, const void *residual, int act, void *out, float *alpha,
                    float *stats , hipStream_t st);

int launch_head3d(int prec, int n, const void *hh, const float *wt, const float *bt, const float *wr, const float *br,
                  float *out7, float *pre_head, hipStream_t st);
int launch_head3d_bwd(int n, const float *pre, const float *d_out, float *d_pre, hipStream_t st);
int launch_ddim3d(const DeviceSchedule &s, int mean_type, int n, const float *x, const float *mo, const int64_t *t,
                  int64_t t_scalar, int ratio, int prev_all_nonneg, float *x_prev, hipStream_t st);

struct StreamJoin {
    hipStream_t side = nullptr, caller = nullptr;
    hipEvent_t ev = nullptr;
    bool armed = false;
    void arm(hipStream_t side_, hipStream_t caller_, hipEvent_t ev_) { side = side_; caller = caller_; ev = ev_; armed = true; }
    hipError_t join() {
        if (!armed) return hipSuccess;
        armed = false;
        hipError_t e = hipEventRecord(ev, side);
        return e == hipSuccess ? hipStreamWaitEvent(caller, ev, 0) : e;
    }
    ~StreamJoin() { (void)join(); }
};
struct QkvScatter {
    int HC, C, n_pad;
    int Cv = 0;
    int blocks = 0;
    const int32_t *row_map;
    void *Q, *K, *Vt, *S;
};
struct DenseLayout {
    const void *Q, *K, *Vt, *S;
    int n_pad;
    int q_prescaled = 0;
    const void *x = nullptr;
    int ldx = 0, kin = 0;
    const void *wqs = nullptr;
    const float *bias = nullptr;
};
bool attn_qsf_applicable(int prec, int heads, int C, int kin, int n_graphs, int max_graph_nodes, int n_pad, int q_prescaled);
bool attn_qsf_enabled();
size_t w_qs_bytes(int heads, int kin);
int pack_w_qs(int heads, int kin, int hc, const void *wd, void *packed, hipStream_t st);
int launch_gemm_mfma(int prec, int M, int K, int Nout, const void *A, int lda, const void *W, const float *bias,
                     int act, const void *res, void *out, int ldo, const QkvScatter *qs, hipStream_t st, int ldw = 0,
                     const void *pre = nullptr, const void *wpacked = nullptr);
size_t xpanel_packed_bytes(int K, int Nout);
bool xpanel_in_model();
void gemm_thin_set(int v);
int xpanel_mode();
int pack_w_xpanel(int K, int Nout, const void *W, int ldw, void *packed, hipStream_t st);
struct DenseMask {
    const uint8_t *mask;
    const int64_t *mask_ptr;
    const int32_t *irr_row_ptr, *irr_col_src, *row_map;
    const int32_t *slot_node = nullptr;
    const uint8_t *blk_class = nullptr;
    const int64_t *blk_class_ptr = nullptr;
    int blk_class_stride = 0;
    const int32_t *rm_meta = nullptr;
    int v_rows = 0, v_n_real = 0;
    const int32_t *v_row_ptr = nullptr, *v_col_src = nullptr;
    const float *v_mult = nullptr;
    float *v_part = nullptr;
    unsigned *v_cnt = nullptr;
    int *v_taken = nullptr;
};
constexpr int DA_VIRT_SPLIT_MAX = 8;
inline DenseMask dense_mask_of(const da_graph *g) {
    DenseMask mk;
    mk.mask = g->mask; mk.mask_ptr = g->mask_ptr; mk.irr_row_ptr = g->irr_row_ptr; mk.irr_col_src = g->irr_col_src; mk.row_map = g->row_map;
    mk.slot_node = g->slot_node;
    mk.rm_meta = g->rm_meta;
    const bool cls = g->blk_class && g->blk_class_ptr && g->blk_class_stride > 0;
    mk.blk_class = cls ? g->blk_class : nullptr; mk.blk_class_ptr = cls ? g->blk_class_ptr : nullptr; mk.blk_class_stride = cls ? g->blk_class_stride : 0;
    return mk;
}
struct DenseFold {
    int cv;
    void *out;
    int n_rows;
};
int launch_attn_dense(int prec, const DenseLayout &L, int heads, int C, int n_graphs, int max_graph_nodes,
                      const int32_t *graph_ptr, const int32_t *pad_ptr, int nodiag, const void *res, int act,
                      void *out, hipStream_t st, const DenseMask *mk = nullptr, const DenseFold *fold = nullptr);
int launch_attn_dual(const DenseLayout &L, int heads, int C, int n_graphs, int max_graph_nodes, const int32_t *graph_ptr,
                     const int32_t *pad_ptr, int nodiag, int act, void *out, const DenseFold *fold, hipStream_t st);
int attn_dense_counters(unsigned long long *out4, int reset);
long long attn_virt_launches(int reset);
long long attn_res_launches(int reset);
long long attn_res_qsf_launches(int reset);
int attn_dual_counters(unsigned long long *out2, int reset);
int launch_attn_csr_cont(int prec, int n_nodes, int n_real, const int32_t *irr_row_ptr, const int32_t *irr_col_src,
                         const int32_t *row_map, int heads, int C, int n_pad, const DenseLayout &L,
                         const void *residual, int act, void *out, hipStream_t st,
                         const float *mult = nullptr );

bool conv_fused_applicable(int prec, int heads, int C, int kin, int max_graph_nodes, int ldo);
int launch_conv_fused(int prec, int heads, int C, int kin, int n_graphs, int max_graph_nodes, const int32_t *graph_ptr,
                      int nodiag, const void *x, int ldx, const void *W, const float *bias, int act, void *out, int ldo,
                      hipStream_t st);

int pcd_knn_launch(int clouds, int N, int dim, const float *x, int ldx, int32_t *idx, const float *xn, hipStream_t st);
int pcd_premap_launch(int C, const float *X, int ldx, const float *Wm, long long total, float *T, hipStream_t st);
int pcd_edge_launch(const float *T, const int32_t *idx, const float *bn_a, const float *wb, int N, int clouds, float *Xout,
                    float *xn, hipStream_t st);
int pcd_conv6_final_launch(const float *X1, const float *X2, const float *X3, const float *w6, int feat, int N, int clouds,
                           float *partial, const float *lin0, int inv, float *out, int ldo, hipStream_t st);

int gcn_plan_kind(const da_graph *g);
int launch_gcn_dinv(const da_graph *g, float *dinv, hipStream_t st);
int launch_gcn_aggregate(int prec, const da_graph *g, int W, const float *dinv, const void *X, const float *bias, int act, void *out,
                         hipStream_t st);
int launch_gcn_aggregate_t(int prec, const da_graph *g, int W, const float *dinv, const void *X, void *out, hipStream_t st);
int launch_gcn_gelu_res(size_t n, const float *pre, const float *res, float *out, hipStream_t st);

struct D3pmStep {
    DeviceSchedule s = {};
    const int32_t *x_t = nullptr;
    const int64_t *t = nullptr;
    int64_t t_scalar = 0;
    int ratio = 1;
    const float *noise = nullptr;
    const uint64_t *seed = nullptr;
    int iteration = 0;
    int32_t *x_prev = nullptr;
    float *post = nullptr;
};
int launch_embed_idx_time(int prec, int n, int K, int F, int D, const int32_t *idx, const int64_t *t, int64_t t_scalar, int steps,
                          const float *time_emb, const float *pos_emb, void *comb_in, hipStream_t st);
struct D3pmRows {
    const void *hh = nullptr, *pz = nullptr, *pre = nullptr;
};
constexpr uint32_t D3PM_WORD_SAMPLING = 0xD3B07384u, D3PM_WORD_TRAINING = 0x51ED270Bu;
constexpr uint32_t D3PM_WORD_SAMPLING_ROT = 0x2A65C0F1u;
inline uint32_t d3pm_domain_word(int domain) {
    return domain == DA_D3PM_DRAW_TRAINING ? D3PM_WORD_TRAINING : domain == DA_D3PM_DRAW_SAMPLING_ROT ? D3PM_WORD_SAMPLING_ROT : D3PM_WORD_SAMPLING;
}
__device__ __forceinline__ float philox_uniform(uint64_t seed, uint64_t ctr, uint32_t iteration, uint32_t word = D3PM_WORD_SAMPLING) {
    uint32_t c0 = (uint32_t)ctr, c1 = (uint32_t)(ctr >> 32), c2 = iteration, c3 = word;
    uint32_t k0 = (uint32_t)seed, k1 = (uint32_t)(seed >> 32);
#pragma unroll
    for (int i = 0; i < 10; ++i) {
        const uint32_t hi0 = __umulhi(0xD2511F53u, c0), lo0 = 0xD2511F53u * c0;
        const uint32_t hi1 = __umulhi(0xCD9E8D57u, c2), lo1 = 0xCD9E8D57u * c2;
        c0 = hi1 ^ c1 ^ k0; c1 = lo1; c2 = hi0 ^ c3 ^ k1; c3 = lo0;
        k0 += 0x9E3779B9u; k1 += 0xBB67AE85u;
    }
    return (float)((c0 >> 8) + 1u) * 5.9604644775390625e-8f;
}
int launch_embed_idx_grad(int n, int K, int D, int F, const int32_t *idx, const float *dcomb, float *grad, hipStream_t st);
int launch_d3pm_tail(int prec, int n, int K, int H, const D3pmRows *rows_c, const D3pmRows *rows_u, float cfg_w, const float *w2,
                     const float *b2, const float *logits_in, float *logits_out, const D3pmStep *step, hipStream_t st);

int launch_embed_idx_time_rot(int prec, int n, int K, int F, int D, int hidden, const int32_t *idx, const int32_t *rot_acc, const int64_t *t,
                              int64_t t_scalar, int steps, const float *time_emb, const float *pos_emb, void *comb_in, const void *proj4,
                              size_t img_stride, void *sel, hipStream_t st);
struct D3pmRotStep {
    DeviceSchedule s = {};
    const int32_t *x_t = nullptr, *rot_t = nullptr;
    const int64_t *t = nullptr;
    int64_t t_scalar = 0;
    int ratio = 1;
    const float *noise_x = nullptr, *noise_rot = nullptr;
    const uint64_t *seed = nullptr;
    int iteration = 0;
    int32_t *x_prev = nullptr, *rot_0 = nullptr, *rot_prev = nullptr;
    float *post_x = nullptr, *post_rot = nullptr;
    int cold = 0, need_prev = 1;
    const int32_t *rot_acc_in = nullptr;
    int32_t *rot_next = nullptr, *rot_acc_out = nullptr;
};
int launch_d3pm_rot_tail(int prec, int n, int K, const void *hh, const float *w2, const float *b2, const float *wr, const float *br,
                         const float *logits_in, const float *rot_logits_in, float *logits_out, float *rot_logits_out,
                         const D3pmRotStep *step, hipStream_t st);

int linear(int prec, int M, int K, int Nout, const void *A, int lda, const void *W, const float *bias, int act,
           const void *res, void *out, int ldo, hipStream_t st);

}
```

### include/diffassemble_hip.h

```cpp
#ifndef DIFFASSEMBLE_HIP_H
#define DIFFASSEMBLE_HIP_H

#include <stddef.h>
#include <stdint.h>

#ifdef __cplusplus
extern "C" {
#endif

#define DA_ABI_VERSION 19

enum { DA_PREC_F32 = 0, DA_PREC_BF16 = 1 };
enum { DA_VARIANT_2D = 0, DA_VARIANT_3D = 1,
       DA_VARIANT_DISCRETE = 2,
       DA_VARIANT_DISCRETE_ROT = 3 };
enum { DA_ARCH_TRANSFORMER = 0, DA_ARCH_EXOPHORMER = 1,
       DA_ARCH_GCN = 2 };
enum { DA_MEAN_EPSILON = 0, DA_MEAN_START_X = 1 };
enum { DA_ACT_NONE = 0, DA_ACT_GELU = 1, DA_ACT_LEAKY02 = 2 };
enum { DA_MAX_LAYERS = 8 };

int da_abi_version(void);
const char *da_last_error(void);

// ... 80 lines not shown

int da_denoiser_flags(const da_denoiser *d);

size_t da_denoiser_workspace_bytes(const da_denoiser *d, const da_graph *g);

int da_denoiser_set_features(da_denoiser *d, const da_graph *g, const float *feats,
                             void *workspace, size_t workspace_bytes, void *stream);

int da_denoiser_forward(da_denoiser *d, const da_graph *g, const float *x, const int64_t *t,
                        int64_t t_scalar, float *out, float *alpha, int alpha_all_layers,
                        float *pre_head, void *workspace, size_t workspace_bytes, void *stream);

int da_gcn_dinv(const da_graph *g, float *dinv, void *stream);
int da_gcn_aggregate(int prec, const da_graph *g, int W, const float *dinv, const void *X, const float *bias, int act,
                     void *out, void *stream);

typedef struct da_schedule {
    int32_t steps;
    const float *betas;
    const float *alphas_cumprod;
    const float *sqrt_recip_alphas;
    const float *sqrt_recip_alphas_cumprod;
    const float *sqrt_recipm1_alphas_cumprod;
    const float *sqrt_one_minus_alphas_cumprod;
    const float *posterior_variance;
} da_schedule;

int da_ddim_step(const da_schedule *s, int variant, int mean_type, int n, int c, const float *x,
                 const float *model_out, const int64_t *t, int64_t t_scalar, int inference_ratio,
                 int prev_all_nonneg, float eta, const float *noise, float *x_prev, void *stream);

int da_ddpm_step(const da_schedule *s, int n, int c, const float *x, const float *model_out,
                 const int64_t *t, int64_t t_scalar, const float *noise, float *x_prev,
                 void *stream);

int da_sample_loop(da_denoiser *d, const da_graph *g, const da_schedule *s, int mean_type,
                   int inference_ratio, int max_iters, const float *x_init, float *traj,
                   float *x_final, void *workspace, size_t workspace_bytes, int use_graph,
                   void *stream);

typedef struct da_loop_opts {
    int32_t sampler;
    float eta;
    int32_t cfg;
    float cfg_w;
    const float *noise;
} da_loop_opts;
int da_sample_loop_ex(da_denoiser *d, const da_graph *g, const da_schedule *s, int mean_type,
                      int inference_ratio, int max_iters, const float *x_init, float *traj,
                      float *x_final, void *workspace, size_t workspace_bytes, int use_graph,
                      const da_loop_opts *opts, void *stream);

int da_sample_loop_pair(da_denoiser *d, const da_schedule *s, int mean_type, int inference_ratio,
                        int max_iters,
                        const da_graph *g_a, const float *x_init_a, float *x_final_a,
                        void *workspace_a, size_t workspace_a_bytes,
                        const da_graph *g_b, const float *x_init_b, float *x_final_b,
                        void *workspace_b, size_t workspace_b_bytes, void *stream);
int da_sample_loop_pair_traj(da_denoiser *d, const da_schedule *s, int mean_type, int inference_ratio,
                             int max_iters,
                             const da_graph *g_a, const float *x_init_a, float *x_final_a,
                             void *workspace_a, size_t workspace_a_bytes,
                             const da_graph *g_b, const float *x_init_b, float *x_final_b,
                             void *workspace_b, size_t workspace_b_bytes,
                             float *traj_a, float *traj_b, size_t traj_stride, void *stream);
int da_sample_loop_pair_ex(da_denoiser *d, const da_schedule *s, int mean_type, int inference_ratio,
                           int max_iters,
                           const da_graph *g_a, const float *x_init_a, float *x_final_a,
                           void *workspace_a, size_t workspace_a_bytes,
                           const da_graph *g_b, const float *x_init_b, float *x_final_b,
                           void *workspace_b, size_t workspace_b_bytes,
                           float *traj_a, float *traj_b, size_t traj_stride,
                           const da_loop_opts *opts, const float *noise_b, size_t noise_stride, void *stream);

int da_denoiser_forward_idx(da_denoiser *d, const da_graph *g, const int32_t *idx, const int64_t *t, int64_t t_scalar,
                            float *logits, float *alpha, int alpha_all_layers, void *workspace, size_t workspace_bytes,
                            void *stream);

int da_d3pm_step(const da_schedule *s, int n, int K, const int32_t *x_t, const float *logits, const int64_t *t,
                 int64_t t_scalar, int inference_ratio, const float *noise, const uint64_t *seed, int iteration,
                 int32_t *x_prev, float *post, void *stream);

int da_d3pm_noise(const uint64_t *seed, int iteration, int n, int K, float *u, void *stream);
enum { DA_D3PM_DRAW_SAMPLING = 0, DA_D3PM_DRAW_TRAINING = 1 };
int da_d3pm_noise_ex(const uint64_t *seed, int iteration, int n, int K, int domain, float *u, void *stream);

typedef struct da_d3pm_opts {
    int32_t cfg;
    float cfg_w;
    const float *noise;
    const uint64_t *seed;
} da_d3pm_opts;
int da_sample_loop_idx(da_denoiser *d, const da_graph *g, const da_schedule *s, int inference_ratio, int max_iters,
                       const int32_t *idx_init, int32_t *traj, int32_t *idx_final, void *workspace, size_t workspace_bytes,
                       int use_graph, const da_d3pm_opts *opts, void *stream);

int da_denoiser_set_features_rot(da_denoiser *d, const da_graph *g, const float *feats4, void *workspace, size_t workspace_bytes,
                                 void *stream);
int da_denoiser_forward_rot(da_denoiser *d, const da_graph *g, const int32_t *idx, const int32_t *rot_acc, const int64_t *t,
                            int64_t t_scalar, float *logits, float *rot_logits, float *alpha, int alpha_all_layers,
                            void *workspace, size_t workspace_bytes, void *stream);

int da_d3pm_rot_step(const da_schedule *s, int n, int K, const int32_t *x_t, const int32_t *rot_t, const float *logits,
                     const float *rot_logits, const int64_t *t, int64_t t_scalar, int inference_ratio, const float *noise_x,
                     const float *noise_rot, const uint64_t *seed, int iteration, int32_t *x_prev, int32_t *rot_0,
                     int32_t *rot_prev, float *post_x, float *post_rot, void *stream);
enum { DA_D3PM_DRAW_SAMPLING_ROT = 2 };

typedef struct da_d3pm_rot_opts {
    int32_t cold;
    int32_t reserved0;
    const int32_t *x_fixed;
    const float *noise_x;
    const float *noise_rot;
    const uint64_t *seed;
} da_d3pm_rot_opts;
int da_sample_loop_rot(da_denoiser *d, const da_graph *g, const da_schedule *s, int inference_ratio, int max_iters,
                       const int32_t *idx_init, const int32_t *rot_init, int32_t *traj_idx, int32_t *traj_rot_acc,
                       int32_t *idx_final, int32_t *rot_acc_final, void *workspace, size_t workspace_bytes, int use_graph,
                       const da_d3pm_rot_opts *opts, void *stream);

enum {
    DA_PROF_EMBED = 0,
    DA_PROF_LINEAR_MLP = 1,
    DA_PROF_LINEAR_QKVS = 2,
    DA_PROF_ATTN_HIDDEN = 3,
    DA_PROF_ATTN_LAST = 4,
    DA_PROF_HEAD = 5,
    DA_PROF_UPDATE = 6,
    DA_PROF_CONV_FUSED = 7,
    DA_PROF_NCLASS = 8
};
int da_profile_enable(da_denoiser *d, int on);
int da_profile_read(da_denoiser *d, float *ms ,
                    int32_t *counts );

int da_linear(int prec, int M, int K, int Nout, const void *A, int lda, const void *W,
              const float *bias, int act, const void *residual, void *out, int ldo, void *stream);

size_t da_linear_packed_bytes(int prec, int K, int Nout);
int da_linear_pack(int prec, int K, int Nout, const void *W, int ldw , void *packed, void *stream);
int da_linear_packed(int prec, int M, int K, int Nout, const void *A, int lda, const void *W, const void *packed,
                     const float *bias, int act, const void *residual, void *out, int ldo, void *stream);

int da_attn_csr(int prec, const da_graph *g, int heads, int C, const void *qkvs, const void *residual,
                int act, void *out, float *alpha, void *stream);

size_t da_attn_dense_scratch_bytes(int prec, const da_graph *g, int heads, int C);
int da_conv_dense(int prec, const da_graph *g, int heads, int C, int Din, const void *x, const void *w,
                  const float *b, const void *residual, int act, void *out, void *scratch, void *stream);

#define DA_CONV_Q_PRESCALED 1
#define DA_CONV_FOLDED_V32 2
int da_conv_dense_ex(int prec, const da_graph *g, int heads, int C, int Din, const void *x, const void *w,
                     const float *b, const void *residual, int act, void *out, void *scratch, int flags,
                     void *stream);

enum {
    DA_DBG_OPT_GEN_WORKGROUPS = 0,
    DA_DBG_DENSE_FAST_EXITS = 1,
    DA_DBG_DUAL_GEN_SLABS = 2,
    DA_DBG_OPT_MASKED_GEN_WORKGROUPS = 3,
    DA_DBG_RES_LAUNCHES = 4,
    DA_DBG_VIRT_IN_LAUNCH = 5,
    DA_DBG_RES_PROJ_LAUNCHES = 6,
    DA_DBG_NCOUNTERS = 8
};
int da_debug_counters(int64_t *out , int n, int reset);

size_t da_train_workspace_bytes(const da_weights *w, const da_graph *g);
size_t da_train_workspace_bytes_ex(const da_weights *w, const da_graph *g, int mma_precision);
#define DA_TRAIN_MMA_FP32 0
#define DA_TRAIN_MMA_BF16 1
int da_train_forward(const da_weights *w, const da_graph *g, const float *x, const int64_t *t,
                     const float *feats, float *out, void *workspace, size_t workspace_bytes,
                     void *stream);
int da_train_backward(const da_weights *w, const da_weights *grads, const da_graph *g, const float *x,
                      const int64_t *t, const float *d_out, float *d_feats, void *workspace,
                      size_t workspace_bytes, void *stream);
int da_train_forward_ex(const da_weights *w, const da_graph *g, const float *x, const int64_t *t,
                        const float *feats, float *out, void *workspace, size_t workspace_bytes,
                        int mma_precision, void *stream);
int da_train_backward_ex(const da_weights *w, const da_weights *grads, const da_graph *g, const float *x,
                         const int64_t *t, const float *d_out, float *d_feats, void *workspace,
                         size_t workspace_bytes, int mma_precision, void *stream);
#define DA_TRAIN_BWD_ALL 0
#define DA_TRAIN_BWD_EARLY 1
#define DA_TRAIN_BWD_LATE 2
int da_train_backward_stage(const da_weights *w, const da_weights *grads, const da_graph *g, const float *x,
                            const int64_t *t, const float *d_out, float *d_feats, void *workspace,
                            size_t workspace_bytes, int mma_precision, int stage, void *stream);

int da_q_sample(int steps, int n, int c, const float *sqrt_alphas_cumprod, const float *sqrt_one_minus_alphas_cumprod,
                const float *x_start, const float *noise, const int64_t *t, float *x_noisy, void *stream);
int da_loss_grad(int kind, size_t n, const float *target, const float *pred, float *loss, float *d_pred, void *stream);

enum { DA_D3PM_LOSS_VB = 0, DA_D3PM_LOSS_CE = 1, DA_D3PM_LOSS_HYBRID = 2 };
int da_d3pm_q_sample(const da_schedule *s, int n, int K, const int32_t *x_start, const int64_t *t, const float *noise,
                     const uint64_t *seed, int iteration, int32_t *x_noisy, void *stream);
int da_d3pm_loss(const da_schedule *s, int n, int K, int kind, float lambda, const float *logits, const int32_t *x_start,
                 const int32_t *x_t, const int64_t *t, float *loss, float *d_logits, float *row_terms, void *stream);
int da_train_forward_idx(const da_weights *w, const da_graph *g, const int32_t *idx, const int64_t *t, const float *feats,
                         float *logits, void *workspace, size_t workspace_bytes, int mma_precision, void *stream);
int da_train_backward_idx(const da_weights *w, const da_weights *grads, const da_graph *g, const int32_t *idx,
                          const int64_t *t, const float *d_logits, float *d_feats, void *workspace, size_t workspace_bytes,
                          int mma_precision, int stage, void *stream);

int da_head3d_backward(int n, const float *pre, const float *d_out, float *d_pre, void *stream);
int da_q_sample_se3(int steps, int n, const float *sqrt_alphas_cumprod, const float *sqrt_one_minus_alphas_cumprod, const float *trap,
                    const float *x_start, const int64_t *t, const float *noise_tr, const float *axes, const float *unif,
                    float *x_noisy, void *stream);

int da_adafactor_step(int n_params, const void *param_table, int n_blocks, const void *block_table,
                      float *flat, const float *flat_grad, float *state, float *scratch,
                      size_t scratch_floats, int step, float eps1, float eps2, float clip_threshold,
                      float decay_rate, void *stream);

int da_adafactor_nd_step(int n_params, const void *param_table, int n_blocks, const void *block_table,
                         int n_jobs, const void *job_table, int *steps, float *state, float *scratch,
                         size_t scratch_floats, int n_slices, size_t colpart_floats, size_t rowpart_floats,
                         float eps1, float eps2, float clip_threshold, float decay_rate, void *stream);

int da_greedy_assign(int n_puzzles, const float *pos1, int ld1, const float *pos2, int ld2,
                     const int32_t *ptr1, const int32_t *ptr2, int max_n, int max_m, long long *out,
                     void *stream);

enum { DA_ENCODER_CONVS = 19, DA_ENCODER_FEATS = 1088 };
typedef struct da_encoder_weights {
    int32_t n_convs;
    int32_t reserved0;
    const float *stem_w, *stem_b;
    const void *conv_w[DA_ENCODER_CONVS];
    const float *conv_b[DA_ENCODER_CONVS];
    const void *lin1_w; const float *lin1_b;
    const void *lin2_w; const float *lin2_b;
} da_encoder_weights;

size_t da_encoder_workspace_bytes(int precision, int n_patches, int chunk);

int da_encoder_forward(int precision, const da_encoder_weights *w, int n_patches, const float *patches,
                       void *feats, int ld_feats, void *workspace, size_t workspace_bytes, int chunk,
                       int zero_workspace, void *stream);

enum { DA_PCD_K = 20, DA_PCD_C = 21, DA_PCD_ROW = 64, DA_PCD_STAGES = 3 };
typedef struct da_pcd_encoder_weights {
    int32_t feat_dim;
    int32_t reserved0;
    const float *premap[DA_PCD_STAGES];
    const float *bn_a[DA_PCD_STAGES];
    const float *conv_b[DA_PCD_STAGES];
    const float *conv6;
    const float *linear0;
} da_pcd_encoder_weights;

size_t da_pcd_encoder_workspace_bytes(int n_points, int chunk, int feat_dim);

int da_pcd_encoder_forward(const da_pcd_encoder_weights *w, int n_parts, int n_points, const float *points, int inv,
                           float *out, int ld_out, void *workspace, size_t workspace_bytes, int chunk, void *stream);

int da_knn(int n_clouds, int n_points, int dim, const float *x, int ldx, int k, int32_t *idx, void *stream);

enum { DA_PCD_TRAIN_LAYERS = 8 };
typedef struct da_pcd_train_weights {
    int32_t feat_dim;
    int32_t reserved0;
    const float *premap[DA_PCD_STAGES];
    float *bn_a[DA_PCD_STAGES];
    float *conv_b[DA_PCD_STAGES];
    float *conv6;
    const float *linear0;
    const float *gamma[DA_PCD_TRAIN_LAYERS], *beta[DA_PCD_TRAIN_LAYERS];
    const float *running_mean[DA_PCD_TRAIN_LAYERS], *running_var[DA_PCD_TRAIN_LAYERS];
    float momentum[DA_PCD_TRAIN_LAYERS], eps[DA_PCD_TRAIN_LAYERS];
    const float *inv_wf[2], *inv_wd[2];
} da_pcd_train_weights;

typedef struct da_pcd_train_grads {
    float *wf[6], *wd[6];
    float *gamma[6], *beta[6];
    float *linear0_w, *linear0_b;
    float *points;
} da_pcd_train_grads;

size_t da_pcd_train_state_bytes(int n_parts, int n_points, int feat_dim);
size_t da_pcd_train_workspace_bytes(int n_parts, int n_points, int chunk, int feat_dim);

int da_pcd_train_forward(const da_pcd_train_weights *w, int n_parts, int n_points, const float *points, int inv, float *out,
                         int ld_out, float *run_out, void *state, size_t state_bytes, void *workspace, size_t workspace_bytes,
                         void *stream);

int da_pcd_train_backward(const da_pcd_train_weights *w, int n_parts, int n_points, const float *points, int inv,
                          const float *grad_out, int ld_g, void *state, const da_pcd_train_grads *g, void *workspace,
                          size_t workspace_bytes, int chunk, void *stream);

enum {
    DA_PCD_PASS_PREMAP = 0,
    DA_PCD_PASS_EDGE_STAT_A,
    DA_PCD_PASS_EDGE_STAT_B,
    DA_PCD_PASS_EDGE_BWD1,
    DA_PCD_PASS_EDGE_BWD2,
    DA_PCD_PASS_EDGE_BWD3,
    DA_PCD_PASS_C6_STAT,
    DA_PCD_PASS_C6_BWD1,
    DA_PCD_PASS_C6_BWD2,
    DA_PCD_PASS_C6_DX,
    DA_PCD_PASS_BN_FIN_FWD,
    DA_PCD_PASS_BN_FIN_BWD,
    DA_PCD_PASS_REV_ADJ,
    DA_PCD_PASS_GATHER,
    DA_PCD_PASS_PREMAP_WGRAD,
    DA_PCD_PASS_HEAD_BWD,
    DA_PCD_PASS_LIN0_GRAD,
    DA_PCD_PASS_VN_LIN,
    DA_PCD_PASS_VN_STAT,
    DA_PCD_PASS_VN_APPLY
};
typedef struct da_pcd_pass_args {
    int32_t n_parts, n_points;
// ... 71 lines not shown
```

Baseline: 101,200.

## Chain fused-projection attention layers through a fragment-major activation layout

```diff
diff --git a/diffassemble_amd/_lib.py b/diffassemble_amd/_lib.py
--- a/diffassemble_amd/_lib.py
+++ b/diffassemble_amd/_lib.py
@@ -12,13 +12,15 @@
 MEAN_EPSILON, MEAN_START_X = 0, 1
 ACT_NONE, ACT_GELU, ACT_LEAKY02 = 0, 1, 2
 CONV_Q_PRESCALED, CONV_FOLDED_V32 = 1, 2
+CONV_X_FM, CONV_OUT_FM = 4, 8
+FOLD_ATTN_PROJ, FOLD_X_FM = 64, 128
 TRAIN_MMA_FP32, TRAIN_MMA_BF16 = 0, 1
 TRAIN_BWD_ALL, TRAIN_BWD_EARLY, TRAIN_BWD_LATE = 0, 1, 2
 D3PM_DRAW_SAMPLING, D3PM_DRAW_TRAINING, D3PM_DRAW_SAMPLING_ROT = 0, 1, 2
 D3PM_LOSS = {"vb": 0, "cross_entropy": 1, "hybrid": 2}
 DBG_COUNTERS = ("opt_gen_workgroups", "dense_fast_exits", "dual_gen_slabs", "opt_masked_gen_workgroups")
 DBG_LAUNCH_COUNTERS = {"resident_launches": 4, "virtual_rows_in_launch": 5,
-                       "resident_projection_launches": 6}
+                       "resident_projection_launches": 6, "resident_fm_input_launches": 7}
 PROF_CLASSES = ("embed", "linear_mlp", "linear_qkvs", "attn_hidden", "attn_last", "head", "update", "conv_fused")
 
 _fp = C.c_void_p
diff --git a/diffassemble_amd/csrc/da_api.hip b/diffassemble_amd/csrc/da_api.hip
--- a/diffassemble_amd/csrc/da_api.hip
+++ b/diffassemble_amd/csrc/da_api.hip
@@ -96,6 +96,7 @@
     void *conv0c_wdp = nullptr, *convLf_wp = nullptr;
     void *conv0c_wqs = nullptr;
     bool attn_qsf = false;
+    bool attn_x_fm = false;
     float *conv0c_bd = nullptr;
     bool q_prescaled = false;
     bool lastfold = false;
@@ -164,8 +165,9 @@
     w.combined = take(np * d->D * s);
     const bool gcn = d->arch == DA_ARCH_GCN;
     w.qkvs = take(gcn ? 0 : np * 4 * (size_t)hcmax * s);
-    w.xa = take(np * 256 * s);
-    w.xb = take(np * 256 * s);
+    const size_t nx = (g->dense || g->hybrid) && (size_t)g->n_pad > np ? (size_t)g->n_pad : np;
+    w.xa = take(nx * 256 * s);
+    w.xb = take(nx * 256 * s);
     w.z = take(np * d->D * s);
     w.hh = take(nrp * d->head_hidden * s);
     const bool disc = d->variant == DA_VARIANT_DISCRETE;
@@ -317,6 +319,20 @@
              return linear(prec, nr, d->hidden, D, w.h, d->hidden, d->mlp_w1, d->mlp_b1, act2, nullptr, w.combined, D, st); }))) return rc;
     const void *xin = fused ? w.h : w.combined;
     int ldx = fused ? d->hidden : D;
+    auto layer_qsf = [&](int l, int ldx_in) -> bool {
+        if (l < 0 || l >= d->n_layers - 1 || d->arch == DA_ARCH_GCN) return false;
+        const ConvW &c = d->conv[l];
+        const int din = (fused && l == 0) ? d->hidden : c.din;
+        const void *wqs = (fused && l == 0) ? d->conv0c_wqs : c.wqs;
+        const bool virt0 = fused && l == 0 && n > nr, al = alpha && alpha_all;
+        if (al || !w.dq || !dense_ok(g, d->heads, c.C)) return false;
+#ifdef DA_EXPERIMENTS
+        if (g->dense && !g->hybrid && n == nr && conv_fused_applicable(prec, d->heads, c.C, din, g->max_graph_nodes, c.hc)) return false;
+#endif
+        return !g->hybrid && !virt0 && n == nr && wqs && ldx_in == din &&
+               attn_qsf_applicable(prec, d->heads, c.C, din, g->n_graphs, g->max_graph_nodes, g->n_pad, d->q_prescaled);
+    };
+    bool x_fm = false;
     if (d->arch == DA_ARCH_GCN) {
         const ConvW &c0 = d->conv[0], &c1 = d->conv[1];
         const int hid = c0.hc;
@@ -408,8 +424,9 @@
             const int xpm = xpanel_mode();
             const void *wpanel = (xpm == 1 || (xpm == 2 && step_rule_batch(g))) ? ((fused && l == 0) ? d->conv0c_wdp : c.wdp) : nullptr;
             const void *wqs = (fused && l == 0) ? d->conv0c_wqs : c.wqs;
-            const bool qsf = !last && !g->hybrid && !resid && !virt0 && n == nr && wqs && ldx == c.din &&
-                             attn_qsf_applicable(prec, d->heads, c.C, c.din, g->n_graphs, g->max_graph_nodes, g->n_pad, d->q_prescaled);
+            const bool qsf = !resid && layer_qsf(l, ldx);
+            const bool out_fm = qsf && d->attn_x_fm && layer_qsf(l + 1, c.hc);
+            DA_REQUIRE(!x_fm || qsf, "da_denoiser_forward: layer %d was handed fragment-major rows it does not take", l);
             if (qsf) rc = 0; else
             rc = timed(d, DA_PROF_LINEAR_QKVS, st, [&] {
                 return launch_gemm_mfma(prec, nproj, c.din, 4 * c.hc, xin, ldx, wdense, bdense, DA_ACT_NONE, nullptr, nullptr, 0, &qs, st, 0,
@@ -421,7 +438,7 @@
             if (rc == 0) {
                 DenseLayout L;
                 L.Q = w.dq; L.K = w.dk; L.Vt = w.dvt; L.S = w.dskip; L.n_pad = g->n_pad; L.q_prescaled = d->q_prescaled;
-                if (qsf) { L.x = xin; L.ldx = ldx; L.kin = c.din; L.wqs = wqs; L.bias = bdense; }
+                if (qsf) { L.x = xin; L.ldx = ldx; L.kin = c.din; L.wqs = wqs; L.bias = bdense; L.x_fm = x_fm; L.out_fm = out_fm; }
                 if (g->hybrid) {
                     DenseMask mk = dense_mask_of(g);
                     int virt_taken = 0;
@@ -473,9 +490,10 @@
                     return launch_attn_dense(prec, L, d->heads, c.C, g->n_graphs, g->max_graph_nodes, g->graph_ptr,
                                              g->pad_ptr, g->dense == 2, resid, act, dst, st); });
                 if (rc > 0) return rc;
-                if (rc == 0) { xin = dst; ldx = c.hc; continue; }
+                if (rc == 0) { xin = dst; ldx = c.hc; x_fm = out_fm; continue; }
             }
         }
+        DA_REQUIRE(!x_fm, "da_denoiser_forward: layer %d was handed fragment-major rows it does not take", l);
         if ((rc = timed(d, DA_PROF_LINEAR_QKVS, st, [&] {
                  return linear(prec, nproj, c.din, 4 * c.hc, xin, ldx, c.w, c.b, DA_ACT_NONE, nullptr, w.qkvs, 4 * c.hc, st); }))) return rc;
         if (virt0 && (rc = launch_scatter_virtual(prec, n - nr, d->V, d->heads, c.C, d->virt_qkvs, nr, nullptr, 0, nullptr, nullptr,
@@ -669,6 +687,7 @@
         return p;
     };
     d->attn_qsf = attn_qsf_enabled();
+    d->attn_x_fm = d->attn_qsf && !(cfg().disable_folds & DA_FOLD_X_FM);
     auto pack_qs = [&](const void *wsrc, int K, int hc, int C) -> void * {
         if (!d->attn_qsf) return nullptr;
         if (precision != DA_PREC_BF16 || C != 32 || H != 8 || (K != 128 && K != 256) || !wsrc || mfma_disabled()) return nullptr;
@@ -1377,6 +1396,8 @@
     const bool qsf = attn_qsf_enabled() && !folded && !residual && !g->hybrid && g->n_nodes == g->n_real && b && w_qs_bytes(heads, Din) <= 2 * hb &&
                      attn_qsf_applicable(prec, heads, C, Din, g->n_graphs, g->max_graph_nodes, g->n_pad, (flags & DA_CONV_Q_PRESCALED) ? 1 : 0);
     void *wq_img = base + hb;
+    DA_REQUIRE(qsf || !(flags & DA_CONV_X_FM), "da_conv_dense_ex: DA_CONV_X_FM on a call that does not take the projection in the attention kernel");
+    DA_REQUIRE(qsf || !(flags & DA_CONV_OUT_FM), "da_conv_dense_ex: DA_CONV_OUT_FM on a call that does not take the projection in the attention kernel");
     int rc = 0;
     if (qsf) {
         if ((rc = pack_w_qs(heads, Din, (int)hc, w, wq_img, st))) return rc;
@@ -1385,7 +1406,7 @@
     DA_REQUIRE(rc == 0, "da_conv_dense_ex: projection shape (Din=%d, Nout=%d) not supported by the MFMA kernels", Din, nout);
     DenseLayout L;
     L.Q = qs.Q; L.K = qs.K; L.Vt = qs.Vt; L.S = qs.S; L.n_pad = g->n_pad; L.q_prescaled = (flags & DA_CONV_Q_PRESCALED) ? 1 : 0;
-    if (qsf) { L.x = x; L.ldx = Din; L.kin = Din; L.wqs = wq_img; L.bias = b; }
+    if (qsf) { L.x = x; L.ldx = Din; L.kin = Din; L.wqs = wq_img; L.bias = b; L.x_fm = (flags & DA_CONV_X_FM) != 0; L.out_fm = (flags & DA_CONV_OUT_FM) != 0; }
     DenseFold fo;
     fo.cv = 32; fo.out = out; fo.n_rows = g->n_real;
     const DenseMask mk = dense_mask_of(g);
@@ -1410,6 +1431,7 @@
     out[DA_DBG_OPT_MASKED_GEN_WORKGROUPS] = (int64_t)a[2];
     out[DA_DBG_RES_LAUNCHES] = (int64_t)da::attn_res_launches(reset);
     out[DA_DBG_RES_PROJ_LAUNCHES] = (int64_t)da::attn_res_qsf_launches(reset);
+    out[DA_DBG_RES_FM_LAUNCHES] = (int64_t)da::attn_res_fm_launches(reset);
     out[DA_DBG_VIRT_IN_LAUNCH] = (int64_t)da::attn_virt_launches(reset);
     return 0;
 }
diff --git a/diffassemble_amd/csrc/da_attn_common.h b/diffassemble_amd/csrc/da_attn_common.h
--- a/diffassemble_amd/csrc/da_attn_common.h
+++ b/diffassemble_amd/csrc/da_attn_common.h
@@ -44,6 +44,7 @@
     int ldx, kin;
     const void *wqs;
     const float *bias_q, *bias_k, *bias_v, *bias_s;
+    int x_fm = 0, out_fm = 0;
 };
 
 template <typename T, int C, int CV = C, int BK = 0> struct Cfg {
diff --git a/diffassemble_amd/csrc/da_attn_dense.hip b/diffassemble_amd/csrc/da_attn_dense.hip
--- a/diffassemble_amd/csrc/da_attn_dense.hip
+++ b/diffassemble_amd/csrc/da_attn_dense.hip
@@ -719,6 +719,8 @@
     p.graph_ptr = graph_ptr; p.pad_ptr = pad_ptr; p.n_pad = L.n_pad; p.H = heads; p.n_graphs = n_graphs;
     p.nqt = 0; p.max_nodes = max_graph_nodes; p.act = act; p.nodiag = nodiag;
     p.x = L.x; p.ldx = L.ldx; p.kin = L.kin; p.wqs = L.wqs;
+    DA_REQUIRE(L.x || !(L.x_fm || L.out_fm), "launch_attn_dense: fragment-major rows without the projection in the attention kernel");
+    p.x_fm = L.x_fm ? 1 : 0; p.out_fm = L.out_fm ? 1 : 0;
     p.bias_q = L.bias; p.bias_k = L.bias ? L.bias + heads * C : nullptr; p.bias_v = L.bias ? L.bias + 2 * heads * C : nullptr; p.bias_s = L.bias ? L.bias + 3 * heads * C : nullptr;
     p.fast = L.q_prescaled ? 1 : 0;
     if (DA_XENV("DA_ATTN_NO_FAST", 0)) p.fast = 0;
@@ -736,7 +738,6 @@
     p.v_part = virt ? mk->v_part : nullptr; p.v_cnt = virt ? mk->v_cnt : nullptr;
     if (mk && mk->v_taken) *mk->v_taken = 0;
     { const char *e = DA_XENV_LIVE("DA_ATTN_DEBUG"); p.debug = e ? atoi(e) : 0; }
-    if (p.x && DA_XENV("DA_QSF_FAKE_FM", 0)) p.debug = 77;
     { const int fg = DA_XENV("DA_ATTN_FORCE_GEN", 0) ? 1 : 0; p.force_gen = fg; if (fg) p.fast = p.fast ? 2 : 0; }
     { const char *e = DA_XENV_LIVE("DA_ATTN_PROF_PTR"); p.prof = e ? (unsigned long long *)strtoull(e, nullptr, 0) : nullptr; }
     if (n_graphs <= 0 || max_graph_nodes <= 0) return 0;
diff --git a/diffassemble_amd/csrc/da_attn_opt.hip b/diffassemble_amd/csrc/da_attn_opt.hip
--- a/diffassemble_amd/csrc/da_attn_opt.hip
+++ b/diffassemble_amd/csrc/da_attn_opt.hip
@@ -882,12 +882,11 @@
     };
     static_assert(!PROG || CF::NCH == 2, "progressive landing: two Q fragments per lane");
     [[maybe_unused]] u32x4 xq[KS];
-    [[maybe_unused]] const int xstep = p.debug == 77 ? 1024 : 32;
+    [[maybe_unused]] const int xstep = p.x_fm ? 1024 : 32;
     [[maybe_unused]] auto x_row = [&](int sl) {
+        if (p.x_fm) return (const unsigned char *)p.x + ((size_t)((pad0 >> 5) + sl) * KS) * 1024 + lane * 16;
         const int nd = max(min(sl * 32 + i, n_g - 1), 0);
-        const unsigned char *row = (const unsigned char *)p.x + ((size_t)(node0 + nd) * (size_t)p.ldx + 8 * half) * 2;
-        if (p.debug == 77) row = (const unsigned char *)p.x + ((size_t)(node0 + max(min(sl * 32, n_g - 32), 0)) * (size_t)p.ldx) * 2 + lane * 16;
-        return row;
+        return (const unsigned char *)p.x + ((size_t)(node0 + nd) * (size_t)p.ldx + 8 * half) * 2;
     };
     [[maybe_unused]] auto x_issue = [&](int sl) {
         const unsigned char *row = x_row(sl);
@@ -946,13 +945,15 @@
     [[maybe_unused]] auto project_kv = [&](auto rl, int sl, const unsigned char *nxt = nullptr) {
         const int rt = (sl & 1) * 32 + i;
         unsigned char *st_ = smem + (size_t)(sl >> 1) * STAGE + (size_t)rt * 64;
+        const bool live = sl * 32 + i < n_g;
+        auto keep_live = [&](u32x4 c_) { return live ? c_ : (u32x4){0u, 0u, 0u, 0u}; };
         f32x16 a;
         chain1(NoReload(), wimg, a);
 #pragma unroll
-        for (int t = 0; t < 2; ++t) *(u32x4 *)(st_ + (((2 * t + half) ^ KG::f(rt)) << 4)) = chunk_of(a, 1, t);
+        for (int t = 0; t < 2; ++t) *(u32x4 *)(st_ + (((2 * t + half) ^ KG::f(rt)) << 4)) = keep_live(chunk_of(a, 1, t));
         chain1(rl, wimg + (size_t)KS * 1024, a, nxt);
 #pragma unroll
-        for (int t = 0; t < 2; ++t) *(u32x4 *)(st_ + KG::KBYTES + ((2 * t + half) << 4)) = chunk_of(a, 2, t);
+        for (int t = 0; t < 2; ++t) *(u32x4 *)(st_ + KG::KBYTES + ((2 * t + half) << 4)) = keep_live(chunk_of(a, 2, t));
     };
     if constexpr (QSF) { if (slab < nslab) x_issue(slab); }
     else if constexpr (!PROG) load_q(slab, qf);
@@ -1345,6 +1346,14 @@
         if (more) load_q(nxt, qn);
         const float lt = ls + __shfl_xor(ls, 32);
         const float inv = lt > 0.f ? 1.0f / (lt + (gen ? 1e-16f : 0.f)) : 0.f;
+        [[maybe_unused]] auto fm_row = [&]() { return (T *)p.out + ((size_t)((pad0 >> 5) + slab) * (size_t)(HC >> 4) + 2 * h) * 512 + (unsigned)(8 * i + 4 * half); };
+        if constexpr (QSF) {
+            if (p.out_fm && qidx >= n_g) {
+                T *zrow = fm_row();
+#pragma unroll
+                for (int jj = 0; jj < 4; ++jj) *(u32x2 *)(zrow + 256 * jj) = (u32x2){0u, 0u};
+            }
+        }
         if (qidx < n_g) {
             const size_t roff = (size_t)(MSK ? my_node : node0 + qidx) * HC + (size_t)h * C + 4 * half;
             u32x2 sk[4], rs[4];
@@ -1353,6 +1362,9 @@
                 sk[jj] = *(const u32x2 *)((const T *)p.S + roff + 8 * jj);
                 rs[jj] = p.res ? *(const u32x2 *)((const T *)p.res + roff + 8 * jj) : (u32x2){0u, 0u};
             }
+            T *orow = (T *)p.out + roff;
+            int ostep = 8;
+            if constexpr (QSF) { if (p.out_fm) { orow = fm_row(); ostep = 256; } }
 #pragma unroll
             for (int jj = 0; jj < 4; ++jj) {
                 float v4[4] = {__fmul_rn(O[4 * jj], inv), __fmul_rn(O[4 * jj + 1], inv), __fmul_rn(O[4 * jj + 2], inv), __fmul_rn(O[4 * jj + 3], inv)};
@@ -1364,7 +1376,7 @@
                 }
 #pragma unroll
                 for (int e = 0; e < 4; ++e) v4[e] = apply_act(v4[e], p.act);
-                st4((T *)p.out + roff + 8 * jj, v4);
+                st4(orow + jj * ostep, v4);
             }
         }
         if (more) {
@@ -1386,6 +1398,10 @@
 static long long g_res_qsf_launches = 0;
 long long attn_res_qsf_launches(int reset) {
     return reset ? __atomic_exchange_n(&g_res_qsf_launches, 0ll, __ATOMIC_RELAXED) : __atomic_load_n(&g_res_qsf_launches, __ATOMIC_RELAXED);
+}
+static long long g_res_fm_launches = 0;
+long long attn_res_fm_launches(int reset) {
+    return reset ? __atomic_exchange_n(&g_res_fm_launches, 0ll, __ATOMIC_RELAXED) : __atomic_load_n(&g_res_fm_launches, __ATOMIC_RELAXED);
 }
 
 static size_t attn_res_qsf_lds(int max_nodes, int kin) {
@@ -1469,6 +1485,7 @@
                     DA_REQUIRE(attn_res_qsf_shape_ok(p.max_nodes, p.n_pad, p.n_graphs, p.kin) && p.wqs && p.bias_q && p.bias_k && p.bias_v && p.bias_s,
                                "k_attn_res: projection in the prologue requested for a shape it does not take");
                     __atomic_fetch_add(&g_res_qsf_launches, 1ll, __ATOMIC_RELAXED);
+                    if (p.x_fm) __atomic_fetch_add(&g_res_fm_launches, 1ll, __ATOMIC_RELAXED);
                     return p.kin == 256 ? launch_res<16, true, true, 64>(p, st) : launch_res<16, true, true, 64 + 128>(p, st);
                 }
 #ifdef DA_EXPERIMENTS
diff --git a/diffassemble_amd/csrc/da_config.h b/diffassemble_amd/csrc/da_config.h
--- a/diffassemble_amd/csrc/da_config.h
+++ b/diffassemble_amd/csrc/da_config.h
@@ -7,7 +7,7 @@
 
 da_config &cfg();
 
-enum { DA_FOLD_MLP2 = 1, DA_FOLD_LAST = 2, DA_FOLD_QSCALE = 4, DA_FOLD_DDIM = 8, DA_FOLD_TAIL = 16, DA_FOLD_HYBRID_OVERLAP = 32, DA_FOLD_ATTN_PROJ = 64 };
+enum { DA_FOLD_MLP2 = 1, DA_FOLD_LAST = 2, DA_FOLD_QSCALE = 4, DA_FOLD_DDIM = 8, DA_FOLD_TAIL = 16, DA_FOLD_HYBRID_OVERLAP = 32, DA_FOLD_ATTN_PROJ = 64, DA_FOLD_X_FM = 128 };
 
 #ifdef DA_EXPERIMENTS
 inline int xenv_read(const char *name, int dflt) { const char *e = getenv(name); return e ? atoi(e) : dflt; }
diff --git a/diffassemble_amd/csrc/da_internal.h b/diffassemble_amd/csrc/da_internal.h
--- a/diffassemble_amd/csrc/da_internal.h
+++ b/diffassemble_amd/csrc/da_internal.h
@@ -127,6 +127,7 @@
     int ldx = 0, kin = 0;
     const void *wqs = nullptr;
     const float *bias = nullptr;
+    bool x_fm = false, out_fm = false;
 };
 bool attn_qsf_applicable(int prec, int heads, int C, int kin, int n_graphs, int max_graph_nodes, int n_pad, int q_prescaled);
 bool attn_qsf_enabled();
@@ -180,6 +181,7 @@
 long long attn_virt_launches(int reset);
 long long attn_res_launches(int reset);
 long long attn_res_qsf_launches(int reset);
+long long attn_res_fm_launches(int reset);
 int attn_dual_counters(unsigned long long *out2, int reset);
 int launch_attn_csr_cont(int prec, int n_nodes, int n_real, const int32_t *irr_row_ptr, const int32_t *irr_col_src,
                          const int32_t *row_map, int heads, int C, int n_pad, const DenseLayout &L,
diff --git a/include/diffassemble_hip.h b/include/diffassemble_hip.h
--- a/include/diffassemble_hip.h
+++ b/include/diffassemble_hip.h
@@ -256,6 +256,8 @@
 
 #define DA_CONV_Q_PRESCALED 1
 #define DA_CONV_FOLDED_V32 2
+#define DA_CONV_X_FM 4
+#define DA_CONV_OUT_FM 8
 int da_conv_dense_ex(int prec, const da_graph *g, int heads, int C, int Din, const void *x, const void *w,
                      const float *b, const void *residual, int act, void *out, void *scratch, int flags,
                      void *stream);
@@ -268,6 +270,7 @@
     DA_DBG_RES_LAUNCHES = 4,
     DA_DBG_VIRT_IN_LAUNCH = 5,
     DA_DBG_RES_PROJ_LAUNCHES = 6,
+    DA_DBG_RES_FM_LAUNCHES = 7,
     DA_DBG_NCOUNTERS = 8
 };
 int da_debug_counters(int64_t *out , int n, int reset);
```

Measured after the change: 104,500, median of 6. +3.3%, better.
